# ddrakard/tensorflow-distributed-on-gke

Measured on AMD Instinct MI355X. Metric: tokens/sec (whole node), Transformer-base en-pt at 1/2/4/8 MI355X, higher is better.
Workload: dtype bf16; 1 GPU; model=transformer-base (6L, d_model=512, heads=8, d_ff=2048, vocab 7765/7010), global_batch=64, local_batch=64, seq_len=128, parallelism=dp1, hip_graph=single, grad_comm=fp32, defer_wgrad=True

## Files before the change

csrc/bindings/gemm.cpp:

```cpp
#include "common.h"

namespace {

void check_operand(const Tensor& t, bool kc, int64_t mn, int64_t K, int64_t ld, const char* n) {
  check_bf16(t, n);
  check_aligned(t, 16, n);
  if (kc) check_extent(t, mn, ld, round8(K), n);
  else check_extent(t, K, ld, round8(mn), n);
}
void check_group_c(const Tensor& C, bool f32, int64_t M, int64_t N, int64_t ldc) {
  TORCH_CHECK(C.is_cuda() && (C.scalar_type() == at::kFloat) == f32 &&
                  (f32 || C.scalar_type() == at::kBFloat16),
              "grouped gemm: C dtypes must match (f32 or bf16)");
  check_extent(C, M, ldc, N, "C");
}

void gemm(const Tensor& A, const Tensor& B, const Tensor& C, const optional<Tensor>& bias,
          const optional<Tensor>& aux, int64_t M, int64_t N, int64_t K, int64_t lda, int64_t ldb,
          int64_t ldc, int64_t ldaux, bool a_kc, bool b_kc, int64_t epi, double alpha,
          double beta, int64_t tile_cfg, int64_t splits, const optional<Tensor>& ws) {
  TORCH_CHECK(C.is_cuda(), "C must be a GPU tensor");
  const bool f32 = C.scalar_type() == at::kFloat;
  TORCH_CHECK(f32 || C.scalar_type() == at::kBFloat16, "C must be f32 or bf16");
  TORCH_CHECK(M > 0 && N > 0 && K > 0, "gemm: empty problem");
  TORCH_CHECK(lda % 8 == 0 && ldb % 8 == 0, "gemm: lda/ldb must be multiples of 8");
  TORCH_CHECK(lda >= round8(a_kc ? K : M), "gemm: lda < round8(", a_kc ? "K)" : "M)");
  TORCH_CHECK(ldb >= round8(b_kc ? K : N), "gemm: ldb < round8(", b_kc ? "K)" : "N)");
  check_operand(A, a_kc, M, K, lda, "A");
  check_operand(B, b_kc, N, K, ldb, "B");
  TORCH_CHECK(ldc >= N, "gemm: ldc < N");
  check_extent(C, M, ldc, N, "C");
  const float* bptr = nullptr;
  if (epi == 1 || epi == 2) {
    TORCH_CHECK(bias.has_value(), "gemm: bias epilogue needs bias");
    check_f32(*bias, "bias");
    TORCH_CHECK(bias->numel() >= N, "gemm: bias too short");
    bptr = bias->data_ptr<float>();
  }
  const void* xptr = nullptr;
  if (epi == 3) {
    TORCH_CHECK(aux.has_value(), "gemm: DRELU epilogue needs aux");
    check_bf16(*aux, "aux");
    check_extent(*aux, M, ldaux, N, "aux");
    xptr = aux->data_ptr();
  }
  float* wptr = nullptr;
  if (splits > 1) {
    TORCH_CHECK(ws.has_value(), "gemm: split-K needs a workspace");
    check_f32(*ws, "ws");
    TORCH_CHECK(ws->numel() >= splits * M * ldc, "gemm: workspace too small");
    wptr = ws->data_ptr<float>();
  }
  c10::DeviceGuard g(A.device());
  const int rc = tdg_gemm(A.data_ptr(), B.data_ptr(), C.data_ptr(), bptr, xptr, (int)M, (int)N,
                          (int)K, (int)lda, (int)ldb, (int)ldc, (int)ldaux, a_kc, b_kc, (int)epi,
                          f32, (float)alpha, (float)beta, (int)tile_cfg, (int)splits, wptr,
                          stream_of(A));
  check_err(rc, "tdg gemm");
}

void gemm_grouped(const std::vector<Tensor>& As, const std::vector<Tensor>& Bs,
                  const std::vector<Tensor>& Cs, int64_t M, int64_t N, int64_t K, int64_t lda,
                  int64_t ldb, int64_t ldc, bool a_kc, bool b_kc, double alpha, double beta,
                  int64_t tile_cfg) {
  const size_t G = As.size();
  TORCH_CHECK(G >= 1 && G <= 32 && Bs.size() == G && Cs.size() == G, "gemm_grouped: 1..32 problems");
  TORCH_CHECK(M > 0 && N > 0 && K > 0 && lda % 8 == 0 && ldb % 8 == 0 && ldc >= N, "gemm_grouped: shape");
  const bool f32 = Cs[0].scalar_type() == at::kFloat;
  std::vector<const void*> a(G), b(G);
  std::vector<void*> c(G);
  for (size_t i = 0; i < G; ++i) {
    check_operand(As[i], a_kc, M, K, lda, "A");
    check_operand(Bs[i], b_kc, N, K, ldb, "B");
    check_group_c(Cs[i], f32, M, N, ldc);
    a[i] = As[i].data_ptr();
    b[i] = Bs[i].data_ptr();
    c[i] = Cs[i].data_ptr();
  }
  c10::DeviceGuard g(As[0].device());
  const int rc = tdg_gemm_grouped(a.data(), b.data(), c.data(), (int)G, (int)M, (int)N, (int)K,
                                  (int)lda, (int)ldb, (int)ldc, a_kc, b_kc, f32, (float)alpha,
                                  (float)beta, (int)tile_cfg, stream_of(As[0]));
  check_err(rc, "tdg gemm_grouped");
}

void gemm_ragged(const std::vector<Tensor>& As, const std::vector<Tensor>& Bs,
                 const std::vector<Tensor>& Cs, const std::vector<int64_t>& shapes, int64_t K,
                 bool a_kc, bool b_kc, double alpha, double beta,
                 const std::vector<c10::optional<Tensor>>& bias_out) {
  const size_t P = As.size();
  TORCH_CHECK(P >= 1 && P <= 64 && Bs.size() == P && Cs.size() == P && shapes.size() == 7 * P,
              "gemm_ragged: 1..64 problems, 7 shape values each (M, N, lda, ldb, ldc, t_first, "
              "t_count)");
  TORCH_CHECK(K > 0 && K % 64 == 0, "gemm_ragged: K must be a multiple of 64");
  const bool f32 = Cs[0].scalar_type() == at::kFloat;
  std::vector<const void*> a(P), b(P);
  std::vector<void*> c(P);
  std::vector<int> sh(7 * P);
  for (size_t i = 0; i < P; ++i) {
    const int64_t M = shapes[7 * i], N = shapes[7 * i + 1], lda = shapes[7 * i + 2],
                  ldb = shapes[7 * i + 3], ldc = shapes[7 * i + 4];
    TORCH_CHECK(M > 0 && N > 0 && lda % 8 == 0 && ldb % 8 == 0 && ldc >= N, "gemm_ragged: shape");
    check_operand(As[i], a_kc, M, K, lda, "A");
    check_operand(Bs[i], b_kc, N, K, ldb, "B");
    check_group_c(Cs[i], f32, M, N, ldc);
    a[i] = As[i].data_ptr();
    b[i] = Bs[i].data_ptr();
    c[i] = Cs[i].data_ptr();
    for (int j = 0; j < 7; ++j) sh[7 * i + j] = (int)shapes[7 * i + j];
  }
  TORCH_CHECK(bias_out.empty() || bias_out.size() == P, "gemm_ragged: bias_out must be empty or P long");
  std::vector<float*> bo(P, nullptr);
  bool any_bias = false;
  for (size_t i = 0; i < bias_out.size(); ++i) {
    if (!bias_out[i].has_value()) continue;
    const Tensor& t = *bias_out[i];
    TORCH_CHECK(!a_kc, "gemm_ragged: fused bias sums need an MN-contiguous A");
    check_f32(t, "bias_out");
    TORCH_CHECK(t.is_contiguous() && t.numel() == shapes[7 * i], "gemm_ragged: bias_out[", i,
                "] must hold M floats");
    bo[i] = t.data_ptr<float>();
    any_bias = true;
  }
  c10::DeviceGuard g(As[0].device());
  const int rc = tdg_gemm_ragged(a.data(), b.data(), c.data(), (int)P, sh.data(), (int)K, a_kc,
                                 b_kc, f32, (float)alpha, (float)beta,
                                 any_bias ? bo.data() : nullptr, stream_of(As[0]));
  check_err(rc, "tdg gemm_ragged");
}

void colsum(const Tensor& X, const Tensor& out, const Tensor& part, int64_t M, int64_t N,
            int64_t ld, int64_t rows_per_block, double beta) {
  check_bf16(X, "X");
  check_f32(out, "out");
  check_f32(part, "part");
  check_extent(X, M, ld, N, "X");
  TORCH_CHECK(out.numel() >= N, "colsum: out too short");
  TORCH_CHECK(part.numel() >= ((M + rows_per_block - 1) / rows_per_block) * N,
              "colsum: partial buffer too small");
  c10::DeviceGuard g(X.device());
  tdg_colsum(X.data_ptr(), out.data_ptr<float>(), part.data_ptr<float>(), (int)M, (int)N, (int)ld,
             (int)rows_per_block, (float)beta, stream_of(X));
  check_err(0, "tdg colsum");
}

void colsum_grouped(const std::vector<Tensor>& Xs, const std::vector<Tensor>& outs,
                    const Tensor& part, int64_t M, int64_t N, int64_t ld, int64_t rows_per_block,
                    double beta) {
  const size_t G = Xs.size();
  TORCH_CHECK(G >= 1 && G <= 32 && outs.size() == G, "colsum_grouped: 1..32 problems");
  check_f32(part, "part");
  const int64_t nparts = (M + rows_per_block - 1) / rows_per_block;
  TORCH_CHECK(part.numel() >= (int64_t)G * nparts * N, "colsum_grouped: partials too small");
  std::vector<const void*> x(G);
  std::vector<float*> o(G);
  for (size_t i = 0; i < G; ++i) {
    check_bf16(Xs[i], "X");
    check_extent(Xs[i], M, ld, N, "X");
    check_f32(outs[i], "out");
    TORCH_CHECK(outs[i].numel() >= N, "colsum_grouped: out too short");
    x[i] = Xs[i].data_ptr();
    o[i] = outs[i].data_ptr<float>();
  }
  c10::DeviceGuard g(Xs[0].device());
  check_err(tdg_colsum_grouped(x.data(), o.data(), (int)G, part.data_ptr<float>(), (int)M, (int)N,
                               (int)ld, (int)rows_per_block, (float)beta, stream_of(Xs[0])),
            "tdg colsum_grouped");
}

}

void def_gemm(py::module_& m) {
  m.def("gemm", &gemm);
  m.def("gemm_grouped", &gemm_grouped);
  m.def("gemm_ragged", &gemm_ragged, py::arg("As"), py::arg("Bs"), py::arg("Cs"), py::arg("shapes"),
        py::arg("K"), py::arg("a_kc"), py::arg("b_kc"), py::arg("alpha"), py::arg("beta"),
        py::arg("bias_out") = std::vector<c10::optional<Tensor>>{});
  m.def("colsum", &colsum);
  m.def("colsum_grouped", &colsum_grouped);
}
```

csrc/include/tdg_api.h:

```cpp
#pragma once
#include <hip/hip_runtime.h>
#include <stdint.h>

#include "tdg_attn.h"

extern "C" {

int tdg_gemm(const void* A, const void* B, void* C, const float* bias, const void* aux, int M,
             int N, int K, int lda, int ldb, int ldc, int ldaux, int a_kc, int b_kc, int epi,
             int out_f32, float alpha, float beta, int tile_cfg, int splits, float* ws,
             hipStream_t st);
int tdg_gemm_grouped(const void* const* A, const void* const* B, void* const* C, int G, int M,
                     int N, int K, int lda, int ldb, int ldc, int a_kc, int b_kc, int out_f32,
                     float alpha, float beta, int tile_cfg, hipStream_t st);
int tdg_gemm_ragged(const void* const* A, const void* const* B, void* const* C, int P,
                    const int* shapes, int K, int a_kc, int b_kc, int out_f32, float alpha,
                    float beta, float* const* bias_out, hipStream_t st);
void tdg_colsum(const void* X, float* out, float* part, int M, int N, int ld, int rows_per_block,
                float beta, hipStream_t st);
int tdg_colsum_grouped(const void* const* X, float* const* out, int G, float* part, int M, int N,
                       int ld, int rows_per_block, float beta, hipStream_t st);

int tdg_attn_fwd(const tdg::AttnArgs* a, int hd, hipStream_t st);
int tdg_qkv_attn_fwd(const tdg::QkvAttnArgs* qa, hipStream_t st);
int tdg_attn_bwd(const tdg::AttnArgs* a, int hd, hipStream_t st);
int tdg_attn_bwd_fdo(const tdg::AttnArgs* a, hipStream_t st);
int tdg_attn_probs(const tdg::AttnArgs* a, int hd, float* probs, hipStream_t st);
int tdg_attn_fwd_fp8(const tdg::AttnArgs* a, int hd, hipStream_t st);
int tdg_attn_bwd_f8(const tdg::AttnArgs* a, int hd, hipStream_t st);

int tdg_ln_fwd(const void* x, const void* s, const float* gamma, const float* beta, void* y,
               void* hsave, float* mean, float* rstd, int M, int D, float p, uint64_t seed,
               const long long* ctr, uint64_t site, float eps, void* y8, const float* s8,
               unsigned* amax8, void* kbits, hipStream_t st);
int tdg_ln_bwd(const void* dy, const void* hsave, const float* mean, const float* rstd,
               const float* gamma, void* dh, void* ds, const void* dres, float* dgamma,
               float* dbeta, float* dbias, float* ws, int M, int D, float p, uint64_t seed,
               const long long* ctr, uint64_t site, int accumulate, int skip_reduce, int rpb,
               void* ds8, const float* s8, unsigned* amax8, const void* kbits, hipStream_t st);
int tdg_reduce_partials_multi(const float* const* parts, float* const* outs, const int* nparts,
                              int G, int N, float beta, hipStream_t st);

int tdg_embed_fwd(const void* tok, int tok64, const void* table, const float* pe, void* out, int M,
                  int L, int D, float scale, float p, uint64_t seed, const long long* ctr,
                  uint64_t site, void* kbits, hipStream_t st);
int tdg_embed_bwd(const void* tok, int tok64, const void* dout, float* dtable, int M, int D,
                  float scale, float p, uint64_t seed, const long long* ctr, uint64_t site,
                  hipStream_t st);
int tdg_embed_bwd_det(const void* tok, int tok64, const void* dout, float* dtable, long long* acc,
                      int M, int D, long long V, float scale, float p, uint64_t seed,
                      const long long* ctr, uint64_t site, float beta, hipStream_t st);
void tdg_embed_csr_ws(int M, int V, int D, long long* n32, long long* n64);
int tdg_embed_csr_ok(int M, int V);
int tdg_embed_csr_sort(int ntab, const void* const* tok, const int* tok64, const int* M,
                       const int* V, int* const* ws32, long long* stamps, hipStream_t st);
int tdg_embed_csr_apply(const void* dout, const void* kbits, float* dtable, int* ws32,
                        long long* ws64, int M, int D, int V, float scale, float p, uint64_t seed,
                        const long long* ctr, uint64_t site, float beta, hipStream_t st);

int tdg_count_tokens(const void* labels, int lab64, int M, float* out, hipStream_t st);
int tdg_prep_batch(const void* src, int S, const void* tgt, int T1, int B, int lab64, void* tgt_in,
                   void* labels, int* src_len, int* tgt_len, float* ntok, long long* ctr,
                   int* row_lab, unsigned* ticket, int* bad_rows, hipStream_t st);
int tdg_xent(void* logits, int M, int V, int ldl, const void* labels, int lab64, const float* ntok,
             float workers, float smoothing, float* row_loss, float* row_correct, int write_grad,
             hipStream_t st);
int tdg_xent_stats(const float* row_loss, const float* row_correct, int M, const float* ntok,
                   float workers, float* step_out, float* accum, hipStream_t st);

int tdg_adam(float* p, float* g, float* m, float* v, void* shadow, long long n, long long* step,
             float beta1, float beta2, float eps, float lr_const, float d_model, float warmup,
             float grad_scale, float weight_decay, int sched, int zero_grad, int inc_step,
             const float* gstate, hipStream_t st);
int tdg_adam_chunks(float* p, float* g, float* m, float* v, void* shadow, long long n,
                    const void* chunks, int nchunks, long long* step, float beta1, float beta2,
                    float eps, float lr_const, float d_model, float warmup, float grad_scale,
                    float weight_decay, int sched, int zero_grad, int inc_step,
                    const float* scale8, unsigned* amax8, const float* gstate, hipStream_t st);
int tdg_adam_step_inc(long long* step, const float* gstate, hipStream_t st);
long long tdg_grad_sumsq(const float* g, const void* chunks, long long nchunks, long long n,
                         float* partials, hipStream_t st);
int tdg_grad_norm_finalize(const float* partials, long long nparts, float* state,
                           unsigned* counters, float clip, int skip_on, float grad_scale,
                           hipStream_t st);
int tdg_to_bf16(const float* p, void* o, long long n, hipStream_t st);
int tdg_transpose_grouped(const void* const* src, void* const* dst, int G, int R, int C,
                          hipStream_t st);

int tdg_gemm_fp8(const void* A, const void* B, void* C, const float* bias, const float* sa,
                 const float* sb, void* C8, const float* sc8, unsigned* amax, int M, int N, int K,
                 int lda, int ldb, int ldc, int ldc8, int epi, int cfg, int afmt, int cfmt,
                 const void* aux, int ldaux, float beta, const void* aux8, float* colsum_out,
                 float colsum_beta, float* ws, hipStream_t st);
int tdg_wgrad_fp8(const void* const* A, const void* const* B, float* const* C,
                  const float* const* sa, const float* const* sb, int P, const int* shapes, int T,
                  float beta, hipStream_t st);
int tdg_fp8_set_persist(int on);
int tdg_fp8_quant(const void* x, void* y8, long long n, const float* scale, unsigned* amax,
                  int fmt, hipStream_t st);
int tdg_fp8_quant_multi(const void* const* x, void* const* y, const long long* n, const int* slot,
                        int nseg, const float* scale, unsigned* amax, hipStream_t st);
int tdg_fp8_quant_colsum(const void* x, int ld, void* y8, int M, int N, const float* scale,
                         unsigned* amax, float* part, int fmt, hipStream_t st);
int tdg_fp8_quant_t(const void* const* src, void* const* dst, const int* slot, int G, int R, int C,
                    const float* scale, unsigned* amax, hipStream_t st);
int tdg_fp8_scale_update(float* scale, unsigned* amax, int n, float margin_pow2, float fmax,
                         hipStream_t st);
int tdg_fp8_dequant(const void* x8, float* y, long long n, float inv_scale, hipStream_t st);

int tdg_signal_create(unsigned long long** host, unsigned long long** dhost,
                      unsigned long long** cnt);
int tdg_signal_emit(unsigned long long* cnt, unsigned long long* dhost, hipStream_t st);

}
```

csrc/include/tdg_gemm.h:

```cpp
#pragma once
#include "tdg_common.h"

#include <type_traits>

namespace tdg {

constexpr int BK = 64;

template <bool KC, int R>
__device__ __forceinline__ int lds_off(int row, int byte) {
  if constexpr (KC) {
    const int seg = (byte >> 5) ^ ((row >> 1) & 3);
    return row * (BK * 2) + (seg << 5) + (byte & 31);
  } else if constexpr (R >= 128) {
    const int seg = (byte >> 5) ^ ((row & 3) | (((row >> 3) & 1) << 2));
    return row * (R * 2) + (seg << 5) + (byte & 31);
  } else {
    static_assert(R == 64, "MN-contiguous tiles must be 64 or 128 wide");
    const int seg = (byte >> 5) ^ (((row >> 1) & 1) | (((row >> 3) & 1) << 1));
    return row * 128 + (seg << 5) + (byte & 31);
  }
}

template <bool KC, int R, int NW>
struct Glds {
  static constexpr int BYTES = R * BK * 2;
  static constexpr int P = BYTES / (NW * 1024);
  static_assert(BYTES % (NW * 1024) == 0, "tile must split into 1 KiB pieces per wave");
  static constexpr int RPP = KC ? 8 : 1024 / (R * 2);
  static constexpr int CPR = KC ? 8 : R / 8;
  int row[P];
  int col[P];
  __device__ __forceinline__ void init(int wid, int lane) {
#pragma unroll
    for (int i = 0; i < P; ++i) {
      const int j = wid * P + i;
      const int r = j * RPP + lane / CPR;
      const int pc = lane % CPR;
      int c;
      if constexpr (KC) {
        c = (((pc >> 1) ^ ((r >> 1) & 3)) << 1) | (pc & 1);
      } else if constexpr (R >= 128) {
        c = (((pc >> 1) ^ ((r & 3) | (((r >> 3) & 1) << 2))) << 1) | (pc & 1);
      } else {
        c = (((pc >> 1) ^ (((r >> 1) & 1) | (((r >> 3) & 1) << 1))) << 1) | (pc & 1);
      }
      row[i] = r;
      col[i] = c * 8;
    }
  }
  __device__ __forceinline__ void issue(const bf16_t* __restrict__ X, int ld, int len, int kend,
                                        int mn0, int k0, char* lds, int wid) const {
#pragma unroll
    for (int i = 0; i < P; ++i) {
      long long off;
      if constexpr (KC) {
        int mn = mn0 + row[i];
        mn = mn < len ? mn : len - 1;
        int k = k0 + col[i];
        k = k < kend ? k : 0;
        off = (long long)mn * ld + k;
      } else {
        int k = k0 + row[i];
        k = k < kend ? k : kend - 1;
        int mn = mn0 + col[i];
        mn = mn < len ? mn : 0;
        off = (long long)k * ld + mn;
      }
      __builtin_amdgcn_global_load_lds(
          (const void*)(X + off),
          (__attribute__((address_space(3))) void*)(lds + (wid * P + i) * 1024), 16, 0, 0);
    }
  }
  __device__ __forceinline__ static void zero_ktail(char* lds, int k0, int kend, int tid, int nt) {
    if constexpr (KC) {
      for (int id = tid; id < R * 8; id += nt) {
        const int r = id >> 3, c = id & 7;
        const int kk = k0 + c * 8;
        if (kk + 8 <= kend) continue;
        short8_t* p = reinterpret_cast<short8_t*>(lds + lds_off<KC, R>(r, c * 16));
        short8_t v = *p;
#pragma unroll
        for (int e = 0; e < 8; ++e)
          if (kk + e >= kend) v[e] = 0;
        *p = v;
      }
    } else {
      for (int id = tid; id < BK * (R / 8); id += nt) {
        const int r = id / (R / 8), c = id % (R / 8);
        if (k0 + r < kend) continue;
        *reinterpret_cast<short8_t*>(lds + lds_off<KC, R>(r, c * 16)) =
            short8_t{0, 0, 0, 0, 0, 0, 0, 0};
      }
    }
  }
};

#ifndef TDG_EPI_SC1
#define TDG_EPI_SC1 1
#endif
#ifndef TDG_GEMM_PRIO
#define TDG_GEMM_PRIO 1
#endif
__device__ __forceinline__ void prio_hi() {
  if (TDG_GEMM_PRIO) __builtin_amdgcn_s_setprio(1);
}
__device__ __forceinline__ void prio_lo() {
  if (TDG_GEMM_PRIO) __builtin_amdgcn_s_setprio(0);
}

template <int N>
__device__ __forceinline__ void wait_vmcnt() {
  asm volatile("s_waitcnt vmcnt(%0)" ::"n"(N) : "memory");
}
template <int N>
__device__ __forceinline__ void wait_vmcnt_known() {
  static_assert(N >= 0 && N <= 63, "vmcnt range");
  __builtin_amdgcn_s_waitcnt((N & 15) | (7 << 4) | (15 << 8) | ((N >> 4) << 14));
}

template <int PT, int NMAX>
__device__ __forceinline__ void wait_tiles(int n) {
  static_assert(NMAX <= 6 && PT * NMAX <= 63, "vmcnt range");
  if (NMAX >= 6 && n >= 6) { wait_vmcnt<(NMAX >= 6 ? 6 * PT : 0)>(); return; }
  if (NMAX >= 5 && n >= 5) { wait_vmcnt<(NMAX >= 5 ? 5 * PT : 0)>(); return; }
  if (NMAX >= 4 && n >= 4) { wait_vmcnt<(NMAX >= 4 ? 4 * PT : 0)>(); return; }
  if (NMAX >= 3 && n >= 3) { wait_vmcnt<(NMAX >= 3 ? 3 * PT : 0)>(); return; }
  if (NMAX >= 2 && n >= 2) { wait_vmcnt<(NMAX >= 2 ? 2 * PT : 0)>(); return; }
  if (NMAX >= 1 && n >= 1) { wait_vmcnt<PT>(); return; }
  wait_vmcnt<0>();
}

__device__ __forceinline__ void lds_barrier() {
  asm volatile("s_waitcnt lgkmcnt(0)" ::: "memory");
  __builtin_amdgcn_s_barrier();
  asm volatile("" ::: "memory");
}

template <bool KC, int R>
__device__ __forceinline__ short8_t frag(const char* lds, int base, int s, int lane) {
  if constexpr (KC) {
    const int row = base + (lane & 15);
    const int byte = (s * 4 + (lane >> 4)) * 16;
    return lds_read_b128_async(lds + lds_off<KC, R>(row, byte));
  } else {
    const int g = lane >> 4, w = lane & 15, q = w >> 2, p = w & 3;
    const int krow = s * 32 + 8 * g + q;
    const int byte = (base + 4 * p) * 2;
    const short4_t lo = lds_read_tr_async(lds + lds_off<KC, R>(krow, byte));
    const short4_t hi = lds_read_tr_async(lds + lds_off<KC, R>(krow + 4, byte));
    return cat4(lo, hi);
  }
}

template <bool KC>
constexpr int frag_ops() {
  return KC ? 1 : 2;
}

enum Epi : int {
  EPI_NONE = 0,
  EPI_BIAS = 1,
  EPI_BIAS_RELU = 2,
  EPI_DRELU = 3,
};

template <int EPI>
__device__ __forceinline__ f32x4 load_bias4(const float* __restrict__ bias, int n, int N) {
  f32x4 b = {0.f, 0.f, 0.f, 0.f};
  if constexpr (EPI == EPI_BIAS || EPI == EPI_BIAS_RELU) {
    if (n + 4 <= N && (reinterpret_cast<uintptr_t>(bias + n) & 15) == 0) {
      b = *reinterpret_cast<const f32x4*>(bias + n);
    } else {
#pragma unroll
      for (int r = 0; r < 4; ++r) b[r] = bias[min(n + r, N - 1)];
    }
  }
  return b;
}

template <int EPI, bool OUT_F32>
__device__ __forceinline__ bool epi_vec_ok(const void* C, int ldc, const bf16_t* aux, int ldaux) {
  constexpr int ES = OUT_F32 ? 4 : 2;
  bool ok = (ldc % 4) == 0 && (reinterpret_cast<uintptr_t>(C) % (4 * ES)) == 0;
  if constexpr (EPI == EPI_DRELU) ok = ok && (ldaux % 4) == 0 && (reinterpret_cast<uintptr_t>(aux) & 7) == 0;
  return ok;
}

template <int EPI, bool OUT_F32>
__device__ __forceinline__ void epi_store4(void* __restrict__ Cv, int ldc, int M, int N, int m, int n,
                                           const f32x4& a, float alpha, float beta, const f32x4& bn,
                                           const bf16_t* __restrict__ aux, int ldaux, bool vec) {
  if (m >= M || n >= N) return;
  float v[4];
#pragma unroll
  for (int r = 0; r < 4; ++r) {
    v[r] = alpha * a[r];
    if constexpr (EPI == EPI_BIAS) v[r] += bn[r];
    if constexpr (EPI == EPI_BIAS_RELU) v[r] = fmaxf(v[r] + bn[r], 0.f);
  }
  const size_t off = (size_t)m * ldc + n;
  if (vec && n + 4 <= N) {
    if constexpr (EPI == EPI_DRELU) {
      const short4_t x = *reinterpret_cast<const short4_t*>(aux + (size_t)m * ldaux + n);
#pragma unroll
      for (int r = 0; r < 4; ++r)
        if (!(bf2f((bf16_t)x[r]) > 0.f)) v[r] = 0.f;
    }
    if constexpr (OUT_F32) {
      f32x4* cp = reinterpret_cast<f32x4*>(reinterpret_cast<float*>(Cv) + off);
      f32x4 o = {v[0], v[1], v[2], v[3]};
      if (beta != 0.f) o += beta * *cp;
      *cp = o;
    } else {
      short4_t* cp = reinterpret_cast<short4_t*>(reinterpret_cast<bf16_t*>(Cv) + off);
      if (beta != 0.f) {
        const short4_t old = *cp;
#pragma unroll
        for (int r = 0; r < 4; ++r) v[r] += beta * bf2f((bf16_t)old[r]);
      }
      short4_t o;
#pragma unroll
      for (int r = 0; r < 4; ++r) o[r] = (short)f2bf(v[r]);
      *cp = o;
    }
  } else {
#pragma unroll
    for (int r = 0; r < 4; ++r) {
      if (n + r >= N) break;
      float x = v[r];
      if constexpr (EPI == EPI_DRELU) {
        if (!(bf2f(aux[(size_t)m * ldaux + n + r]) > 0.f)) x = 0.f;
      }
      if constexpr (OUT_F32) {
        float* cp = reinterpret_cast<float*>(Cv) + off + r;
        if (beta != 0.f) x += beta * *cp;
        *cp = x;
      } else {
        bf16_t* cp = reinterpret_cast<bf16_t*>(Cv) + off + r;
        if (beta != 0.f) x += beta * bf2f(*cp);
        *cp = f2bf(x);
      }
    }
  }
}

template <int EPI, bool OUT_F32, int TM, int TN, int RPASS>
struct EpiLds {
  static constexpr int ES = OUT_F32 ? 4 : 2;
  static constexpr int SP = TN * 16 * ES + 16;
  static constexpr int CPR = TN * 16 * ES / 16;
  static constexpr int EPC = 16 / ES;
  static constexpr int ITER = RPASS * CPR / 64;
  static constexpr int BYTES = RPASS * SP;
  static_assert(RPASS % 16 == 0 && (TM * 16) % RPASS == 0, "passes of whole 16-row sub-tiles");
  static_assert((RPASS * CPR) % 64 == 0, "whole chunk iterations");

  __device__ static __forceinline__ int row_of(int lane, int t) { return (lane + 64 * t) / CPR; }
  __device__ static __forceinline__ int col_of(int lane, int t) { return ((lane + 64 * t) % CPR) * EPC; }

  __device__ static __forceinline__ void run(char* wimg, const f32x4 (&acc)[TM][TN], int lane,
                                             void* __restrict__ Cv, int ldc, int M, int N, int mw0,
                                             int nw0, float alpha, float beta,
                                             const float* __restrict__ bias,
                                             const bf16_t* __restrict__ aux, int ldaux, bool vec) {
    int4 none[ITER];
    run_pre<false>(wimg, acc, lane, Cv, ldc, M, N, mw0, nw0, alpha, beta, bias, aux, ldaux, vec,
                   none, false, none, false);
  }
  template <bool PRE>
  __device__ static __forceinline__ void run_pre(char* wimg, const f32x4 (&acc)[TM][TN], int lane,
                                                 void* __restrict__ Cv, int ldc, int M, int N,
                                                 int mw0, int nw0, float alpha, float beta,
                                                 const float* __restrict__ bias,
                                                 const bf16_t* __restrict__ aux, int ldaux, bool vec,
                                                 const int4 (&pre_aux)[ITER], bool use_aux,
                                                 const int4 (&pre_c)[ITER], bool use_c) {
    const int g = lane >> 4, r16 = lane & 15;
    bool vok = vec && ((ldc * ES) % 16) == 0 && (reinterpret_cast<uintptr_t>(Cv) & 15) == 0;
    if constexpr (EPI == EPI_DRELU)
      vok = vok && (ldaux % EPC) == 0 && (reinterpret_cast<uintptr_t>(aux) % (2 * EPC)) == 0;
#if TDG_EPI_SC1
    const WtBuf wt(Cv, ((size_t)(M - 1) * ldc + N) * ES);
#endif
    f32x4 bn[TN];
#pragma unroll
    for (int j = 0; j < TN; ++j) bn[j] = load_bias4<EPI>(bias, nw0 + 16 * j + 4 * g, N);
    using VecT = typename std::conditional<OUT_F32, f32x4, short8_t>::type;
    constexpr bool AUX8 = EPI == EPI_DRELU && EPC == 8;
    const bool loc_aux = AUX8 && !(PRE && use_aux) && vok;
    const bool loc_c = !(PRE && use_c) && beta != 0.f && vok;
#pragma unroll
    for (int p = 0; p < TM * 16 / RPASS; ++p) {
      int4 la[ITER], lc[ITER];
      if (loc_aux || loc_c) {
#pragma unroll
        for (int t = 0; t < ITER; ++t) {
          const int id = lane + 64 * t;
          const int m = mw0 + p * RPASS + id / CPR, n = nw0 + (id % CPR) * EPC;
          const bool in = m < M && n + EPC <= N;
          if (loc_aux) {
            const bf16_t* a = in ? aux + (size_t)m * ldaux + n : aux;
            la[t] = *reinterpret_cast<const int4*>(a);
          }
          if (loc_c) {
            const char* c = in ? reinterpret_cast<const char*>(Cv) + ((size_t)m * ldc + n) * ES
                               : reinterpret_cast<const char*>(Cv);
            lc[t] = *reinterpret_cast<const int4*>(c);
          }
        }
      }
#pragma unroll
      for (int ii = 0; ii < RPASS / 16; ++ii) {
        const int i = p * (RPASS / 16) + ii;
#pragma unroll
        for (int j = 0; j < TN; ++j) {
          float v[4];
#pragma unroll
          for (int r = 0; r < 4; ++r) {
            v[r] = alpha * acc[i][j][r];
            if constexpr (EPI == EPI_BIAS) v[r] += bn[j][r];
            if constexpr (EPI == EPI_BIAS_RELU) v[r] = fmaxf(v[r] + bn[j][r], 0.f);
          }
          char* dst = wimg + (16 * ii + r16) * SP + (16 * j + 4 * g) * ES;
          if constexpr (OUT_F32) {
            *reinterpret_cast<f32x4*>(dst) = f32x4{v[0], v[1], v[2], v[3]};
          } else {
            short4_t w;
#pragma unroll
            for (int r = 0; r < 4; ++r) w[r] = (short)f2bf(v[r]);
            *reinterpret_cast<short4_t*>(dst) = w;
          }
        }
      }
      asm volatile("s_waitcnt lgkmcnt(0)" ::: "memory");
#pragma unroll
      for (int t = 0; t < ITER; ++t) {
        const int id = lane + 64 * t;
        const int row = id / CPR, ch = id % CPR;
        const int m = mw0 + p * RPASS + row;
        const int n = nw0 + ch * EPC;
        VecT vals = *reinterpret_cast<const VecT*>(wimg + row * SP + ch * 16);
        if (m >= M || n >= N) continue;
        char* cp = reinterpret_cast<char*>(Cv) + ((size_t)m * ldc + n) * ES;
        if (vok && n + EPC <= N) {
          if constexpr (EPI == EPI_DRELU) {
            if constexpr (EPC == 8) {
              const short8_t x = __builtin_bit_cast(short8_t, (PRE && use_aux) ? pre_aux[t] : la[t]);
#pragma unroll
              for (int e = 0; e < 8; ++e)
                if (!(bf2f((bf16_t)x[e]) > 0.f)) vals[e] = 0;
            } else {
              const short4_t x = *reinterpret_cast<const short4_t*>(aux + (size_t)m * ldaux + n);
#pragma unroll
              for (int e = 0; e < 4; ++e)
                if (!(bf2f((bf16_t)x[e]) > 0.f)) vals[e] = 0;
            }
          }
          if (beta != 0.f) {
            const VecT old = __builtin_bit_cast(VecT, (PRE && use_c) ? pre_c[t] : lc[t]);
            if constexpr (OUT_F32) {
              vals += beta * old;
            } else {
#pragma unroll
              for (int e = 0; e < 8; ++e)
                vals[e] = (short)f2bf(bf2f((bf16_t)vals[e]) + beta * bf2f((bf16_t)old[e]));
            }
          }
#if TDG_EPI_SC1
          wt.st16(cp, vals);
#else
          *reinterpret_cast<VecT*>(cp) = vals;
#endif
        } else {
#pragma unroll
          for (int e = 0; e < EPC; ++e) {
            if (n + e >= N) break;
            float v = OUT_F32 ? (float)vals[e] : bf2f((bf16_t)vals[e]);
            if constexpr (EPI == EPI_DRELU) {
              if (!(bf2f(aux[(size_t)m * ldaux + n + e]) > 0.f)) v = 0.f;
            }
            if constexpr (OUT_F32) {
              float* c = reinterpret_cast<float*>(cp) + e;
              if (beta != 0.f) v += beta * *c;
              *c = v;
            } else {
              bf16_t* c = reinterpret_cast<bf16_t*>(cp) + e;
              if (beta != 0.f) v += beta * bf2f(*c);
              *c = f2bf(v);
            }
          }
        }
      }
      asm volatile("s_waitcnt lgkmcnt(0)" ::: "memory");
    }
  }
};

template <int N>
__device__ __forceinline__ void tie_all(short8_t (&f)[N]) {
#pragma unroll
  for (int i = 0; i < N; ++i) tie(f[i]);
}

}
```

csrc/kernels/gemm.hip:

```cpp
#include "tdg_api.h"
#include "gemm_impl.h"

namespace tdg {

__global__ __launch_bounds__(256) void colsum_partial_kernel(const bf16_t* __restrict__ X,
                                                             float* __restrict__ part, int M, int N,
                                                             int ld, int rows_per_block) {
  __shared__ float red[32][65];
  const int cg = threadIdx.x & 7, rl = threadIdx.x >> 3;
  const int col0 = blockIdx.x * 64 + cg * 8;
  const int r0 = blockIdx.y * rows_per_block;
  const int r1 = min(M, r0 + rows_per_block);
  float acc[8];
#pragma unroll
  for (int i = 0; i < 8; ++i) acc[i] = 0.f;
  const bool vec = (col0 + 8 <= N) && (ld % 8 == 0);
  for (int r = r0 + rl; r < r1; r += 32) {
    const bf16_t* p = X + (size_t)r * ld + col0;
    if (vec) {
      const short8_t v = *reinterpret_cast<const short8_t*>(p);
#pragma unroll
      for (int i = 0; i < 8; ++i) acc[i] += bf2f((bf16_t)v[i]);
    } else {
#pragma unroll
      for (int i = 0; i < 8; ++i)
        if (col0 + i < N) acc[i] += bf2f(p[i]);
    }
  }
#pragma unroll
  for (int i = 0; i < 8; ++i) red[rl][cg * 8 + i] = acc[i];
  __syncthreads();
  if (threadIdx.x < 64) {
    float s = 0.f;
#pragma unroll 8
    for (int k = 0; k < 32; ++k) s += red[k][threadIdx.x];
    const int col = blockIdx.x * 64 + threadIdx.x;
    if (col < N) part[(size_t)blockIdx.y * N + col] = s;
  }
}

struct ColsumGroup {
  const bf16_t* X[32];
  float* out[32];
};

__global__ __launch_bounds__(256) void colsum_partial_grouped_kernel(ColsumGroup grp,
                                                                     float* __restrict__ part, int M,
                                                                     int N, int ld,
                                                                     int rows_per_block) {
  __shared__ float red[32][65];
  const bf16_t* X = grp.X[blockIdx.z];
  float* pz = part + (size_t)blockIdx.z * gridDim.y * N;
  const int cg = threadIdx.x & 7, rl = threadIdx.x >> 3;
  const int col0 = blockIdx.x * 64 + cg * 8;
  const int r0 = blockIdx.y * rows_per_block;
  const int r1 = min(M, r0 + rows_per_block);
  float acc[8];
#pragma unroll
  for (int i = 0; i < 8; ++i) acc[i] = 0.f;
  const bool vec = (col0 + 8 <= N) && (ld % 8 == 0);
  for (int r = r0 + rl; r < r1; r += 32) {
    const bf16_t* p = X + (size_t)r * ld + col0;
    if (vec) {
      const short8_t v = *reinterpret_cast<const short8_t*>(p);
#pragma unroll
      for (int i = 0; i < 8; ++i) acc[i] += bf2f((bf16_t)v[i]);
    } else {
#pragma unroll
      for (int i = 0; i < 8; ++i)
        if (col0 + i < N) acc[i] += bf2f(p[i]);
    }
  }
#pragma unroll
  for (int i = 0; i < 8; ++i) red[rl][cg * 8 + i] = acc[i];
  __syncthreads();
  if (threadIdx.x < 64) {
    float s = 0.f;
#pragma unroll 8
    for (int k = 0; k < 32; ++k) s += red[k][threadIdx.x];
    const int col = blockIdx.x * 64 + threadIdx.x;
    if (col < N) pz[(size_t)blockIdx.y * N + col] = s;
  }
}

__global__ __launch_bounds__(256) void reduce_partials_grouped_kernel(ColsumGroup grp,
                                                                      const float* __restrict__ part,
                                                                      int N, int P, float beta) {
  __shared__ float red[4][64];
  const float* pz = part + (size_t)blockIdx.y * P * N;
  float* out = grp.out[blockIdx.y];
  const int c = threadIdx.x & 63, g = threadIdx.x >> 6;
  const int col = blockIdx.x * 64 + c;
  float s = 0.f;
  if (col < N) {
#pragma unroll 8
    for (int p = g; p < P; p += 4) s += pz[(size_t)p * N + col];
  }
  red[g][c] = s;
  __syncthreads();
  if (g == 0 && col < N) {
    const float t = red[0][c] + red[1][c] + red[2][c] + red[3][c];
    out[col] = (beta != 0.f ? beta * out[col] : 0.f) + t;
  }
}

}

extern "C" int tdg_gemm(const void* A, const void* B, void* C, const float* bias, const void* aux,
                        int M, int N, int K, int lda, int ldb, int ldc, int ldaux, int a_kc,
                        int b_kc, int epi, int out_f32, float alpha, float beta, int tile_cfg,
                        int splits, float* ws, hipStream_t st) {
  const bf16_t* a = (const bf16_t*)A;
  const bf16_t* b = (const bf16_t*)B;
  const bf16_t* x = (const bf16_t*)aux;
  auto fn = a_kc ? (b_kc ? gemm_nt : gemm_nn) : (b_kc ? gemm_tt : gemm_tn);
  return fn(epi, out_f32 != 0, tile_cfg, a, b, C, bias, x, M, N, K, lda, ldb, ldc, ldaux, alpha,
            beta, splits, ws, st);
}

extern "C" int tdg_gemm_grouped(const void* const* A, const void* const* B, void* const* C, int G,
                                int M, int N, int K, int lda, int ldb, int ldc, int a_kc, int b_kc,
                                int out_f32, float alpha, float beta, int tile_cfg, hipStream_t st) {
  if (G < 1 || G > MAXG) return -2;
  GemmGroup g{};
  for (int i = 0; i < G; ++i) {
    g.A[i] = (const bf16_t*)A[i];
    g.B[i] = (const bf16_t*)B[i];
    g.C[i] = C[i];
  }
  auto fn = a_kc ? (b_kc ? gemm_grouped_nt : gemm_grouped_nn)
                 : (b_kc ? gemm_grouped_tt : gemm_grouped_tn);
  return fn(g, G, M, N, K, lda, ldb, ldc, out_f32 != 0, alpha, beta, tile_cfg, st);
}

extern "C" int tdg_gemm_ragged(const void* const* A, const void* const* B, void* const* C, int P,
                               const int* shapes, int K, int a_kc, int b_kc, int out_f32,
                               float alpha, float beta, float* const* bias_out,
                               hipStream_t st) {
  if (P < 1 || P > R256_MAXP) return -2;
  R256Args args{};
  int ncls = 0, tiles = 0;
  bool prev_partial = false;
  for (int i = 0; i < P; ++i) {
    const int* s = shapes + 7 * i;
    const int tpp = cdiv(s[0], 256) * cdiv(s[1], 256);
    const int first = s[5], count = s[6] < 0 ? tpp - s[5] : s[6];
    if (first < 0 || count <= 0 || first + count > tpp) return -8;
    const bool partial = count != tpp;
    const bool same = ncls > 0 && !partial && !prev_partial && args.cls[ncls - 1].M == s[0] &&
                      args.cls[ncls - 1].N == s[1] && args.cls[ncls - 1].lda == s[2] &&
                      args.cls[ncls - 1].ldb == s[3] && args.cls[ncls - 1].ldc == s[4];
    if (!same) {
      if (ncls == R256_MAXC) return -5;
      R256Class& c = args.cls[ncls++];
      c.M = s[0]; c.N = s[1]; c.lda = s[2]; c.ldb = s[3]; c.ldc = s[4];
      c.tiles_m = cdiv(s[0], 256); c.tiles_n = cdiv(s[1], 256);
      c.tile_start = tiles; c.prob_start = i; c.t_first = first;
      if ((!a_kc && s[2] % 8) || (!b_kc && s[3] % 8)) return -6;
    }
    prev_partial = partial;
    tiles += count;
    args.A[i] = (const bf16_t*)A[i];
    args.B[i] = (const bf16_t*)B[i];
    args.C[i] = C[i];
    args.bias_out[i] = bias_out ? bias_out[i] : nullptr;
    if (args.bias_out[i] && a_kc) return -7;
  }
  args.ncls = ncls;
  if (a_kc && b_kc) return gemm_ragged_nt(args, tiles, K, out_f32 != 0, alpha, beta, st);
  if (a_kc && !b_kc) return out_f32 ? -4 : gemm_ragged_nn(args, tiles, K, false, alpha, beta, st);
  if (!a_kc && !b_kc) return gemm_ragged_tn(args, tiles, K, out_f32 != 0, alpha, beta, st);
  return -4;
}

extern "C" void tdg_colsum(const void* X, float* out, float* part, int M, int N, int ld,
                           int rows_per_block, float beta, hipStream_t st) {
  const int nparts = cdiv(M, rows_per_block);
  dim3 grid(cdiv(N, 64), nparts);
  hipLaunchKernelGGL(colsum_partial_kernel, grid, dim3(256), 0, st, (const bf16_t*)X, part, M, N,
                     ld, rows_per_block);
  launch_reduce_partials(part, out, N, nparts, beta, st);
}

extern "C" int tdg_colsum_grouped(const void* const* X, float* const* out, int G, float* part,
                                  int M, int N, int ld, int rows_per_block, float beta,
                                  hipStream_t st) {
  if (G < 1 || G > 32) return -2;
  ColsumGroup g{};
  for (int i = 0; i < G; ++i) {
    g.X[i] = (const bf16_t*)X[i];
    g.out[i] = out[i];
  }
  const int nparts = cdiv(M, rows_per_block);
  hipLaunchKernelGGL(colsum_partial_grouped_kernel, dim3(cdiv(N, 64), nparts, G), dim3(256), 0, st,
                     g, part, M, N, ld, rows_per_block);
  hipLaunchKernelGGL(reduce_partials_grouped_kernel, dim3(cdiv(N, 64), G), dim3(256), 0, st, g,
                     part, N, nparts, beta);
  return 0;
}
```

csrc/kernels/gemm_impl.h:

```cpp
#pragma once
#include "tdg_common.h"
#include "tdg_gemm.h"
#include "tdg_reduce.h"
#include "gemm_pipe.h"

#include <cstdlib>
#include <type_traits>

namespace tdg {



constexpr int MAXG = 32;
struct GemmGroup {
  const bf16_t* A[MAXG];
  const bf16_t* B[MAXG];
  void* C[MAXG];
};

template <int BM, int BN, int WM, int WN, int STAGES, bool A_KC, bool B_KC, int EPI,
          bool OUT_F32>
__global__ __launch_bounds__(WM* WN * 64) void gemm_kernel(
    const bf16_t* __restrict__ A, const bf16_t* __restrict__ B, void* __restrict__ Cv,
    const float* __restrict__ bias, const bf16_t* __restrict__ aux, int M, int N, int K, int lda,
    int ldb, int ldc, int ldaux, float alpha, float beta, int k_per_split, long long split_stride,
    const GemmGroup grp) {
  if (gridDim.y > 1) {
    A = grp.A[blockIdx.y];
    B = grp.B[blockIdx.y];
    Cv = grp.C[blockIdx.y];
  }
  constexpr int NW = WM * WN;
  constexpr int NT = NW * 64;
  constexpr int TM = BM / WM / 16;
  constexpr int TN = BN / WN / 16;
  constexpr int A_BYTES = BM * BK * 2, B_BYTES = BN * BK * 2;
  constexpr int SB = A_BYTES + B_BYTES;
  using GA = Glds<A_KC, BM, NW>;
  using GB = Glds<B_KC, BN, NW>;
  constexpr int PT = GA::P + GB::P;
  extern __shared__ __attribute__((aligned(16))) char smem[];

  const int tid = threadIdx.x, lane = tid & 63;
  const int wid = __builtin_amdgcn_readfirstlane(tid >> 6);
  const int wm = wid / WN, wn = wid % WN;
  const int tiles_m = cdiv(M, BM), tiles_n = cdiv(N, BN);
  const int nwg = tiles_m * tiles_n;
  const int t = xcd_remap(blockIdx.x, nwg);
  int tm, tn;
  if (tiles_n <= tiles_m) {
    tn = t % tiles_n;
    tm = t / tiles_n;
  } else {
    tm = t % tiles_m;
    tn = t / tiles_m;
  }
  const int m0 = tm * BM, n0 = tn * BN;
  TDG_STAMP(0);

  const int kb = blockIdx.z * k_per_split;
  const int ke = min(K, kb + k_per_split);
  const int nk = cdiv(ke - kb, BK);
  const bool ktail = ((ke - kb) % BK) != 0;

  GA ga;
  GB gb;
  ga.init(wid, lane);
  gb.init(wid, lane);

  using OutT = typename std::conditional<OUT_F32, float, bf16_t>::type;
  constexpr int WTM = BM / WM, WTN = BN / WN;
  constexpr int RPASS = OUT_F32 ? (WTM < 32 ? WTM : 32) : WTM;
  using Epi = EpiLds<EPI, OUT_F32, TM, TN, RPASS>;
  using EpiF = EpiLds<EPI_NONE, true, TM, TN, (WTM < 32 ? WTM : 32)>;
  static_assert(NW * Epi::BYTES <= STAGES * (BM + BN) * BK * 2 &&
                    NW * EpiF::BYTES <= STAGES * (BM + BN) * BK * 2,
                "epilogue images must fit in the pipeline LDS");
  const bool split = gridDim.z > 1;
  const bool vec = epi_vec_ok<EPI, OUT_F32>(Cv, ldc, aux, ldaux);
  constexpr bool SINGLE = RPASS == WTM;
  const bool pre_aux = SINGLE && EPI == EPI_DRELU && !split && vec && (ldaux % 8) == 0 &&
                       (reinterpret_cast<uintptr_t>(aux) & 15) == 0;
  const bool pre_c = SINGLE && beta != 0.f && !split && vec && ((ldc * (int)sizeof(OutT)) % 16) == 0;
  int4 aux_r[Epi::ITER], c_r[Epi::ITER];
#pragma unroll
  for (int t = 0; t < Epi::ITER; ++t) {
    const int m = m0 + wm * WTM + Epi::row_of(lane, t);
    const int n = n0 + wn * WTN + Epi::col_of(lane, t);
    const bool in = m < M && n + Epi::EPC <= N;
    if (pre_aux && in) aux_r[t] = *reinterpret_cast<const int4*>(aux + (size_t)m * ldaux + n);
    if (pre_c && in)
      c_r[t] = *reinterpret_cast<const int4*>(reinterpret_cast<const OutT*>(Cv) + (size_t)m * ldc + n);
  }

  f32x4 acc[TM][TN];
#pragma unroll
  for (int i = 0; i < TM; ++i)
#pragma unroll
    for (int j = 0; j < TN; ++j) acc[i][j] = f32x4{0.f, 0.f, 0.f, 0.f};

  static_assert(BK == 64, "two 32-deep k-steps per tile");
  const int abase = wm * (BM / WM), bbase = wn * (BN / WN);
#pragma unroll
  for (int s = 0; s < STAGES; ++s) {
    if (s < nk) {
      ga.issue(A, lda, M, ke, m0, kb + s * BK, smem + s * SB, wid);
      gb.issue(B, ldb, N, ke, n0, kb + s * BK, smem + s * SB + A_BYTES, wid);
    }
  }
  short8_t fa0[TM], fb0[TN], fa1[TM], fb1[TN];
  if (nk > 0) {
    if (nk >= STAGES)
      wait_vmcnt<(STAGES - 1) * PT>();
    else
      wait_vmcnt<0>();
    lds_barrier();
    TDG_STAMP(1);
    if (ktail && nk == 1) {
      GA::zero_ktail(smem, kb, ke, tid, NT);
      GB::zero_ktail(smem + A_BYTES, kb, ke, tid, NT);
      lds_barrier();
    }
#pragma unroll
    for (int i = 0; i < TM; ++i) fa0[i] = frag<A_KC, BM>(smem, abase + 16 * i, 0, lane);
#pragma unroll
    for (int j = 0; j < TN; ++j) fb0[j] = frag<B_KC, BN>(smem + A_BYTES, bbase + 16 * j, 0, lane);
  }

  constexpr int STEP_OPS = TM * frag_ops<A_KC>() + TN * frag_ops<B_KC>();
  auto kstep = [&](int kt, auto modec) {
    constexpr int MODE = decltype(modec)::value;
    const char* st = smem + (kt % STAGES) * SB;
#pragma unroll
    for (int i = 0; i < TM; ++i) fa1[i] = frag<A_KC, BM>(st, abase + 16 * i, 1, lane);
#pragma unroll
    for (int j = 0; j < TN; ++j) fb1[j] = frag<B_KC, BN>(st + A_BYTES, bbase + 16 * j, 1, lane);
    lgkm_wait<STEP_OPS>();
    tie_all(fa0);
    tie_all(fb0);
    prio_hi();
#pragma unroll
    for (int i = 0; i < TM; ++i)
#pragma unroll
      for (int j = 0; j < TN; ++j) acc[i][j] = mfma16(fb0[j], fa0[i], acc[i][j]);
    prio_lo();
    if constexpr (MODE >= 1) {
      if constexpr (MODE >= 2) wait_vmcnt<(STAGES - 2) * PT>();
      else wait_vmcnt<0>();
      lds_barrier();
      const char* nx = smem + ((kt + 1) % STAGES) * SB;
      if constexpr (MODE <= 2) {
        if (ktail && kt + 1 == nk - 1) {
          GA::zero_ktail(const_cast<char*>(nx), kb + (kt + 1) * BK, ke, tid, NT);
          GB::zero_ktail(const_cast<char*>(nx) + A_BYTES, kb + (kt + 1) * BK, ke, tid, NT);
          lds_barrier();
        }
      }
      if constexpr (MODE == 3) {
        char* ns = smem + (kt % STAGES) * SB;
        ga.issue(A, lda, M, ke, m0, kb + (kt + STAGES) * BK, ns, wid);
        gb.issue(B, ldb, N, ke, n0, kb + (kt + STAGES) * BK, ns + A_BYTES, wid);
      }
#pragma unroll
      for (int i = 0; i < TM; ++i) fa0[i] = frag<A_KC, BM>(nx, abase + 16 * i, 0, lane);
#pragma unroll
      for (int j = 0; j < TN; ++j) fb0[j] = frag<B_KC, BN>(nx + A_BYTES, bbase + 16 * j, 0, lane);
    } else {
      lgkm_wait<0>();
    }
    tie_all(fa1);
    tie_all(fb1);
    prio_hi();
#pragma unroll
    for (int i = 0; i < TM; ++i)
#pragma unroll
      for (int j = 0; j < TN; ++j) acc[i][j] = mfma16(fb1[j], fa1[i], acc[i][j]);
    prio_lo();
  };
  {
    int kt = 0;
    for (; kt + STAGES < nk; ++kt) kstep(kt, std::integral_constant<int, 3>{});
    if (kt + STAGES - 1 < nk && kt + 1 < nk) kstep(kt++, std::integral_constant<int, 2>{});
    for (; kt + 1 < nk; ++kt) kstep(kt, std::integral_constant<int, 1>{});
    if (kt < nk) kstep(kt, std::integral_constant<int, 0>{});
  }

  TDG_STAMP(2);
  lds_barrier();
  const int mw0 = m0 + wm * WTM, nw0 = n0 + wn * WTN;
  if (split) {
    float* Cs = reinterpret_cast<float*>(Cv) + (size_t)blockIdx.z * split_stride;
    EpiF::run(smem + wid * EpiF::BYTES, acc, lane, Cs, ldc, M, N, mw0, nw0, 1.f, 0.f, nullptr,
              nullptr, 0, epi_vec_ok<EPI_NONE, true>(Cs, ldc, nullptr, 0));
  } else {
    Epi::template run_pre<true>(smem + wid * Epi::BYTES, acc, lane, Cv, ldc, M, N, mw0, nw0, alpha,
                                beta, bias, aux, ldaux, vec, aux_r, pre_aux, c_r, pre_c);
  }
#ifdef TDG_STAMPS
  TDG_STAMP(3);
  asm volatile("s_waitcnt vmcnt(0)" ::: "memory");
  TDG_STAMP(4);
#endif
}

constexpr int R256_MAXP = 64, R256_MAXC = 8;
struct R256Class {
  int M, N, lda, ldb, ldc, tiles_m, tiles_n, tile_start, prob_start, t_first;
};
struct R256Args {
  const bf16_t* A[R256_MAXP];
  const bf16_t* B[R256_MAXP];
  void* C[R256_MAXP];
  float* bias_out[R256_MAXP];
  R256Class cls[R256_MAXC];
  int ncls;
};

template <bool A_KC, bool B_KC, int EPI, bool OUT_F32>
__global__ __launch_bounds__(512) void gemm256_kernel(const R256Args args,
                                                      const float* __restrict__ bias,
                                                      const bf16_t* __restrict__ aux, int K,
                                                      int ldaux, float alpha, float beta) {
  constexpr int NW = 8;
  constexpr int HB = 128 * BK * 2;
  constexpr int SB = 4 * HB;
  using GA = Glds<A_KC, 128, NW>;
  using GB = Glds<B_KC, 128, NW>;
  static_assert(GA::P == 2 && GB::P == 2, "half-tile = 2 pieces per wave");
  extern __shared__ __attribute__((aligned(16))) char smem[];

  const int tid = threadIdx.x, lane = tid & 63;
  const int wid = __builtin_amdgcn_readfirstlane(tid >> 6);
  const int wm = wid >> 2, wn = wid & 3;

  const int t0 = xcd_remap(blockIdx.x, gridDim.x);
  R256Class cl = args.cls[0];
#pragma unroll
  for (int i = 1; i < R256_MAXC; ++i)
    if (i < args.ncls && t0 >= args.cls[i].tile_start) cl = args.cls[i];
  const int M = cl.M, N = cl.N, lda = cl.lda, ldb = cl.ldb, ldc = cl.ldc;
  const int tpp = cl.tiles_m * cl.tiles_n;
  const int lt = t0 - cl.tile_start + cl.t_first;
  const int p = cl.prob_start + lt / tpp;
  const int t = lt % tpp;
  const bf16_t* __restrict__ A = args.A[p];
  const bf16_t* __restrict__ B = args.B[p];
  void* __restrict__ Cv = args.C[p];
  int tm, tn;
  if (cl.tiles_n <= cl.tiles_m) {
    tn = t % cl.tiles_n;
    tm = t / cl.tiles_n;
  } else {
    tm = t % cl.tiles_m;
    tn = t / cl.tiles_m;
  }
  float* __restrict__ bias_out = A_KC ? nullptr : args.bias_out[p];
  const bool do_bsum = bias_out != nullptr && tn == 0;
  float bsum0 = 0.f, bsum1 = 0.f;
  const int m0 = tm * 256, n0 = tn * 256;
  const int nk = K / BK;
  TDG_STAMP(0);

  GA ga;
  GB gb;
  ga.init(wid, lane);
  gb.init(wid, lane);
  uint32_t a_off[2][2], b_off[2][2];
#pragma unroll
  for (int i = 0; i < 2; ++i) {
    const int xa = A_KC ? ga.row[i] : ga.col[i];
    const int xb = B_KC ? gb.row[i] : gb.col[i];
    const int ka = A_KC ? ga.col[i] : ga.row[i];
    const int kb = B_KC ? gb.col[i] : gb.row[i];
#pragma unroll
    for (int hh = 0; hh < 2; ++hh) {
      int ma = m0 + (xa >> 6) * 128 + hh * 64 + (xa & 63);
      int nb = n0 + (xb >> 5) * 64 + hh * 32 + (xb & 31);
      if (A_KC) {
        ma = ma < M ? ma : M - 1;
        a_off[hh][i] = 2u * (uint32_t)(ma * lda + ka);
      } else {
        ma = ma < M ? ma : 0;
        a_off[hh][i] = 2u * (uint32_t)(ka * lda + ma);
      }
      if (B_KC) {
        nb = nb < N ? nb : N - 1;
        b_off[hh][i] = 2u * (uint32_t)(nb * ldb + kb);
      } else {
        nb = nb < N ? nb : 0;
        b_off[hh][i] = 2u * (uint32_t)(kb * ldb + nb);
      }
    }
  }
  const int nrec_a = 2 * (A_KC ? (M - 1) * lda + K : (K - 1) * lda + M);
  const int nrec_b = 2 * (B_KC ? (N - 1) * ldb + K : (K - 1) * ldb + N);
  const uint32_t kstep_a = A_KC ? BK * 2u : (uint32_t)BK * (uint32_t)lda * 2u;
  const uint32_t kstep_b = B_KC ? BK * 2u : (uint32_t)BK * (uint32_t)ldb * 2u;
  auto issue = [&](const bf16_t* X, int nrec, const uint32_t* offs, uint32_t soff, char* dst) {
#pragma unroll
    for (int i = 0; i < 2; ++i)
      __builtin_amdgcn_raw_ptr_buffer_load_lds(
          __builtin_amdgcn_make_buffer_rsrc(const_cast<bf16_t*>(X), (short)0, nrec, 0x00020000),
          (__attribute__((address_space(3))) void*)(dst + (wid * 2 + i) * 1024), 16, offs[i],
          (int)soff, 0, 0);
  };
  auto issue_half = [&](int kt, int h) {
    char* st = smem + (kt & 1) * SB;
    if (h == 0) issue(A, nrec_a, a_off[0], kstep_a * (uint32_t)kt, st + 0 * HB);
    else if (h == 1) issue(B, nrec_b, b_off[0], kstep_b * (uint32_t)kt, st + 2 * HB);
    else if (h == 2) issue(B, nrec_b, b_off[1], kstep_b * (uint32_t)kt, st + 3 * HB);
    else issue(A, nrec_a, a_off[1], kstep_a * (uint32_t)kt, st + 1 * HB);
  };

  f32x4 acc[8][4];
#pragma unroll
  for (int i = 0; i < 8; ++i)
#pragma unroll
    for (int j = 0; j < 4; ++j) acc[i][j] = f32x4{0.f, 0.f, 0.f, 0.f};

  const int arow = wm * 64, brow = wn * 32;
  short8_t fa[8][2], fb[4][2];
  auto bias_sum = [&](int ph) {
    const bf16x2_t one = __builtin_bit_cast(bf16x2_t, 0x3f803f80);
    float bs = ph == 0 ? bsum0 : bsum1;
#pragma unroll
    for (int i = 0; i < 4; ++i) {
      if (i != wn) continue;
#pragma unroll
      for (int s2 = 0; s2 < 2; ++s2) {
        const short8_t f = ph == 0 ? fa[i][s2] : fa[4 + i][s2];
#pragma unroll
        for (int e = 0; e < 4; ++e)
          bs = __builtin_amdgcn_fdot2_f32_bf16(
              __builtin_bit_cast(bf16x2_t, (short2_t){f[2 * e], f[2 * e + 1]}), one, bs, false);
      }
    }
    if (ph == 0) bsum0 = bs;
    else bsum1 = bs;
  };
  {
#pragma unroll
    for (int h = 0; h < 4; ++h) issue_half(0, h);
    if (nk > 1) {
#pragma unroll
      for (int h = 0; h < 3; ++h) issue_half(1, h);
    }
    const int fg = lane >> 4, fcl = lane & 15, fq = fcl >> 2, fp = fcl & 3;
    const uint32_t lds0 = (uint32_t)(uintptr_t)smem;
    auto kc_base = [&](int row0, int s) -> uint32_t {
      return lds0 + (row0 + fcl) * (BK * 2) + (((2 * s + (fg >> 1)) ^ ((fcl >> 1) & 3)) << 5) + (fg & 1) * 16;
    };
    auto mn_base = [&](int sub) -> uint32_t {
      return lds0 + (8 * fg + fq) * 256 + 8 * fp + ((sub ^ (fq | ((fg & 1) << 2))) << 5);
    };
    uint32_t rba[4], rbb[2];
#pragma unroll
    for (int i = 0; i < 4; ++i) rba[i] = A_KC ? kc_base(arow, i & 1) : mn_base((arow >> 4) + i);
#pragma unroll
    for (int j = 0; j < 2; ++j) rbb[j] = B_KC ? kc_base(brow, j) : mn_base((brow >> 4) + j);
    auto frag_imm = [&](auto kcc, auto hc, auto ic, auto sc, const uint32_t* b) -> short8_t {
      constexpr bool KC = decltype(kcc)::value;
      constexpr int H = decltype(hc)::value, I = decltype(ic)::value, S = decltype(sc)::value;
      if constexpr (KC) {
        return lds_read_b128_at<H * HB + I * 16 * BK * 2>(b[S]);
      } else {
        return cat4(lds_read_tr16_at<H * HB + 8192 * S>(b[I]), lds_read_tr16_at<H * HB + 8192 * S + 1024>(b[I]));
      }
    };
    using AKCc = std::integral_constant<bool, A_KC>;
    using BKCc = std::integral_constant<bool, B_KC>;
    auto kstep_deep = [&](int kt, auto modec) {
      constexpr int MODE = decltype(modec)::value;
      const uint32_t stg = (uint32_t)(kt & 1) * SB;
      uint32_t ba[4], bb[2];
#pragma unroll
      for (int i = 0; i < 4; ++i) ba[i] = rba[i] + stg;
#pragma unroll
      for (int j = 0; j < 2; ++j) bb[j] = rbb[j] + stg;
#pragma unroll
      for (int ph = 0; ph < 4; ++ph) {
        if (ph < 3) {
          if (ph == 0) wait_vmcnt<MODE == 1 ? 4 : 10>();
          else if (ph == 1) wait_vmcnt<MODE == 1 ? 2 : 10>();
          else wait_vmcnt<MODE == 3 ? 12 : (MODE == 2 ? 8 : 0)>();
          lds_barrier();
          if (kt == 0 && ph == 0) TDG_STAMP(1);
        }
        using C0 = std::integral_constant<int, 0>;
        using C1 = std::integral_constant<int, 1>;
        using C2 = std::integral_constant<int, 2>;
        using C3 = std::integral_constant<int, 3>;
        if (ph == 0) {
          static_for<4>([&](auto I) {
            fa[I][0] = frag_imm(AKCc{}, C0{}, I, C0{}, ba);
            fa[I][1] = frag_imm(AKCc{}, C0{}, I, C1{}, ba);
          });
          static_for<2>([&](auto J) {
            fb[J][0] = frag_imm(BKCc{}, C2{}, J, C0{}, bb);
            fb[J][1] = frag_imm(BKCc{}, C2{}, J, C1{}, bb);
          });
        } else if (ph == 1) {
          static_for<2>([&](auto J) {
            fb[2 + J][0] = frag_imm(BKCc{}, C3{}, J, C0{}, bb);
            fb[2 + J][1] = frag_imm(BKCc{}, C3{}, J, C1{}, bb);
          });
        } else if (ph == 2) {
          static_for<4>([&](auto I) {
            fa[4 + I][0] = frag_imm(AKCc{}, C1{}, I, C0{}, ba);
            fa[4 + I][1] = frag_imm(AKCc{}, C1{}, I, C1{}, ba);
          });
        }
        if constexpr (MODE >= 2) {
          if (ph == 0) issue_half(kt + 1, 3);
        }
        if constexpr (MODE == 3) {
          if (ph == 1) {
            issue_half(kt + 2, 0);
            issue_half(kt + 2, 1);
          } else if (ph == 2) {
            issue_half(kt + 2, 2);
          }
        }
        if (ph < 3) {
          lgkm_wait<0>();
          if (ph == 0) {
#pragma unroll
            for (int i = 0; i < 4; ++i) tie_all(fa[i]);
#pragma unroll
            for (int j = 0; j < 2; ++j) tie_all(fb[j]);
          } else if (ph == 1) {
#pragma unroll
            for (int j = 2; j < 4; ++j) tie_all(fb[j]);
          } else {
#pragma unroll
            for (int i = 4; i < 8; ++i) tie_all(fa[i]);
          }
        }
        const int i0 = (ph < 2) ? 0 : 4;
        const int j0 = (ph == 0 || ph == 3) ? 0 : 2;
        __builtin_amdgcn_s_setprio(1);
#pragma unroll
        for (int s2 = 0; s2 < 2; ++s2)
#pragma unroll
          for (int i = 0; i < 4; ++i)
#pragma unroll
            for (int j = 0; j < 2; ++j)
              acc[i0 + i][j0 + j] = mfma16(fb[j0 + j][s2], fa[i0 + i][s2], acc[i0 + i][j0 + j]);
        __builtin_amdgcn_s_setprio(0);
        if (do_bsum && (ph == 0 || ph == 2)) bias_sum(ph);
      }
    };
    int kt = 0;
    for (; kt + 2 < nk; ++kt) kstep_deep(kt, std::integral_constant<int, 3>{});
    if (kt + 1 < nk) kstep_deep(kt++, std::integral_constant<int, 2>{});
    kstep_deep(kt, std::integral_constant<int, 1>{});
  }
  if (do_bsum) {
    bsum0 += __shfl_xor(bsum0, 16, 64);
    bsum0 += __shfl_xor(bsum0, 32, 64);
    bsum1 += __shfl_xor(bsum1, 16, 64);
    bsum1 += __shfl_xor(bsum1, 32, 64);
    if (lane < 16) {
      const int mA = m0 + wm * 128 + 16 * wn + lane, mB = mA + 64;
      if (mA < M) bias_out[mA] = alpha * bsum0 + (beta != 0.f ? beta * bias_out[mA] : 0.f);
      if (mB < M) bias_out[mB] = alpha * bsum1 + (beta != 0.f ? beta * bias_out[mB] : 0.f);
    }
  }

  TDG_STAMP(2);
  wait_vmcnt<0>();
  lds_barrier();
  {
    constexpr int RPASS = OUT_F32 ? 32 : 64;
    using Epi = EpiLds<EPI, OUT_F32, 8, 4, RPASS>;
    static_assert(8 * Epi::BYTES <= 2 * 4 * 128 * BK * 2, "epilogue images fit in the stages");
    Epi::run(smem + wid * Epi::BYTES, acc, lane, Cv, ldc, M, N, m0 + wm * 128, n0 + wn * 64, alpha,
             beta, bias, aux, ldaux, epi_vec_ok<EPI, OUT_F32>(Cv, ldc, aux, ldaux));
  }
#ifdef TDG_STAMPS
  TDG_STAMP(3);
  asm volatile("s_waitcnt vmcnt(0)" ::: "memory");
  TDG_STAMP(4);
#endif
}

template <int EPI, bool OUT_F32>
__global__ void splitk_reduce_kernel(const float* __restrict__ ws, void* __restrict__ Cv,
                                     const float* __restrict__ bias, const bf16_t* __restrict__ aux,
                                     int M, int N, int ldc, int ldaux, int splits,
                                     long long split_stride, float alpha, float beta) {
  const long long total = (long long)M * N;
  for (long long idx = (long long)blockIdx.x * blockDim.x + threadIdx.x; idx < total;
       idx += (long long)gridDim.x * blockDim.x) {
    const int m = (int)(idx / N), n = (int)(idx % N);
    const size_t o = (size_t)m * ldc + n;
    float v = 0.f;
    for (int z = 0; z < splits; ++z) v += ws[(size_t)z * split_stride + o];
    v *= alpha;
    if constexpr (EPI == EPI_BIAS) v += bias[n];
    if constexpr (EPI == EPI_BIAS_RELU) v = fmaxf(v + bias[n], 0.f);
    if constexpr (EPI == EPI_DRELU) {
      if (!(bf2f(aux[(size_t)m * ldaux + n]) > 0.f)) v = 0.f;
    }
    if constexpr (OUT_F32) {
      float* C = reinterpret_cast<float*>(Cv);
      if (beta != 0.f) v += beta * C[o];
      C[o] = v;
    } else {
      bf16_t* C = reinterpret_cast<bf16_t*>(Cv);
      if (beta != 0.f) v += beta * bf2f(C[o]);
      C[o] = f2bf(v);
    }
  }
}

}

using namespace tdg;

namespace {

template <int BM, int BN, int WM, int WN, int ST, bool AK, bool BKc, int EPI, bool F32>
void launch_cfg(const bf16_t* A, const bf16_t* B, void* C, const float* bias, const bf16_t* aux,
                int M, int N, int K, int lda, int ldb, int ldc, int ldaux, float alpha, float beta,
                int splits, float* ws, hipStream_t st, const GemmGroup* grp = nullptr, int G = 1) {
  static const GemmGroup kNoGroup{};
  const GemmGroup& gr = grp ? *grp : kNoGroup;
  const int tiles = cdiv(M, BM) * cdiv(N, BN);
  const int lds = ST * (BM + BN) * BK * 2;
  static bool attr_set = false;
  if (!attr_set) {
    (void)hipFuncSetAttribute((const void*)gemm_kernel<BM, BN, WM, WN, ST, AK, BKc, EPI, F32>,
                              hipFuncAttributeMaxDynamicSharedMemorySize, 160 * 1024);
    (void)hipFuncSetAttribute((const void*)gemm_kernel<BM, BN, WM, WN, ST, AK, BKc, EPI_NONE, true>,
                              hipFuncAttributeMaxDynamicSharedMemorySize, 160 * 1024);
    attr_set = true;
  }
  if (splits <= 1 || G > 1) {
    hipLaunchKernelGGL((gemm_kernel<BM, BN, WM, WN, ST, AK, BKc, EPI, F32>), dim3(tiles, G, 1),
                       dim3(WM * WN * 64), lds, st, A, B, C, bias, aux, M, N, K, lda, ldb, ldc,
                       ldaux, alpha, beta, K, 0LL, gr);
  } else {
    int kps = cdiv(cdiv(K, splits), BK) * BK;
    splits = cdiv(K, kps);
    const long long stride = (long long)M * ldc;
    hipLaunchKernelGGL((gemm_kernel<BM, BN, WM, WN, ST, AK, BKc, EPI_NONE, true>),
                       dim3(tiles, 1, splits), dim3(WM * WN * 64), lds, st, A, B, (void*)ws, bias,
                       aux, M, N, K, lda, ldb, ldc, ldaux, 1.f, 0.f, kps, stride, gr);
    const long long total = (long long)M * N;
    const int blocks = (int)std::min<long long>(4096, (total + 255) / 256);
    hipLaunchKernelGGL((splitk_reduce_kernel<EPI, F32>), dim3(blocks), dim3(256), 0, st, ws, C,
                       bias, aux, M, N, ldc, ldaux, splits, stride, alpha, beta);
  }
}

template <bool AK, bool BKc, int EPI, bool F32>
constexpr bool has_256() {
  if (AK && BKc) return !F32 || EPI == EPI_NONE;
  if (AK && !BKc) return !F32 && (EPI == EPI_NONE || EPI == EPI_DRELU);
  if (!AK && !BKc) return EPI == EPI_NONE;
  return false;
}

inline bool r256_offsets_ok(const R256Args& a, bool akc, bool bkc, int K) {
  for (int c = 0; c < a.ncls; ++c) {
    const R256Class& k = a.cls[c];
    const long long ea = akc ? (long long)(k.M - 1) * k.lda + K : (long long)(K - 1) * k.lda + k.M;
    const long long eb = bkc ? (long long)(k.N - 1) * k.ldb + K : (long long)(K - 1) * k.ldb + k.N;
    if (ea * 2 >= 0x7fffffffLL || eb * 2 >= 0x7fffffffLL) return false;
  }
  return true;
}

template <bool AK, bool BKc, int EPI, bool F32>
int launch_256(const R256Args& args, int tiles, const float* bias, const bf16_t* aux, int K,
               int ldaux, float alpha, float beta, hipStream_t st) {
  if constexpr (!has_256<AK, BKc, EPI, F32>()) {
    return -4;
  } else {
    if (K % BK != 0 || tiles <= 0) return -3;
    if (!r256_offsets_ok(args, AK, BKc, K)) return -9;
    constexpr int lds = 2 * 4 * 128 * BK * 2;
    static bool attr = false;
    if (!attr) {
      (void)hipFuncSetAttribute((const void*)gemm256_kernel<AK, BKc, EPI, F32>,
                                hipFuncAttributeMaxDynamicSharedMemorySize, 160 * 1024);
      attr = true;
    }
    hipLaunchKernelGGL((gemm256_kernel<AK, BKc, EPI, F32>), dim3(tiles), dim3(512), lds, st, args,
                       bias, aux, K, ldaux, alpha, beta);
    return 0;
  }
}

inline int r256_single(R256Args& a, const bf16_t* const* A, const bf16_t* const* B,
                       void* const* C, int G, int M, int N, int lda, int ldb, int ldc) {
  a.ncls = 1;
  for (int i = 0; i < G; ++i) {
    a.A[i] = A[i];
    a.B[i] = B[i];
    a.C[i] = C[i];
  }
  R256Class& c = a.cls[0];
  c.M = M; c.N = N; c.lda = lda; c.ldb = ldb; c.ldc = ldc;
  c.tiles_m = cdiv(M, 256); c.tiles_n = cdiv(N, 256);
  c.tile_start = 0; c.prob_start = 0; c.t_first = 0;
  return G * c.tiles_m * c.tiles_n;
}

template <int BM, int BN, int WM, int WN, int NS, bool AK, bool BKc, int EPI, bool F32>
bool launch_pipe(const bf16_t* A, const bf16_t* B, void* C, const float* bias, const bf16_t* aux,
                 int M, int N, int K, int lda, int ldb, int ldc, int ldaux, float alpha, float beta,
                 hipStream_t st) {
  if (K % PK != 0 || K <= 0) return false;
  const long long ab = AK ? (long long)(M - 1) * lda + K : (long long)(K - 1) * lda + M;
  const long long bb = BKc ? (long long)(N - 1) * ldb + K : (long long)(K - 1) * ldb + N;
  if (ab * 2 >= 0x7fffffffLL || bb * 2 >= 0x7fffffffLL) return false;
  if ((!AK && lda % 8) || (!BKc && ldb % 8)) return false;
  constexpr int lds = NS * (BM + BN) * PK * 2;
  static bool attr = false;
  if (!attr) {
    (void)hipFuncSetAttribute((const void*)gemm_pipe_kernel<BM, BN, WM, WN, NS, AK, BKc, EPI, F32>,
                              hipFuncAttributeMaxDynamicSharedMemorySize, 160 * 1024);
    attr = true;
  }
  const int tiles = cdiv(M, BM) * cdiv(N, BN);
  hipLaunchKernelGGL((gemm_pipe_kernel<BM, BN, WM, WN, NS, AK, BKc, EPI, F32>), dim3(tiles),
                     dim3(WM * WN * 64), lds,
                     st, A, B, C, bias, aux, M, N, K, lda, ldb, ldc, ldaux, alpha, beta,
                     (int)(ab * 2), (int)(bb * 2));
  return true;
}

template <bool AK, bool BKc, int EPI, bool F32>
void launch_tiles(int tile_cfg, const bf16_t* A, const bf16_t* B, void* C, const float* bias,
                  const bf16_t* aux, int M, int N, int K, int lda, int ldb, int ldc, int ldaux,
                  float alpha, float beta, int splits, float* ws, hipStream_t st,
                  const GemmGroup* grp = nullptr, int G = 1) {
  if (tile_cfg >= 20 && tile_cfg <= 26) {
    if (!grp && splits <= 1) {
      bool ok = false;
#define TDG_PIPE(ID, BM_, BN_, WM_, WN_, NS_)                                                      \
  case ID:                                                                                    \
    ok = launch_pipe<BM_, BN_, WM_, WN_, NS_, AK, BKc, EPI, F32>(A, B, C, bias, aux, M, N, K, lda, \
                                                                 ldb, ldc, ldaux, alpha, beta, st); \
    break;
      switch (tile_cfg) {
        TDG_PIPE(20, 256, 256, 2, 4, 4)
        TDG_PIPE(21, 256, 128, 2, 4, 6)
        TDG_PIPE(22, 128, 256, 2, 4, 6)
        TDG_PIPE(23, 256, 256, 2, 2, 4)
        TDG_PIPE(24, 256, 256, 2, 2, 5)
        TDG_PIPE(25, 256, 128, 2, 2, 6)
        TDG_PIPE(26, 128, 256, 2, 2, 6)
        default: break;
      }
#undef TDG_PIPE
      if (ok) return;
    }
    tile_cfg = 13;
  }
  if (tile_cfg == 12) {
    if (splits <= 1 && (AK || lda % 8 == 0) && (BKc || ldb % 8 == 0)) {
      R256Args args{};
      const bf16_t* a1 = A;
      const bf16_t* b1 = B;
      void* c1 = C;
      const int tiles = grp ? r256_single(args, grp->A, grp->B, grp->C, G, M, N, lda, ldb, ldc)
                            : r256_single(args, &a1, &b1, &c1, 1, M, N, lda, ldb, ldc);
      if (launch_256<AK, BKc, EPI, F32>(args, tiles, bias, aux, K, ldaux, alpha, beta, st) == 0)
        return;
    }
    tile_cfg = 13;
  }
#define TDG_CFG(ID, BM_, BN_, WM_, WN_, ST_)                                                  \
  case ID:                                                                                    \
    launch_cfg<BM_, BN_, WM_, WN_, ST_, AK, BKc, EPI, F32>(A, B, C, bias, aux, M, N, K, lda, ldb, \
                                                          ldc, ldaux, alpha, beta, splits, ws,   \
                                                          st, grp, G);                           \
    break;
  switch (tile_cfg) {
    TDG_CFG(0, 128, 128, 2, 2, 2)
    TDG_CFG(1, 128, 64, 2, 2, 3)
    TDG_CFG(2, 64, 128, 2, 2, 3)
    TDG_CFG(3, 64, 64, 2, 2, 4)
    TDG_CFG(4, 128, 128, 2, 4, 3)
    TDG_CFG(5, 256, 128, 4, 2, 2)
    TDG_CFG(6, 128, 256, 2, 4, 2)
    TDG_CFG(7, 64, 128, 2, 2, 2)
    TDG_CFG(9, 256, 128, 4, 2, 3)
    TDG_CFG(10, 128, 256, 2, 4, 3)
    TDG_CFG(11, 128, 128, 2, 2, 4)
    TDG_CFG(13, 128, 128, 2, 4, 4)
    TDG_CFG(14, 128, 128, 2, 4, 5)
    default:
      TDG_CFG(8, 64, 64, 2, 2, 2)
  }
#undef TDG_CFG
}

template <bool AK, bool BKc>
int dispatch_epi(int epi, bool f32, int tile_cfg, const bf16_t* A, const bf16_t* B, void* C,
                 const float* bias, const bf16_t* aux, int M, int N, int K, int lda, int ldb,
                 int ldc, int ldaux, float alpha, float beta, int splits, float* ws,
                 hipStream_t st) {
#define TDG_E(E, F)                                                                              \
  if (epi == E && f32 == F) {                                                                    \
    launch_tiles<AK, BKc, E, F>(tile_cfg, A, B, C, bias, aux, M, N, K, lda, ldb, ldc, ldaux,     \
                                alpha, beta, splits, ws, st);                                    \
    return 0;                                                                                    \
  }
  TDG_E(EPI_NONE, false)
  TDG_E(EPI_NONE, true)
  TDG_E(EPI_BIAS, false)
  TDG_E(EPI_BIAS, true)
  TDG_E(EPI_BIAS_RELU, false)
  TDG_E(EPI_DRELU, false)
#undef TDG_E
  return -1;
}

}

namespace tdg {
using GemmFn = int(int epi, bool f32, int tile_cfg, const bf16_t* A, const bf16_t* B, void* C,
                   const float* bias, const bf16_t* aux, int M, int N, int K, int lda, int ldb,
                   int ldc, int ldaux, float alpha, float beta, int splits, float* ws,
                   hipStream_t st);
using GemmGroupedFn = int(const GemmGroup& g, int G, int M, int N, int K, int lda, int ldb,
                          int ldc, bool f32, float alpha, float beta, int tile_cfg,
                          hipStream_t st);
using GemmRaggedFn = int(const R256Args& args, int tiles, int K, bool f32, float alpha,
                         float beta, hipStream_t st);
GemmFn gemm_nt, gemm_nn, gemm_tn, gemm_tt;
GemmGroupedFn gemm_grouped_nt, gemm_grouped_nn, gemm_grouped_tn, gemm_grouped_tt;
GemmRaggedFn gemm_ragged_nt, gemm_ragged_nn, gemm_ragged_tn, gemm_ragged_tt;
}

#define TDG_GEMM_LAYOUT(NAME, AK, BKc)                                                          \
  namespace tdg {                                                                               \
  int gemm_##NAME(int epi, bool f32, int tile_cfg, const bf16_t* A, const bf16_t* B, void* C,    \
                  const float* bias, const bf16_t* aux, int M, int N, int K, int lda, int ldb,     \
                  int ldc, int ldaux, float alpha, float beta, int splits, float* ws,              \
                  hipStream_t st) {                                                              \
    return dispatch_epi<AK, BKc>(epi, f32, tile_cfg, A, B, C, bias, aux, M, N, K, lda, ldb, ldc,  \
                                 ldaux, alpha, beta, splits, ws, st);                             \
  }                                                                                             \
  int gemm_grouped_##NAME(const GemmGroup& g, int G, int M, int N, int K, int lda, int ldb,       \
                          int ldc, bool f32, float alpha, float beta, int tile_cfg,              \
                          hipStream_t st) {                                                      \
    if (f32)                                                                                    \
      launch_tiles<AK, BKc, EPI_NONE, true>(tile_cfg, g.A[0], g.B[0], g.C[0], nullptr, nullptr,  \
                                            M, N, K, lda, ldb, ldc, 0, alpha, beta, 1, nullptr,  \
                                            st, &g, G);                                           \
    else                                                                                        \
      launch_tiles<AK, BKc, EPI_NONE, false>(tile_cfg, g.A[0], g.B[0], g.C[0], nullptr, nullptr, \
                                             M, N, K, lda, ldb, ldc, 0, alpha, beta, 1, nullptr, \
                                             st, &g, G);                                          \
    return 0;                                                                                   \
  }                                                                                             \
  int gemm_ragged_##NAME(const R256Args& args, int tiles, int K, bool f32, float alpha,         \
                         float beta, hipStream_t st) {                                          \
    if (f32)                                                                                    \
      return launch_256<AK, BKc, EPI_NONE, true>(args, tiles, nullptr, nullptr, K, 0, alpha, beta, \
                                                st);                                             \
    return launch_256<AK, BKc, EPI_NONE, false>(args, tiles, nullptr, nullptr, K, 0, alpha, beta,  \
                                                st);                                             \
  }                                                                                             \
  static_assert(std::is_same<decltype(gemm_##NAME), GemmFn>::value &&                           \
                    std::is_same<decltype(gemm_grouped_##NAME), GemmGroupedFn>::value &&        \
                    std::is_same<decltype(gemm_ragged_##NAME), GemmRaggedFn>::value,            \
                "layout entry points must match their declarations");                          \
  }
```

csrc/kernels/gemm_pipe.h:

```cpp
#pragma once
#include "tdg_common.h"
#include "tdg_gemm.h"

namespace tdg {

constexpr int PK = 32;

template <bool KC, int R>
__device__ __forceinline__ int plds_off(int row, int byte) {
  if constexpr (KC) {
    const int ch = (byte >> 4) ^ (((row >> 3) & 1) << 1);
    return row * 64 + (ch << 4) + (byte & 15);
  } else {
    return lds_off<false, R>(row, byte);
  }
}

template <bool KC, int R, int NW>
struct PStage {
  static constexpr int BYTES = R * PK * 2;
  static constexpr int P = BYTES / (NW * 1024);
  static_assert(BYTES % (NW * 1024) == 0, "tile must split into 1 KiB pieces per wave");
  uint32_t voff[P];
  const bf16_t* base;
  int nrec;
  uint32_t kstep;
  __device__ __forceinline__ void init(const bf16_t* X, int ld, int len, int mn0, int nrec_bytes,
                                       int wid, int lane) {
    base = X;
    nrec = nrec_bytes;
#pragma unroll
    for (int i = 0; i < P; ++i) {
      const int piece = wid * P + i;
      if constexpr (KC) {
        const int r = piece * 16 + (lane >> 2);
        const int c = (lane & 3) ^ (((r >> 3) & 1) << 1);
        int mn = mn0 + r;
        mn = mn < len ? mn : len - 1;
        voff[i] = (uint32_t)(((long long)mn * ld + c * 8) * 2);
      } else {
        constexpr int RPP = 1024 / (R * 2);
        constexpr int CPR = R / 8;
        const int r = piece * RPP + lane / CPR;
        const int pc = lane % CPR;
        const int c = (((pc >> 1) ^ ((r & 3) | (((r >> 3) & 1) << 2))) << 1) | (pc & 1);
        int mn = mn0 + c * 8;
        mn = mn < len ? mn : 0;
        voff[i] = (uint32_t)(((long long)r * ld + mn) * 2);
      }
    }
    kstep = KC ? PK * 2 : (uint32_t)PK * (uint32_t)ld * 2u;
  }
  __device__ __forceinline__ void issue(int i, int kt, char* lds, int wid) const {
    __builtin_amdgcn_raw_ptr_buffer_load_lds(
        __builtin_amdgcn_make_buffer_rsrc(const_cast<bf16_t*>(base), (short)0, nrec, 0x00020000), (__attribute__((address_space(3))) void*)(lds + (wid * P + i) * 1024), 16, voff[i],
        (int)(kstep * (uint32_t)kt), 0, 0);
  }
};

template <bool KC, int R>
struct PFrag {
  static constexpr int NI = KC ? 1 : 2;
  short8_t v;
  short4_t lo, hi;
  __device__ __forceinline__ void read(const char* lds, int base, int lane) {
    if constexpr (KC) {
      const int row = base + (lane & 15);
      v = lds_read_b128_async(lds + plds_off<true, R>(row, (lane >> 4) * 16));
    } else {
      const int g = lane >> 4, w = lane & 15, q = w >> 2, p = w & 3;
      const int krow = 8 * g + q;
      const int byte = (base + 4 * p) * 2;
      lo = lds_read_tr_async(lds + plds_off<false, R>(krow, byte));
      hi = lds_read_tr_async(lds + plds_off<false, R>(krow + 4, byte));
    }
  }
  __device__ __forceinline__ void tie_() {
    if constexpr (KC) {
      tie(v);
    } else {
      tie(lo);
      tie(hi);
    }
  }
  __device__ __forceinline__ short8_t get() const {
    if constexpr (KC) return v;
    else return cat4(lo, hi);
  }
};

template <int BM, int BN, int WM, int WN, int NS, bool A_KC, bool B_KC>
struct Pipe {
  static constexpr int NW = WM * WN;
  static constexpr int TM = BM / (16 * WM), TN = BN / (16 * WN);
  static constexpr int A_BYTES = BM * PK * 2, SB = A_BYTES + BN * PK * 2;
  using SA = PStage<A_KC, BM, NW>;
  using SBt = PStage<B_KC, BN, NW>;
  static constexpr int PT = SA::P + SBt::P;

  static __device__ __forceinline__ void stage(const SA& sa, const SBt& sb, char* smem, int kt,
                                               int wid) {
    char* st = smem + (kt % NS) * SB;
#pragma unroll
    for (int i = 0; i < SA::P; ++i) sa.issue(i, kt, st, wid);
#pragma unroll
    for (int i = 0; i < SBt::P; ++i) sb.issue(i, kt, st + A_BYTES, wid);
  }
  static __device__ __forceinline__ void stage_piece(const SA& sa, const SBt& sb, char* smem, int q,
                                                     int kt, int wid) {
    char* st = smem + (kt % NS) * SB;
    if (q < SA::P) sa.issue(q, kt, st, wid);
    else sb.issue(q - SA::P, kt, st + A_BYTES, wid);
  }

  using FA = PFrag<A_KC, BM>;
  using FBt = PFrag<B_KC, BN>;
  static constexpr int LGKM = (TM - 1) * FA::NI + TN * FBt::NI;
  template <typename F>
  static __device__ __forceinline__ void throttle() {
    lgkm_wait<15 - F::NI>();
  }

  static __device__ __forceinline__ void ktile(int kt, int nk, FBt (&FB)[TN],
                                               FBt (&FN)[TN], FA (&fa)[TM],
                                               f32x4 (&acc)[TM][TN], const SA& sa, const SBt& sb,
                                               char* smem, int lane, int wid, int abase,
                                               int bbase) {
    float none[TM];
    ktile_bs<false>(kt, nk, FB, FN, fa, acc, sa, sb, smem, lane, wid, abase, bbase, none, false);
  }
  static __device__ __forceinline__ void ktile_s(int kt, int nk, FBt (&FB)[TN],
                                                 FBt (&FN)[TN], FA (&fa)[TM],
                                                 f32x4 (&acc)[TM][TN], const SA& sa, const SBt& sb,
                                                 char* smem, int lane, int wid, int abase,
                                                 int bbase) {
    float none[TM];
    ktile_bs<false, true>(kt, nk, FB, FN, fa, acc, sa, sb, smem, lane, wid, abase, bbase, none,
                          false);
  }
  template <bool BS, bool STEADY = false>
  static __device__ __forceinline__ void ktile_bs(int kt, int nk, FBt (&FB)[TN],
                                                  FBt (&FN)[TN], FA (&fa)[TM],
                                                  f32x4 (&acc)[TM][TN], const SA& sa,
                                                  const SBt& sb, char* smem, int lane, int wid,
                                                  int abase, int bbase, float (&bs)[TM],
                                                  bool do_bs) {
    if (STEADY || kt + 1 < nk) {
      if constexpr (STEADY) wait_vmcnt<(NS - 3) * PT>();
      else wait_tiles<PT, NS - 2>(kt == 0 ? min(NS - 2, nk - 2) : min(NS - 3, nk - 2 - kt));
      __builtin_amdgcn_s_barrier();
    }
    const char* nx = smem + ((kt + 1) % NS) * SB;
    const int rt = kt - 1 + NS;
    const bool refill = STEADY || (rt < nk && kt >= 1);
#pragma unroll
    for (int j = 0; j < TN; ++j) {
      throttle<FBt>();
      FN[j].read(nx + A_BYTES, bbase + 16 * j, lane);
    }
#pragma unroll
    for (int i = 0; i < TM; ++i) {
      lgkm_wait<LGKM>();
      fa[i].tie_();
      if (i == 0) {
#pragma unroll
        for (int j = 0; j < TN; ++j) FB[j].tie_();
      }
      const short8_t a = fa[i].get();
      __builtin_amdgcn_s_setprio(1);
#pragma unroll
      for (int j = 0; j < TN; ++j) acc[i][j] = mfma16(FB[j].get(), a, acc[i][j]);
      __builtin_amdgcn_s_setprio(0);
      if constexpr (BS) {
        if (do_bs) {
          const bf16x2_t one = __builtin_bit_cast(bf16x2_t, 0x3f803f80);
          float b = bs[i];
#pragma unroll
          for (int e = 0; e < 4; ++e)
            b = __builtin_amdgcn_fdot2_f32_bf16(
                __builtin_bit_cast(bf16x2_t, (short2_t){a[2 * e], a[2 * e + 1]}), one, b, false);
          bs[i] = b;
        }
      }
      throttle<FA>();
      fa[i].read(nx, abase + 16 * i, lane);
#pragma unroll
      for (int q = 0; q < PT; ++q)
        if (q * TM / PT == i && refill) stage_piece(sa, sb, smem, q, rt, wid);
      __builtin_amdgcn_sched_barrier(0);
    }
  }
};

template <int BM, int BN, int WM, int WN, int NS, bool A_KC, bool B_KC, int EPI, bool OUT_F32>
__global__ __launch_bounds__(WM * WN * 64) void gemm_pipe_kernel(
    const bf16_t* __restrict__ A, const bf16_t* __restrict__ B, void* __restrict__ Cv,
    const float* __restrict__ bias, const bf16_t* __restrict__ aux, int M, int N, int K, int lda,
    int ldb, int ldc, int ldaux, float alpha, float beta, int a_bytes, int b_bytes) {
  using P = Pipe<BM, BN, WM, WN, NS, A_KC, B_KC>;
  constexpr int NW = P::NW, TM = P::TM, TN = P::TN, A_BYTES = P::A_BYTES, SB = P::SB, PT = P::PT;
  constexpr int WTM = BM / WM, WTN = BN / WN;
  static_assert(NS >= 3, "ring: refilled, being read, landed");
  extern __shared__ __attribute__((aligned(16))) char smem[];

  const int tid = threadIdx.x, lane = tid & 63;
  const int wid = __builtin_amdgcn_readfirstlane(tid >> 6);
  const int wm = wid / WN, wn = wid % WN;
  const int tiles_m = cdiv(M, BM), tiles_n = cdiv(N, BN);
  const int t = xcd_remap(blockIdx.x, tiles_m * tiles_n);
  int tm, tn;
  if (tiles_n <= tiles_m) {
    tn = t % tiles_n;
    tm = t / tiles_n;
  } else {
    tm = t % tiles_m;
    tn = t / tiles_m;
  }
  const int m0 = tm * BM, n0 = tn * BN;
  const int nk = K / PK;

  typename P::SA sa;
  typename P::SBt sb;
  sa.init(A, lda, M, m0, a_bytes, wid, lane);
  sb.init(B, ldb, N, n0, b_bytes, wid, lane);
  f32x4 acc[TM][TN];
#pragma unroll
  for (int i = 0; i < TM; ++i)
#pragma unroll
    for (int j = 0; j < TN; ++j) acc[i][j] = f32x4{0.f, 0.f, 0.f, 0.f};

  const int abase = wm * WTM, bbase = wn * WTN;
#pragma unroll
  for (int s = 0; s < NS - 1; ++s)
    if (s < nk) P::stage(sa, sb, smem, s, wid);
  wait_tiles<PT, NS - 2>(min(NS - 1, nk) - 1);
  __builtin_amdgcn_s_barrier();
  typename P::FA fa[TM];
  typename P::FBt fb[TN], fbn[TN];
#pragma unroll
  for (int j = 0; j < TN; ++j) {
    lgkm_wait<15 - P::FBt::NI>();
    fb[j].read(smem + A_BYTES, bbase + 16 * j, lane);
  }
#pragma unroll
  for (int i = 0; i < TM; ++i) {
    lgkm_wait<15 - P::FA::NI>();
    fa[i].read(smem, abase + 16 * i, lane);
  }

  if (NS - 1 < nk) P::stage(sa, sb, smem, NS - 1, wid);
  int kt = 0;
  if (nk > 0) P::ktile(kt++, nk, fb, fbn, fa, acc, sa, sb, smem, lane, wid, abase, bbase);
  for (; kt + 1 <= nk - NS; kt += 2) {
    P::ktile_s(kt, nk, fbn, fb, fa, acc, sa, sb, smem, lane, wid, abase, bbase);
    P::ktile_s(kt + 1, nk, fb, fbn, fa, acc, sa, sb, smem, lane, wid, abase, bbase);
  }
  for (; kt + 1 < nk; kt += 2) {
    P::ktile(kt, nk, fbn, fb, fa, acc, sa, sb, smem, lane, wid, abase, bbase);
    P::ktile(kt + 1, nk, fb, fbn, fa, acc, sa, sb, smem, lane, wid, abase, bbase);
  }
  if (kt < nk) P::ktile(kt, nk, fbn, fb, fa, acc, sa, sb, smem, lane, wid, abase, bbase);

  lgkm_wait<0>();
  wait_vmcnt<0>();
  lds_barrier();
  {
    using OutT = typename std::conditional<OUT_F32, float, bf16_t>::type;
    (void)sizeof(OutT);
    constexpr int RPASS = OUT_F32 ? (WTM < 32 ? WTM : 32) : (WTM > 64 ? 64 : WTM);
    using Epi = EpiLds<EPI, OUT_F32, TM, TN, RPASS>;
    static_assert(NW * Epi::BYTES <= NS * SB, "epilogue images fit in the stages");
    Epi::run(smem + wid * Epi::BYTES, acc, lane, Cv, ldc, M, N, m0 + wm * WTM, n0 + wn * WTN, alpha,
             beta, bias, aux, ldaux, epi_vec_ok<EPI, OUT_F32>(Cv, ldc, aux, ldaux));
  }
}

}
```

tensorflow_distributed_on_gke_amd/models/layers.py:

```python
from __future__ import annotations

import math
import os
from dataclasses import dataclass, field
from typing import Optional

import torch

from tensorflow_distributed_on_gke_amd.models.params import Param, ParamStore
from tensorflow_distributed_on_gke_amd.ops import kernels as K
from tensorflow_distributed_on_gke_amd.ops import fp8, philox

LN_EPS = 1e-6
RAGGED_WGRAD = True


@dataclass
class RunCtx:

    training: bool = False
    dropout: float = 0.1
    seed: int = 0
    ctr: Optional[torch.Tensor] = None
    accumulate: bool = False
    store: Optional[ParamStore] = None
    attn_maps: Optional[dict] = None
    fp8: Optional[object] = None
    wgrad: Optional["WgradQueue"] = None
    emb_csr: Optional[dict] = None

    @property
    def p(self) -> float:
        return self.dropout if self.training else 0.0

    def cpu_offset(self, site: int) -> int:
        if self.ctr is None:
            return site
        return philox.rng_offset(int(self.ctr.item()), site)


@dataclass
class KVGrad:

    buf: Optional[torch.Tensor] = None
    dec_len: int = 0
    heads: int = 0
    f8b: bool = False
    buf8: Optional[torch.Tensor] = None
    part: Optional[torch.Tensor] = None
    wkv: Optional["Param"] = None


def _dgrad_res(dy2: torch.Tensor, w: Param, N: int, dres: Optional[torch.Tensor]) -> torch.Tensor:
    if dres is None:
        return K.linear_dgrad(dy2, w.compute, N)
    return _dgrad_into(dy2, w, N, dres)


def _keep_scale(rt: RunCtx, site: int, shape, device) -> Optional[torch.Tensor]:
    p = rt.p
    if p <= 0:
        return None
    n = math.prod(shape)
    keep = philox.keep_mask(rt.seed, rt.cpu_offset(site), n, p).view(shape)
    return keep.to(torch.float32).to(device) / (1.0 - p)


def _beta(rt: RunCtx) -> float:
    return 1.0 if rt.accumulate else 0.0


def _ready(rt: RunCtx, *params: Param) -> None:
    if rt.store is not None:
        for p in params:
            rt.store.grad_ready(p)


def _write_grad(p: Param, g: torch.Tensor, rt: RunCtx) -> None:
    if rt.accumulate:
        p.grad.add_(g.to(p.grad.dtype))
    else:
        p.grad.copy_(g.to(p.grad.dtype))


class WgradQueue:

    def __init__(self, flush_at_boundary: bool = False, wave_tiles: int = 0):
        self.items = []
        self.flush_at_boundary = flush_at_boundary
        self.wave_tiles = wave_tiles
        self.layers_per_step = 0
        self._layer_ends = 0
        self._cursor = 0
        self.reductions = []
        self.reduced_params = []
        self.fp8_items = []
        self.small_per_shape = False

    def boundary(self) -> None:
        if self.flush_at_boundary and not self._chunking() and (self.items or self.reductions or self.fp8_items):
            self.flush()

    @staticmethod
    def _tiles(it) -> int:
        dy2, x2, N = it[0], it[1], it[2]
        return -(-N // 256) * -(-x2.shape[1] // 256)

    @staticmethod
    def _ragged_ok(it) -> bool:
        dy2, x2 = it[0], it[1]
        return x2.shape[0] % 64 == 0 and dy2.stride(0) % 8 == 0 and x2.stride(0) % 8 == 0

    def _chunking(self) -> bool:
        return bool(self.wave_tiles) and RAGGED_WGRAD

    def layer_end(self) -> None:
        self._layer_ends += 1
        last = self.layers_per_step > 0 and self._layer_ends >= self.layers_per_step
        if self._chunking() and self.fp8_items:
            self._flush_fp8()
        if not self._chunking() or not self.items:
            return
        if last or not all(self._ragged_ok(it) for it in self.items):
            self.flush()
            return
        queued = sum(self._tiles(it) for it in self.items) - self._cursor
        n = queued // self.wave_tiles * self.wave_tiles
        if n:
            self._launch_prefix(n)
            self._finish_flush()

    def add(self, dy2, x2, N, w: Param, b: Optional[Param], beta: float, rt: "RunCtx"):
        self.items.append((dy2, x2, N, w, b, beta, rt))

    def add_fp8(self, dy8, sa, x8, sb, w: Param, beta: float, rt: "RunCtx"):
        self.fp8_items.append((dy8, sa, x8, sb, w, beta, rt))

    def _flush_fp8(self) -> None:
        if not self.fp8_items:
            return
        by_beta = {}
        for it in self.fp8_items:
            by_beta.setdefault(it[5], []).append(it)
        for beta, its in by_beta.items():
            its.sort(key=lambda it: (it[4].shape, it[0].stride(0), it[2].stride(0)))
            fp8.wgrad_fp8([it[0] for it in its], [it[1] for it in its], [it[2] for it in its],
                          [it[3] for it in its], [it[4].grad for it in its], beta)
        for it in self.fp8_items:
            _ready(it[6], it[4])
        self.fp8_items = []

    def step_done(self) -> None:
        self._layer_ends = 0

    def flush(self) -> None:
        self._flush_fp8()
        if self.items:
            if RAGGED_WGRAD and all(self._ragged_ok(it) for it in self.items) and (
                    not self.small_per_shape or self._cursor
                    or sum(self._tiles(it) for it in self.items) >= K.NUM_CU // 2):
                self._launch_prefix(sum(self._tiles(it) for it in self.items) - self._cursor)
            else:
                self._flush_grouped()
                self._flush_bias()
                self._done = self.items
                self.items = []
        else:
            self._done = []
        self._finish_flush()

    def _finish_flush(self) -> None:
        if self.reductions:
            K.reduce_partials_multi(self.reductions)
        done = getattr(self, "_done", [])
        for dy2, x2, N, w, b, beta, rt in done:
            _ready(rt, w, *([b] if b is not None else []))
        for rt, p in self.reduced_params:
            _ready(rt, p)
        rts = [it[6] for it in done] + [rp[0] for rp in self.reduced_params]
        if rts and rts[0].store is not None:
            rts[0].store.grad_sync()
        self._done = []
        self.reductions = []
        self.reduced_params = []

    def _launch_prefix(self, n: int) -> None:
        sel = []
        done = []
        left = n
        while left > 0 and self.items:
            it = self.items[0]
            avail = self._tiles(it) - self._cursor
            take = min(avail, left)
            sel.append((it, self._cursor, take))
            left -= take
            if take == avail:
                done.append(self.items.pop(0))
                self._cursor = 0
            else:
                self._cursor += take
        self._done = done
        runs = {}
        for it, first, cnt in sel:
            dy2, x2, N, w, b, beta, rt = it
            full = first == 0 and cnt == self._tiles(it)
            key = (N, x2.shape[1], dy2.stride(0), x2.stride(0)) if full else ("cut", id(it), first)
            runs.setdefault((x2.shape[0], beta), {}).setdefault(key, []).append((it, first, cnt))
        for (_, beta), by_shape in runs.items():
            groups = list(by_shape.values())
            for s0 in range(0, len(groups), K.RAGGED_MAX_SHAPES):
                chunk = [e for grp in groups[s0:s0 + K.RAGGED_MAX_SHAPES] for e in grp]
                for c0 in range(0, len(chunk), K.RAGGED_MAX_PROBLEMS):
                    part = chunk[c0:c0 + K.RAGGED_MAX_PROBLEMS]
                    K.wgrad_ragged([e[0][0] for e in part], [e[0][1] for e in part],
                                   [e[0][3].grad for e in part], beta,
                                   [e[0][4].grad if e[0][4] is not None else None for e in part],
                                   ranges=[(e[1], e[2]) for e in part])

    def _flush_grouped(self) -> None:
        groups = {}
        for it in self.items:
            dy2, x2, N, w, b, beta, rt = it
            key = (tuple(dy2.shape), dy2.stride(0), tuple(x2.shape), x2.stride(0), N, beta)
            groups.setdefault(key, []).append(it)
        for key, items in groups.items():
            for c0 in range(0, len(items), 32):
                chunk = items[c0:c0 + 32]
                beta = chunk[0][5]
                if len(chunk) == 1:
                    dy2, x2, N, w, *_ = chunk[0]
                    K.linear_wgrad(dy2, x2, N, w.grad, beta)
                else:
                    K.wgrad_grouped([i[0] for i in chunk], [i[1] for i in chunk],
                                    [i[3].grad for i in chunk], beta)

    def _flush_bias(self) -> None:
        bgroups = {}
        for dy2, x2, N, w, b, beta, rt in self.items:
            if b is not None:
                bgroups.setdefault((tuple(dy2.shape), dy2.stride(0), N, beta), []).append((dy2, b))
        for (shape, ld, N, beta), items in bgroups.items():
            for c0 in range(0, len(items), 32):
                chunk = items[c0:c0 + 32]
                if len(chunk) == 1:
                    K.colsum(chunk[0][0], N, chunk[0][1].grad, beta)
                else:
                    K.colsum_grouped([i[0] for i in chunk], [i[1].grad for i in chunk], beta)


def _wgrad(rt: RunCtx, dy2, x2, N: int, w: Param, b: Optional[Param] = None) -> None:
    bt = _beta(rt)
    if rt.wgrad is not None:
        rt.wgrad.add(dy2, x2, N, w, b, bt, rt)
        return
    K.linear_wgrad(dy2, x2, N, w.grad, bt)
    if b is not None:
        K.colsum(dy2, N, b.grad, bt)
    _ready(rt, w, *([b] if b is not None else []))


def _attn_lean(rt: RunCtx, M: int, w_in: Param, w_out: Optional[Param], d: int) -> bool:
    st = rt.fp8
    return (st is not None and rt.training and rt.wgrad is not None and fp8.ATTN_PROJ_FP8
            and id(w_in) in st.proj_bwd and (w_out is None or id(w_out) in st.attn_out)
            and fp8.wgrad_fp8_ok(M, d, d))


def _fp8_grad_bias(g: torch.Tensor, g_slot: int, b: Param, rt: RunCtx, key: str):
    st = rt.fp8
    g8, part, nparts = fp8.quantize_colsum(g, st.gmeta, g_slot, key)
    q = rt.wgrad
    q.reductions.append((part, b.grad, nparts, g.shape[1], _beta(rt)))
    q.reduced_params.append((rt, b))
    return g8


def _fold_bias_later(rt: RunCtx, part: torch.Tensor, nparts: int, N: int, b: Param) -> None:
    q = rt.wgrad
    q.reductions.append((part, b.grad, nparts, N, _beta(rt)))
    q.reduced_params.append((rt, b))


def _fp8_dgrad_into(g8, g_slot: int, w: Param, out: torch.Tensor, rt: RunCtx, beta: float) -> None:
    st = rt.fp8
    wt8, swt = st.weights.get(w, transposed=not fp8.DGRAD_PLAIN_W)
    fp8.gemm_bf8_dgrad(g8, st.gmeta, g_slot, wt8, st.meta, swt, out, beta=beta,
                       w_plain=fp8.DGRAD_PLAIN_W)


def _fp8_dgrad8(g8, g_slot: int, w: Param, out_slot: int, rt: RunCtx) -> torch.Tensor:
    st = rt.fp8
    wt8, swt = st.weights.get(w, transposed=not fp8.DGRAD_PLAIN_W)
    return fp8.gemm_bf8_dgrad(g8, st.gmeta, g_slot, wt8, st.meta, swt, None, out8_slot=out_slot,
                              w_plain=fp8.DGRAD_PLAIN_W)


def _f8_bwd_planned(rt: RunCtx, lean: bool, Lq: int, Lk: int, hd: int) -> bool:
    return (lean and fp8.ATTN_BWD_F8 and rt.attn_maps is None and K.attn_bwd_f8_ok(Lq, Lk, hd))


def _attn_f8_bwd(ctx, Lq: int, Lk: int, hd: int) -> bool:
    return getattr(ctx, "f8b", False) and getattr(ctx, "q8", None) is not None


def _proj_ln_fwd(a2, w: Param, b: Param, x, gamma: Param, beta: Param, site: int, rt: RunCtx):
    s = K.linear_fwd(a2, w.compute, b.master)
    return _ln_fwd(x, s.view(x.shape), gamma, beta, site, rt)


LN_KEEP_BITS = os.environ.get("TDG_LN_KEEP_BITS", "1") != "0"


def _kbits(rt: RunCtx, x: torch.Tensor) -> Optional[torch.Tensor]:
    D = x.shape[-1]
    if LN_KEEP_BITS and x.is_cuda and rt.training and rt.p > 0 and D % 512 == 0:
        return torch.empty(x.numel() // D, D // 8, dtype=torch.uint8, device=x.device)
    return None


def _ln_fwd(x, s, gamma: Param, beta: Param, site: int, rt: RunCtx):
    if x.is_cuda:
        y8 = s8 = a8 = None
        slot = rt.fp8.ln_slots.get(id(gamma)) if rt.fp8 is not None else None
        if slot is not None:
            y8 = torch.empty(x.shape, dtype=fp8.FP8, device=x.device)
            s8, a8 = rt.fp8.meta.s(slot), rt.fp8.meta.a(slot)
            rt.fp8.stash[slot] = y8
        kbits = _kbits(rt, x)
        y, h, mean, rstd = K.ln_fwd(x.contiguous(), s.contiguous(), gamma.master, beta.master,
                                    rt.p, rt.seed, rt.ctr, site, y8=y8, s8=s8, amax8=a8, kbits=kbits)
        return y, (h, mean, rstd, None, kbits)
    ks = _keep_scale(rt, site, s.shape, s.device)
    h = x + (s * ks if ks is not None else s)
    mean = h.mean(-1, keepdim=True)
    rstd = torch.rsqrt(((h - mean) ** 2).mean(-1, keepdim=True) + LN_EPS)
    return (h - mean) * rstd * gamma.master + beta.master, (h, mean, rstd, ks, None)


def _ln_bwd(dy, saved, gamma: Param, beta: Param, sub_bias: Param, site: int, rt: RunCtx,
            ds8_slot: Optional[int] = None):
    h, mean, rstd, ks = saved[:4]
    if dy.is_cuda:
        q = rt.wgrad
        ds8 = s8 = a8 = None
        if ds8_slot is not None:
            gm = rt.fp8.gmeta
            ds8 = torch.empty(dy.shape, dtype=gm.dtype, device=dy.device)
            s8, a8 = gm.s(ds8_slot), gm.a(ds8_slot)
        dh, ds = K.ln_bwd(dy.contiguous(), h, mean, rstd, gamma.master, gamma.grad, beta.grad,
                          sub_bias.grad, rt.p, rt.seed, rt.ctr, site, want_ds=ds8 is None,
                          accumulate=rt.accumulate, defer=q.reductions if q is not None else None,
                          ds8=ds8, s8=s8, amax8=a8, kbits=saved[4])
        if ds8 is not None:
            ds = ds8
        if q is not None:
            q.reduced_params += [(rt, gamma), (rt, beta), (rt, sub_bias)]
            return dh, ds
    else:
        xhat = (h - mean) * rstd
        D = h.shape[-1]
        g = dy * gamma.master
        dh = rstd * (g - g.mean(-1, keepdim=True) - xhat * (g * xhat).mean(-1, keepdim=True))
        ds = dh * ks if ks is not None else dh
        _write_grad(gamma, (dy * xhat).reshape(-1, D).sum(0), rt)
        _write_grad(beta, dy.reshape(-1, D).sum(0), rt)
        _write_grad(sub_bias, ds.reshape(-1, D).sum(0), rt)
    _ready(rt, gamma, beta, sub_bias)
    return dh, ds


def _dgrad_into(dy2: torch.Tensor, w: Param, N: int, dx: torch.Tensor) -> torch.Tensor:
    if dy2.is_cuda:
        return K.linear_dgrad(dy2, w.compute, N, out=dx.view(dy2.shape[0], -1), beta=1.0)
    dx.view(dy2.shape[0], -1).add_(dy2 @ w.master)
    return dx


class EmbedFn(torch.autograd.Function):
    @staticmethod
    def forward(ctx, anchor, tok, table: Param, pe: torch.Tensor, site: int, rt: RunCtx):
        d = table.shape[1]
        scale = math.sqrt(d)
        ctx.table, ctx.site, ctx.rt, ctx.scale = table, site, rt, scale
        ctx.save_for_backward(tok)
        if tok.is_cuda:
            ctx.kbits = None
            ctx.csr = rt.emb_csr.get(site) if rt.emb_csr else None
            if ctx.csr is not None and rt.p > 0 and d % 512 == 0:
                ctx.kbits = torch.empty(tok.numel(), d // 8, dtype=torch.uint8, device=tok.device)
            return K.embed_fwd(tok, table.compute, pe, scale, rt.p, rt.seed, rt.ctr, site,
                               kbits=ctx.kbits)
        B, L = tok.shape
        x = table.master[tok] * scale + pe[:L].unsqueeze(0)
        ks = _keep_scale(rt, site, x.shape, x.device)
        ctx.ks = ks
        return x * ks if ks is not None else x

    @staticmethod
    def backward(ctx, dout):
        (tok,) = ctx.saved_tensors
        table, rt = ctx.table, ctx.rt
        if dout.is_cuda:
            dc = dout.contiguous()
            K.embed_bwd(tok, dc, table.grad, ctx.scale, rt.p, rt.seed, rt.ctr, ctx.site,
                        accumulate=rt.accumulate, kbits=ctx.kbits, csr=ctx.csr)
            _ready(rt, table)
            return None, None, None, None, None, None
        else:
            g = dout * ctx.ks if ctx.ks is not None else dout
            g = (g * ctx.scale).reshape(-1, table.shape[1])
            table.grad.index_add_(0, tok.reshape(-1), g.to(table.grad.dtype))
        _ready(rt, table)
        return None, None, None, None, None, None


def _ref_attn_fwd(q, k, v, kv_len, causal, scale):
    s = torch.einsum("bqhd,bkhd->bhqk", q, k) * scale
    B, H, Lq, Lk = s.shape
    mask = torch.zeros(B, 1, Lq, Lk, dtype=s.dtype, device=s.device)
    keys = torch.arange(Lk, device=s.device)
    if kv_len is not None:
        mask = mask + (keys.view(1, 1, 1, Lk) >= kv_len.view(B, 1, 1, 1).to(keys.device)).to(s.dtype)
    if causal:
        qs = torch.arange(Lq, device=s.device)
        mask = torch.maximum(mask, (keys.view(1, Lk) > qs.view(Lq, 1)).to(s.dtype).view(1, 1, Lq, Lk))
    p = torch.softmax(s + mask * -1e9, dim=-1)
    out = torch.einsum("bhqk,bkhd->bqhd", p, v)
    return out, p


def _ref_attn_bwd(q, k, v, p, dout, scale):
    dv = torch.einsum("bhqk,bqhd->bkhd", p, dout)
    dp = torch.einsum("bqhd,bkhd->bhqk", dout, v)
    ds = p * (dp - (dp * p).sum(-1, keepdim=True))
    dq = torch.einsum("bhqk,bkhd->bqhd", ds, k) * scale
    dk = torch.einsum("bhqk,bqhd->bkhd", ds, q) * scale
    return dq, dk, dv


def attention_probs(q, k, kv_len, causal: bool, scale: float) -> torch.Tensor:
    if q.is_cuda:
        return K.attn_probs(q, k, kv_len, scale, causal)
    return _ref_attn_fwd(q, k, k, kv_len, causal, scale)[1]


class SelfAttnBlockFn(torch.autograd.Function):
    @staticmethod
    def forward(ctx, x, wqkv: Param, bqkv: Param, wo: Param, bo: Param, gamma: Param,
                beta: Param, heads: int, kv_len, causal: bool, site: int, rt: RunCtx):
        B, L, d = x.shape
        hd = d // heads
        scale = 1.0 / math.sqrt(hd)
        ctx.p = (wqkv, bqkv, wo, bo, gamma, beta)
        ctx.meta = (heads, causal, scale, site, rt)
        x2 = x.reshape(B * L, d)
        ctx.lean = lean = x.is_cuda and _attn_lean(rt, B * L, wqkv, wo, d)
        kx = [] if lean else None
        if x.is_cuda:
            f8 = rt.fp8 is not None and K.attn_fwd_fp8_ok(L, L, hd)
            ctx.f8b = f8 and _f8_bwd_planned(rt, lean, L, L, hd)
            r = (rt.fp8.linear(x2, wqkv, bqkv, want8=f8, keep_x8=kx, want_y=not ctx.f8b)
                 if rt.fp8 is not None else None)
            qkv, qkv8 = (r[0], r[1]) if f8 and r is not None else (r, None)
            fused = None
            if qkv is None and not ctx.f8b and rt.fp8 is None and rt.attn_maps is None:
                fused = K.qkv_attn_fwd(x2, wqkv.compute, bqkv.master, B, heads, kv_len, scale, causal)
                if fused is not None:
                    qkv = fused[0]
            if qkv is None and not ctx.f8b:
                qkv = K.linear_fwd(x2, wqkv.compute, bqkv.master)
            q5 = qkv.view(B, L, 3, heads, hd) if qkv is not None else None
            o8e = None
            ctx.q8 = None
            if fused is not None:
                o, aux = fused[1], fused[2]
            elif qkv8 is not None:
                q85 = qkv8.view(B, L, 3, heads, hd)
                s8 = rt.fp8.meta.s(r[2])
                ctx.q8 = (qkv8, r[2])
                o8e = rt.fp8.o8_for(wo, (B, L, heads, hd), x.device) if lean else None
                o, aux = K.attn_fwd_fp8(q85[:, :, 0], q85[:, :, 1], q85[:, :, 2], s8, s8, s8, kv_len,
                                        scale, causal, *(o8e or ()))
            else:
                o, aux = K.attn_fwd(q5[:, :, 0], q5[:, :, 1], q5[:, :, 2], kv_len, scale, causal)
            s = None
        else:
            qkv = x2 @ wqkv.master.t() + bqkv.master
            q5 = qkv.view(B, L, 3, heads, hd)
            o, aux = _ref_attn_fwd(q5[:, :, 0], q5[:, :, 1], q5[:, :, 2], kv_len, causal, scale)
            s = o.reshape(B * L, d) @ wo.master.t() + bo.master
        if rt.attn_maps is not None:
            rt.attn_maps[site] = attention_probs(q5[:, :, 0], q5[:, :, 1], kv_len, causal, scale)
        ctx.f8a = None
        if lean:
            s, o8 = rt.fp8.out_proj(o.view(B * L, d), wo, bo, o8e[0] if o8e else None)
            ctx.f8a = (kx[0], kx[1], o8)
            y, ctx.ln = _ln_fwd(x, s.view(B, L, d), gamma, beta, site, rt)
        elif s is None:
            y, ctx.ln = _proj_ln_fwd(o.view(B * L, d), wo, bo, x, gamma, beta, site, rt)
        else:
            y, ctx.ln = _ln_fwd(x, s.view(B, L, d), gamma, beta, site, rt)
        ctx.save_for_backward(x2, qkv, o, aux, kv_len)
        return y

    @staticmethod
    def backward(ctx, dy):
        wqkv, bqkv, wo, bo, gamma, beta = ctx.p
        heads, causal, scale, site, rt = ctx.meta
        x2, qkv, o, aux, kv_len = ctx.saved_tensors
        B, L, d = dy.shape
        M = B * L
        hd = d // heads
        bt = _beta(rt)
        if ctx.lean:
            return SelfAttnBlockFn._backward_fp8(ctx, dy)
        dh, ds = _ln_bwd(dy, ctx.ln, gamma, beta, bo, site, rt)
        ds2 = ds.reshape(M, d)
        q5 = qkv.view(B, L, 3, heads, hd)
        if dy.is_cuda:
            _wgrad(rt, ds2, o.view(M, d), d, wo)
            dqkv = torch.empty(M, 3 * d, dtype=torch.bfloat16, device=dy.device)
            g5 = dqkv.view(B, L, 3, heads, hd)
            if not K.attn_bwd_fdo(q5[:, :, 0], q5[:, :, 1], q5[:, :, 2], o, ds2, wo.compute, aux,
                                  g5[:, :, 0], g5[:, :, 1], g5[:, :, 2], kv_len, scale, causal):
                do = K.linear_dgrad(ds2, wo.compute, d)
                K.attn_bwd(q5[:, :, 0], q5[:, :, 1], q5[:, :, 2], o, do.view(B, L, heads, hd), aux,
                           g5[:, :, 0], g5[:, :, 1], g5[:, :, 2], kv_len, scale, causal)
            _wgrad(rt, dqkv, x2, 3 * d, wqkv, bqkv)
            dx = _dgrad_res(dqkv, wqkv, 3 * d, dh)
            if rt.wgrad is not None:
                rt.wgrad.layer_end()
            return (dx.view(B, L, d),) + (None,) * 11
        else:
            _write_grad(wo, ds2.t() @ o.reshape(M, d), rt)
            _ready(rt, wo)
            do = (ds2 @ wo.master).view(B, L, heads, hd)
            dq, dk, dv = _ref_attn_bwd(q5[:, :, 0], q5[:, :, 1], q5[:, :, 2], aux, do, scale)
            dqkv = torch.stack([dq, dk, dv], dim=2).reshape(M, 3 * d)
            _write_grad(wqkv, dqkv.t() @ x2, rt)
            _write_grad(bqkv, dqkv.sum(0), rt)
        _ready(rt, wqkv, bqkv)
        dx = _dgrad_into(dqkv, wqkv, 3 * d, dh)
        return (dx.view(B, L, d),) + (None,) * 11

    @staticmethod
    def _backward_fp8(ctx, dy):
        wqkv, bqkv, wo, bo, gamma, beta = ctx.p
        heads, causal, scale, site, rt = ctx.meta
        x2, qkv, o, aux, kv_len = ctx.saved_tensors
        B, L, d = dy.shape
        M, hd, bt = B * L, d // heads, _beta(rt)
        st = rt.fp8
        x8, xs, o8 = ctx.f8a
        os_, go = st.attn_out[id(wo)]
        dh, ds8 = _ln_bwd(dy, ctx.ln, gamma, beta, bo, site, rt, ds8_slot=go)
        ds8 = ds8.view(M, d)
        gq = st.proj_bwd[id(wqkv)]
        if _attn_f8_bwd(ctx, L, L, hd):
            gdo, gds = st.attn_bwd8[id(wo)]
            do8 = _fp8_dgrad8(ds8, go, wo, gdo, rt)
            qkv8, qs = ctx.q8
            q85 = qkv8.view(B, L, 3, heads, hd)
            s8 = st.meta.s(qs)
            dqkv8 = torch.empty(M, 3 * d, dtype=st.gmeta.dtype, device=dy.device)
            g85 = dqkv8.view(B, L, 3, heads, hd)
            part = K.workspace(f"f8cs_qkv{site}", B * 3 * d, dy.device)
            nparts = K.attn_bwd_f8(q85[:, :, 0], q85[:, :, 1], q85[:, :, 2], s8, s8, s8, o,
                                   do8.view(B, L, heads, hd), st.gmeta.s(gdo), aux, kv_len, scale,
                                   causal, st.gmeta.s(gds), st.gmeta.a(gds), dq8=g85[:, :, 0],
                                   dk8=g85[:, :, 1], dv8=g85[:, :, 2], sg8=st.gmeta.s(gq),
                                   amaxg8=st.gmeta.a(gq), cs_part=part, cs_ld=3 * d, cs_q=0,
                                   cs_k=d, cs_v=2 * d)
            _fold_bias_later(rt, part[: nparts * 3 * d], nparts, 3 * d, bqkv)
            return SelfAttnBlockFn._finish_fp8(ctx, rt, st, dh, ds8, go, dqkv8, gq, x8, xs, o8, os_,
                                               M, d, B, L, bt)
        do = torch.empty(M, d, dtype=torch.bfloat16, device=dy.device)
        _fp8_dgrad_into(ds8, go, wo, do, rt, 0.0)
        q5 = qkv.view(B, L, 3, heads, hd)
        dqkv = torch.empty(M, 3 * d, dtype=torch.bfloat16, device=dy.device)
        g5 = dqkv.view(B, L, 3, heads, hd)
        if fp8.ATTN_BWD_G8 and K.attn_bwd_g8_ok(L, L, hd):
            dqkv8 = torch.empty(M, 3 * d, dtype=st.gmeta.dtype, device=dy.device)
            g85 = dqkv8.view(B, L, 3, heads, hd)
            part = K.workspace(f"qcs_qkv{site}", B * -(-L // 128) * 3 * d, dy.device)
            nparts = K.attn_bwd_g8(q5[:, :, 0], q5[:, :, 1], q5[:, :, 2], o, do.view(B, L, heads, hd),
                                   aux, g5[:, :, 0], g5[:, :, 1], g5[:, :, 2], kv_len, scale, causal,
                                   g85[:, :, 0], g85[:, :, 1], g85[:, :, 2], st.gmeta.s(gq),
                                   st.gmeta.a(gq), part, 3 * d, 0, d, 2 * d)
            _fold_bias_later(rt, part[: nparts * 3 * d], nparts, 3 * d, bqkv)
        else:
            K.attn_bwd(q5[:, :, 0], q5[:, :, 1], q5[:, :, 2], o, do.view(B, L, heads, hd), aux,
                       g5[:, :, 0], g5[:, :, 1], g5[:, :, 2], kv_len, scale, causal)
            dqkv8 = _fp8_grad_bias(dqkv, gq, bqkv, rt, f"qkv{site}")
        return SelfAttnBlockFn._finish_fp8(ctx, rt, st, dh, ds8, go, dqkv8, gq, x8, xs, o8, os_, M,
                                           d, B, L, bt)

    @staticmethod
    def _finish_fp8(ctx, rt, st, dh, ds8, go, dqkv8, gq, x8, xs, o8, os_, M, d, B, L, bt):
        wqkv, bqkv, wo = ctx.p[0], ctx.p[1], ctx.p[2]
        _fp8_dgrad_into(dqkv8, gq, wqkv, dh.view(M, d), rt, 1.0)
        q = rt.wgrad
        q.add_fp8(ds8, st.gmeta.s(go), o8, st.meta.s(os_), wo, bt, rt)
        q.add_fp8(dqkv8, st.gmeta.s(gq), x8, st.meta.s(xs), wqkv, bt, rt)
        q.layer_end()
        return (dh.view(B, L, d),) + (None,) * 11


def _take_dkv(dkv_in, kvh: KVGrad, rows: int) -> torch.Tensor:
    dkv = (dkv_in if dkv_in is not None else kvh.buf).reshape(rows, -1)
    kvh.buf = None
    return dkv


class CrossKVFn(torch.autograd.Function):

    @staticmethod
    def forward(ctx, enc, wkv: Param, bkv: Param, kvh: KVGrad, rt: RunCtx):
        B, S, d = enc.shape
        e2 = enc.reshape(B * S, d)
        ctx.p = (wkv, bkv)
        ctx.kvh, ctx.rt, ctx.shape = kvh, rt, (B, S, d)
        ctx.save_for_backward(e2)
        ctx.lean = lean = enc.is_cuda and _attn_lean(rt, B * S, wkv, None, d)
        kx = [] if lean else None
        ctx.f8a = None
        T = kvh.dec_len
        hd = d // kvh.heads if kvh.heads else 0
        kvh.f8b = bool(lean and enc.is_cuda and T and K.attn_fwd_fp8_ok(T, S, hd)
                       and fp8.wgrad_fp8_ok(B * T, d, d) and _f8_bwd_planned(rt, True, T, S, hd))
        if enc.is_cuda:
            kv = None
            if rt.fp8 is not None:
                r = rt.fp8.linear(e2.contiguous(), wkv, bkv, want8=True, keep_x8=kx, want_y=not kvh.f8b)
                if lean and r is not None:
                    ctx.f8a = tuple(kx)
                if r is not None:
                    kv = r[0]
                    rt.fp8.kv8 = (r[1].view(B, S, -1), r[2])
                    if kvh.f8b:
                        kv = torch.zeros(1, dtype=torch.bfloat16, device=enc.device).expand(
                            B * S, r[1].shape[1])
            if kv is None:
                kv = K.linear_fwd(e2.contiguous(), wkv.compute, bkv.master)
        else:
            kv = e2 @ wkv.master.t() + bkv.master
        return kv.view(B, S, -1)

    @staticmethod
    def backward(ctx, dkv_in):
        wkv, bkv = ctx.p
        rt = ctx.rt
        B, S, d = ctx.shape
        (e2,) = ctx.saved_tensors
        kvh = ctx.kvh
        N = wkv.shape[0]
        bt = _beta(rt)
        if e2.is_cuda and ctx.f8a is not None:
            st = rt.fp8
            x8, xs = ctx.f8a
            gk = st.proj_bwd[id(wkv)]
            if kvh.f8b:
                dkv8 = kvh.buf8.reshape(B * S, -1)
                _fold_bias_later(rt, kvh.part, B, N, bkv)
                kvh.buf8 = kvh.part = None
            else:
                dkv8 = _fp8_grad_bias(_take_dkv(dkv_in, kvh, B * S).contiguous(), gk, bkv, rt, "kv")
            rt.wgrad.add_fp8(dkv8, st.gmeta.s(gk), x8, st.meta.s(xs), wkv, bt, rt)
            rt.wgrad.boundary()
            denc = torch.empty(B * S, d, dtype=torch.bfloat16, device=e2.device)
            _fp8_dgrad_into(dkv8, gk, wkv, denc, rt, 0.0)
            if rt.store is not None:
                rt.store.release_point()
            return denc.view(B, S, d), None, None, None, None
        dkv = _take_dkv(dkv_in, kvh, B * S)
        if e2.is_cuda:
            _wgrad(rt, dkv, e2, N, wkv, bkv)
            if rt.wgrad is not None:
                rt.wgrad.boundary()
            denc = _dgrad_res(dkv, wkv, N, None)
        else:
            _write_grad(wkv, dkv.t() @ e2, rt)
            _write_grad(bkv, dkv.sum(0), rt)
            _ready(rt, wkv, bkv)
            denc = dkv @ wkv.master
        if rt.store is not None:
            rt.store.release_point()
        return denc.view(B, S, d), None, None, None, None


class CrossAttnBlockFn(torch.autograd.Function):

    @staticmethod
    def forward(ctx, x, kv_all, layer: int, kvh: KVGrad, wq: Param, bq: Param, wo: Param,
                bo: Param, gamma: Param, beta: Param, heads: int, kv_len, site: int, rt: RunCtx):
        B, T, d = x.shape
        S = kv_all.shape[1]
        hd = d // heads
        scale = 1.0 / math.sqrt(hd)
        ctx.p = (wq, bq, wo, bo, gamma, beta)
        ctx.meta = (heads, scale, site, rt, layer, kvh)
        x2 = x.reshape(B * T, d)
        kv5 = None
        if not kvh.f8b:
            if not kv_all.is_contiguous():
                raise ValueError("kv_all must be contiguous")
            kv5 = kv_all[:, :, layer * 2 * d:(layer + 1) * 2 * d].view(B, S, 2, heads, hd)
        ctx.lean = lean = x.is_cuda and _attn_lean(rt, B * T, wq, wo, d)
        kx = [] if lean else None
        if x.is_cuda:
            o8e = None
            f8 = (rt.fp8 is not None and rt.fp8.kv8 is not None and K.attn_fwd_fp8_ok(T, S, hd))
            ctx.f8b = f8 and _f8_bwd_planned(rt, lean, T, S, hd)
            if kvh.f8b and not ctx.f8b:
                raise RuntimeError("cross-attention: the batched K|V were produced for the fp8 "
                                   "backward (no bf16 copy) but this layer does not run it")
            r = (rt.fp8.linear(x2, wq, bq, want8=f8, keep_x8=kx, want_y=not ctx.f8b)
                 if rt.fp8 is not None else None)
            q, q8 = (r[0], r[1]) if f8 and r is not None else (r, None)
            fused = None
            if q is None and not ctx.f8b and rt.fp8 is None and rt.attn_maps is None and kv5 is not None:
                fused = K.qkv_attn_fwd(x2, wq.compute, bq.master, B, heads, kv_len, scale, False,
                                       k=kv5[:, :, 0], v=kv5[:, :, 1])
                if fused is not None:
                    q = fused[0]
            if q is None and not ctx.f8b:
                q = K.linear_fwd(x2, wq.compute, bq.master)
            ctx.q8 = None
            if fused is not None:
                o, aux = fused[1], fused[2]
            elif q8 is not None:
                kv8, kvs = rt.fp8.kv8
                if kv8.shape != kv_all.shape:
                    raise RuntimeError(f"fp8 cross K|V {tuple(kv8.shape)} is not this forward's "
                                       f"{tuple(kv_all.shape)}")
                kv85 = kv8[:, :, layer * 2 * d:(layer + 1) * 2 * d].view(B, S, 2, heads, hd)
                skv = rt.fp8.meta.s(kvs)
                ctx.q8 = (q8, r[2], kv85, kvs)
                o8e = rt.fp8.o8_for(wo, (B, T, heads, hd), x.device) if lean else None
                o, aux = K.attn_fwd_fp8(q8.view(B, T, heads, hd), kv85[:, :, 0], kv85[:, :, 1],
                                        rt.fp8.meta.s(r[2]), skv, skv, kv_len, scale, False,
                                        *(o8e or ()))
            else:
                o, aux = K.attn_fwd(q.view(B, T, heads, hd), kv5[:, :, 0], kv5[:, :, 1], kv_len,
                                    scale, False)
            s = None
        else:
            q = x2 @ wq.master.t() + bq.master
            o, aux = _ref_attn_fwd(q.view(B, T, heads, hd), kv5[:, :, 0], kv5[:, :, 1], kv_len,
                                   False, scale)
            s = o.reshape(B * T, d) @ wo.master.t() + bo.master
        if rt.attn_maps is not None:
            rt.attn_maps[site] = attention_probs(q.view(B, T, heads, hd), kv5[:, :, 0], kv_len, False, scale)
        ctx.f8a = None
        if lean:
            s, o8 = rt.fp8.out_proj(o.view(B * T, d), wo, bo, o8e[0] if o8e else None)
            ctx.f8a = (kx[0], kx[1], o8)
            y, ctx.ln = _ln_fwd(x, s.view(B, T, d), gamma, beta, site, rt)
        elif s is None:
            y, ctx.ln = _proj_ln_fwd(o.view(B * T, d), wo, bo, x, gamma, beta, site, rt)
        else:
            y, ctx.ln = _ln_fwd(x, s.view(B, T, d), gamma, beta, site, rt)
        ctx.save_for_backward(x2, kv_all, q, o, aux, kv_len)
        return y

    @staticmethod
    def backward(ctx, dy):
        wq, bq, wo, bo, gamma, beta = ctx.p
        heads, scale, site, rt, layer, kvh = ctx.meta
        x2, kv_all, q, o, aux, kv_len = ctx.saved_tensors
        B, T, d = dy.shape
        S = kv_all.shape[1]
        hd = d // heads
        bt = _beta(rt)
        M = B * T
        if kvh.f8b:
            dkv_all = kv5 = g5 = None
        else:
            if kvh.buf is None:
                kvh.buf = torch.empty(B * S, kv_all.shape[2], dtype=kv_all.dtype, device=dy.device)
            dkv_all = kvh.buf.view(B, S, -1)
            kv5 = kv_all[:, :, layer * 2 * d:(layer + 1) * 2 * d].view(B, S, 2, heads, hd)
            g5 = dkv_all[:, :, layer * 2 * d:(layer + 1) * 2 * d].view(B, S, 2, heads, hd)
        if ctx.lean:
            st = rt.fp8
            x8, xs, o8 = ctx.f8a
            os_, go = st.attn_out[id(wo)]
            dh, ds8 = _ln_bwd(dy, ctx.ln, gamma, beta, bo, site, rt, ds8_slot=go)
            ds8 = ds8.view(M, d)
            gq = st.proj_bwd[id(wq)]
            if _attn_f8_bwd(ctx, T, S, hd):
                gdo, gds = st.attn_bwd8[id(wo)]
                do8 = _fp8_dgrad8(ds8, go, wo, gdo, rt)
                q8, qs, kv85, kvs = ctx.q8
                skv = st.meta.s(kvs)
                dq8 = torch.empty(M, d, dtype=st.gmeta.dtype, device=dy.device)
                part = K.workspace(f"f8cs_q{site}", B * d, dy.device)
                if kvh.f8b:
                    NKV = kv_all.shape[2]
                    if kvh.buf8 is None:
                        kvh.buf8 = torch.empty(B, S, NKV, dtype=st.gmeta.dtype, device=dy.device)
                        kvh.part = torch.empty(B, NKV, dtype=torch.float32, device=dy.device)
                    g85 = kvh.buf8[:, :, layer * 2 * d:(layer + 1) * 2 * d].view(B, S, 2, heads, hd)
                    gk = st.proj_bwd[id(kvh.wkv)]
                    kvo = dict(dk8=g85[:, :, 0], dv8=g85[:, :, 1], sgkv8=st.gmeta.s(gk),
                               amaxgkv8=st.gmeta.a(gk), cs_part2=kvh.part, cs_ld2=NKV,
                               cs_k=layer * 2 * d, cs_v=layer * 2 * d + d)
                else:
                    kvo = dict(dk=g5[:, :, 0], dv=g5[:, :, 1])
                nparts = K.attn_bwd_f8(q8.view(B, T, heads, hd), kv85[:, :, 0], kv85[:, :, 1],
                                       st.meta.s(qs), skv, skv, o, do8.view(B, T, heads, hd),
                                       st.gmeta.s(gdo), aux, kv_len, scale, False, st.gmeta.s(gds),
                                       st.gmeta.a(gds), dq8=dq8.view(B, T, heads, hd),
                                       sg8=st.gmeta.s(gq), amaxg8=st.gmeta.a(gq), cs_part=part,
                                       cs_ld=d, cs_q=0, **kvo)
                _fold_bias_later(rt, part[: nparts * d], nparts, d, bq)
                _fp8_dgrad_into(dq8, gq, wq, dh.view(M, d), rt, 1.0)
                rt.wgrad.add_fp8(ds8, st.gmeta.s(go), o8, st.meta.s(os_), wo, bt, rt)
                rt.wgrad.add_fp8(dq8, st.gmeta.s(gq), x8, st.meta.s(xs), wq, bt, rt)
                dkv_ret = None
                if layer == 0:
                    dkv_ret = dkv_all if dkv_all is not None else torch.zeros(
                        1, dtype=kv_all.dtype, device=dy.device).expand(kv_all.shape)
                return (dh.view(B, T, d), dkv_ret) + (None,) * 12
            do = torch.empty(M, d, dtype=torch.bfloat16, device=dy.device)
            _fp8_dgrad_into(ds8, go, wo, do, rt, 0.0)
            dq = torch.empty(M, d, dtype=torch.bfloat16, device=dy.device)
            if fp8.ATTN_BWD_G8 and K.attn_bwd_g8_ok(T, S, hd):
                dq8 = torch.empty(M, d, dtype=st.gmeta.dtype, device=dy.device)
                part = K.workspace(f"qcs_q{site}", B * -(-T // 128) * d, dy.device)
                nparts = K.attn_bwd_g8(q.view(B, T, heads, hd), kv5[:, :, 0], kv5[:, :, 1], o,
                                       do.view(B, T, heads, hd), aux, dq.view(B, T, heads, hd),
                                       g5[:, :, 0], g5[:, :, 1], kv_len, scale, False,
                                       dq8.view(B, T, heads, hd), None, None, st.gmeta.s(gq),
                                       st.gmeta.a(gq), part, d, 0, 0, 0, skip_bf16=False)
                _fold_bias_later(rt, part[: nparts * d], nparts, d, bq)
            else:
                K.attn_bwd(q.view(B, T, heads, hd), kv5[:, :, 0], kv5[:, :, 1], o,
                           do.view(B, T, heads, hd), aux, dq.view(B, T, heads, hd), g5[:, :, 0],
                           g5[:, :, 1], kv_len, scale, False)
                dq8 = _fp8_grad_bias(dq, gq, bq, rt, f"q{site}")
            _fp8_dgrad_into(dq8, gq, wq, dh.view(M, d), rt, 1.0)
            rt.wgrad.add_fp8(ds8, st.gmeta.s(go), o8, st.meta.s(os_), wo, bt, rt)
            rt.wgrad.add_fp8(dq8, st.gmeta.s(gq), x8, st.meta.s(xs), wq, bt, rt)
            dkv_ret = dkv_all if layer == 0 else None
            return (dh.view(B, T, d), dkv_ret) + (None,) * 12
        dh, ds = _ln_bwd(dy, ctx.ln, gamma, beta, bo, site, rt)
        ds2 = ds.reshape(M, d)
        if dy.is_cuda:
            _wgrad(rt, ds2, o.view(M, d), d, wo)
            dq = torch.empty(M, d, dtype=torch.bfloat16, device=dy.device)
            if not K.attn_bwd_fdo(q.view(B, T, heads, hd), kv5[:, :, 0], kv5[:, :, 1], o, ds2,
                                  wo.compute, aux, dq.view(B, T, heads, hd), g5[:, :, 0],
                                  g5[:, :, 1], kv_len, scale, False):
                do = K.linear_dgrad(ds2, wo.compute, d)
                K.attn_bwd(q.view(B, T, heads, hd), kv5[:, :, 0], kv5[:, :, 1], o,
                           do.view(B, T, heads, hd), aux, dq.view(B, T, heads, hd), g5[:, :, 0],
                           g5[:, :, 1], kv_len, scale, False)
            _wgrad(rt, dq, x2, d, wq, bq)
        else:
            _write_grad(wo, ds2.t() @ o.reshape(M, d), rt)
            _ready(rt, wo)
            do = (ds2 @ wo.master).view(B, T, heads, hd)
            dqh, dk, dv = _ref_attn_bwd(q.view(B, T, heads, hd), kv5[:, :, 0], kv5[:, :, 1], aux,
                                        do, scale)
            g5[:, :, 0] = dk
            g5[:, :, 1] = dv
            dq = dqh.reshape(M, d)
            _write_grad(wq, dq.t() @ x2, rt)
            _write_grad(bq, dq.sum(0), rt)
            _ready(rt, wq, bq)
        dx = _dgrad_res(dq, wq, d, dh)
        dkv_ret = dkv_all if layer == 0 else None
        return (dx.view(B, T, d), dkv_ret) + (None,) * 12


class FFNBlockFn(torch.autograd.Function):

    @staticmethod
    def forward(ctx, x, w1: Param, b1: Param, w2: Param, b2: Param, gamma: Param, beta: Param,
                site: int, rt: RunCtx):
        B, L, d = x.shape
        x2 = x.reshape(B * L, d)
        ctx.p = (w1, b1, w2, b2, gamma, beta)
        ctx.meta = (site, rt)
        ctx.f8 = None
        ctx.lean = False
        if x.is_cuda and rt.fp8 is not None:
            st = rt.fp8
            xs, hs = st.ffn_slots[id(w1)]
            w1_8, s1 = st.weights.get(w1)
            w2_8, s2 = st.weights.get(w2)
            x8 = st.stash.pop(xs, None)
            if x8 is None:
                x8 = fp8.quantize(x2, st.meta, xs)
            x8 = x8.view(x2.shape)
            lean = (rt.training and rt.wgrad is not None and fp8.WGRAD_FP8
                    and st.ffn_bwd_slots.get(id(w1)) is not None
                    and fp8.wgrad_fp8_ok(B * L, d, w1.shape[0]))
            h, h8 = fp8.gemm_fp8(x8, w1_8, b1.master, st.meta, xs, s1, relu=True, out8_slot=hs,
                                 want_y=not lean)
            f, _ = fp8.gemm_fp8(h8, w2_8, b2.master, st.meta, hs, s2)
            ctx.f8 = (x8, h8) if rt.training else None
            ctx.lean = lean
        elif x.is_cuda:
            h = K.linear_fwd(x2, w1.compute, b1.master, relu=True)
            f = None
        else:
            h = torch.relu(x2 @ w1.master.t() + b1.master)
            f = h @ w2.master.t() + b2.master
        if f is None:
            y, ctx.ln = _proj_ln_fwd(h, w2, b2, x, gamma, beta, site, rt)
        else:
            y, ctx.ln = _ln_fwd(x, f.view(B, L, d), gamma, beta, site, rt)
        ctx.save_for_backward(x2, h if h is not None else x2)
        return y

    @staticmethod
    def backward(ctx, dy):
        w1, b1, w2, b2, gamma, beta = ctx.p
        site, rt = ctx.meta
        x2, h = ctx.saved_tensors
        B, L, d = dy.shape
        ff = w1.shape[0]
        bt = _beta(rt)
        f8w = ctx.lean
        bw = rt.fp8.ffn_bwd_slots.get(id(w1)) if (dy.is_cuda and rt.fp8 is not None) else None
        dh, ds = _ln_bwd(dy, ctx.ln, gamma, beta, b2, site, rt, ds8_slot=bw[0] if f8w else None)
        ds2 = ds.reshape(B * L, d)
        if dy.is_cuda:
            if not f8w:
                _wgrad(rt, ds2, h, d, w2)
            if bw is not None:
                st = rt.fp8
                gs, gh = bw
                M = B * L
                ds8 = ds2 if f8w else fp8.quantize(ds2, st.gmeta, gs)
                wp = fp8.DGRAD_PLAIN_W
                w2t8, s2t = st.weights.get(w2, transposed=not wp)
                w1t8, s1t = st.weights.get(w1, transposed=not wp)
                if f8w:
                    x8, h8 = ctx.f8
                    xs, hs = st.ffn_slots[id(w1)]
                    q = rt.wgrad
                    dpre8 = fp8.gemm_bf8_dgrad(ds8, st.gmeta, gs, w2t8, st.meta, s2t, None,
                                               relu_aux8=h8.view(M, ff), out8_slot=gh,
                                               colsum_out=b1.grad, colsum_beta=bt, w_plain=wp,
                                               defer=q.reductions)
                    q.reduced_params.append((rt, b1))
                    q.add_fp8(ds8.view(M, d), st.gmeta.s(gs), h8.view(M, ff), st.meta.s(hs), w2, bt, rt)
                    q.add_fp8(dpre8.view(M, ff), st.gmeta.s(gh), x8.view(M, d), st.meta.s(xs), w1, bt, rt)
                else:
                    dpre = torch.empty(M, ff, dtype=ds2.dtype, device=ds2.device)
                    dpre8 = fp8.gemm_bf8_dgrad(ds8, st.gmeta, gs, w2t8, st.meta, s2t, dpre, relu_aux=h,
                                               out8_slot=gh, w_plain=wp)
                    _wgrad(rt, dpre, x2, ff, w1, b1)
                fp8.gemm_bf8_dgrad(dpre8, st.gmeta, gh, w1t8, st.meta, s1t, dh.view(M, d), beta=1.0,
                                   w_plain=wp)
                return (dh.view(B, L, d),) + (None,) * 8
            if w2.compute_t is not None and not w2.compute_t_stale:
                dpre = K.linear_dgrad_t(ds2, w2.compute_t, relu_aux=h)
            else:
                dpre = K.linear_dgrad(ds2, w2.compute, d, relu_aux=h)
            _wgrad(rt, dpre, x2, ff, w1, b1)
            dx = _dgrad_res(dpre, w1, ff, dh)
            return (dx.view(B, L, d),) + (None,) * 8
        else:
            _write_grad(w2, ds2.t() @ h, rt)
            _ready(rt, w2)
            dpre = (ds2 @ w2.master) * (h > 0).to(ds2.dtype)
            _write_grad(w1, dpre.t() @ x2, rt)
            _write_grad(b1, dpre.sum(0), rt)
        _ready(rt, w1, b1)
        dx = _dgrad_into(dpre, w1, ff, dh)
        return (dx.view(B, L, d),) + (None,) * 8
```

tensorflow_distributed_on_gke_amd/ops/kernels.py:

```python
from __future__ import annotations

import math
import os
from typing import Dict, List, Optional, Tuple

import torch

from tensorflow_distributed_on_gke_amd.ops._ext import C

EPI_NONE, EPI_BIAS, EPI_BIAS_RELU, EPI_DRELU = 0, 1, 2, 3
NUM_CU = 256

_WS: Dict[Tuple[int, int, str], torch.Tensor] = {}
_WS_RETIRED: List[torch.Tensor] = []


def workspace(name: str, numel: int, device, dtype=torch.float32, zero: bool = False) -> torch.Tensor:
    dev = torch.device(device)
    sid = torch.cuda.current_stream(dev).stream_id if dev.type == "cuda" else 0
    key = (dev.index or 0, sid, name)
    t = _WS.get(key)
    if t is None or t.numel() < numel or t.dtype != dtype:
        if t is not None:
            _WS_RETIRED.append(t)
        t = (torch.zeros if zero else torch.empty)(max(numel, 1), dtype=dtype, device=dev)
        _WS[key] = t
    return t


def reset_workspace() -> None:
    _WS.clear()
    _WS_RETIRED.clear()


_TILES = {0: (128, 128), 1: (128, 64), 2: (64, 128), 3: (64, 64), 4: (128, 128), 5: (256, 128),
          6: (128, 256), 7: (64, 128), 8: (64, 64), 9: (256, 128), 10: (128, 256), 11: (128, 128),
          12: (256, 256), 13: (128, 128), 14: (128, 128),
          20: (256, 256), 21: (256, 128), 22: (128, 256)}
_CFG_OVERRIDE: Dict[Tuple[int, int, int, bool, bool], Tuple[int, int]] = {}


def set_gemm_config(M: int, N: int, K: int, a_kc: bool, b_kc: bool, cfg: int, splits: int) -> None:
    _CFG_OVERRIDE[(M, N, K, a_kc, b_kc)] = (cfg, splits)


def choose_gemm(M: int, N: int, K: int, a_kc: bool = True, b_kc: bool = True) -> Tuple[int, int]:
    o = _CFG_OVERRIDE.get((M, N, K, a_kc, b_kc))
    if o is not None:
        return o
    if not a_kc and not b_kc:
        t128 = math.ceil(M / 128) * math.ceil(N / 128)
        splits = 1
        while t128 * splits < NUM_CU and K // (splits * 2) >= 512:
            splits *= 2
        return 0, splits
    if K % 64 == 0 and math.ceil(M / 256) * math.ceil(N / 256) >= 192:
        return 12, 1
    if a_kc and not b_kc and N >= 1024 and math.ceil(M / 128) * math.ceil(N / 256) >= NUM_CU:
        return 6, 1
    return (13, 1) if not b_kc else (4, 1)


_TUNED: Dict[tuple, Tuple[int, int]] = {}
AUTOTUNE = os.environ.get("TDG_GEMM_AUTOTUNE", "0") == "1"
_CANDIDATES = [(0, 1), (4, 1), (5, 1), (6, 1), (9, 1), (10, 1), (12, 1), (13, 1), (14, 1),
               (20, 1), (21, 1), (22, 1)]


def _autotune(key, run) -> Tuple[int, int]:
    M, N, K, a_kc, b_kc = key[:5]
    cands = list(_CANDIDATES)
    if not a_kc and not b_kc:
        cands = [(c, s) for c in (0, 7, 8) for s in (1, 2, 4, 8) if K // s >= 256] + [(12, 1)]
    times: Dict[Tuple[int, int], float] = {}
    for rnd in range(2):
        for cfg in cands:
            if rnd and cfg not in times:
                continue
            try:
                run(cfg)
                ev = [torch.cuda.Event(enable_timing=True) for _ in range(2)]
                ev[0].record()
                for _ in range(5):
                    run(cfg)
                ev[1].record()
                ev[1].synchronize()
                t = ev[0].elapsed_time(ev[1])
            except RuntimeError:
                continue
            times[cfg] = min(t, times.get(cfg, float("inf")))
    return min(times, key=times.get)


def _key_str(k: tuple) -> str:
    M, N, K, a_kc, b_kc, epi, dt, ld8, beta = k
    return f"{M},{N},{K},{int(a_kc)},{int(b_kc)},{epi},{str(dt).replace('torch.', '')},{int(ld8)},{int(beta)}"


def save_tuned(path: str) -> None:
    import json

    with open(path, "w") as f:
        json.dump({_key_str(k): list(v[0]) for k, v in sorted(_TUNED.items(), key=lambda kv: str(kv[0]))},
                  f, indent=0)


def load_tuned(path: str) -> int:
    import json

    if not os.path.exists(path):
        return 0
    with open(path) as f:
        data = json.load(f)
    for ks, v in data.items():
        M, N, K, a, b, epi, dt, ld8, beta = ks.split(",")
        key = (int(M), int(N), int(K), bool(int(a)), bool(int(b)), int(epi), getattr(torch, dt),
               bool(int(ld8)), bool(int(beta)))
        cfg = (int(v[0]), int(v[1]))
        _TUNED[key] = (cfg, cfg)
    return len(data)


TUNED_FILE = os.environ.get("TDG_GEMM_TUNED_FILE") or os.path.join(
    os.path.dirname(os.path.abspath(__file__)), "gemm_tuned_gfx950.json")
load_tuned(TUNED_FILE)


def _tok_bucket(v: int) -> int:
    return -(-v // 1024) * 1024


def gemm(A, B, Cout, M, N, K, lda, ldb, ldc, a_kc, b_kc, epi=EPI_NONE, bias=None, aux=None,
         ldaux=0, alpha=1.0, beta=0.0, cfg: Optional[Tuple[int, int]] = None) -> torch.Tensor:

    def run(c, out=Cout):
        tile, splits = c
        ws = workspace("splitk", splits * M * ldc, A.device) if splits > 1 else None
        C().gemm(A, B, out, bias, aux, M, N, K, lda, ldb, ldc, ldaux, a_kc, b_kc, epi, alpha,
                 beta, tile, splits, ws)

    if cfg is None:
        Mk, Kk = (M, _tok_bucket(K)) if (not a_kc and not b_kc) else (_tok_bucket(M), K)
        key = (Mk, N, Kk, a_kc, b_kc, epi, Cout.dtype, ldc % 8 == 0, beta != 0.0)
        ent = _TUNED.get(key)
        if ent is None:
            o = _CFG_OVERRIDE.get((M, N, K, a_kc, b_kc))
            if o is not None:
                ent = (o, o)
        if ent is None and AUTOTUNE and A.is_cuda and not torch.cuda.is_current_stream_capturing():
            if beta != 0.0:
                scratch = workspace("tune_c", Cout.numel(), A.device, Cout.dtype)[: Cout.numel()]
                scratch = scratch.view_as(Cout)
                best = _autotune(key, lambda c: run(c, scratch))
            else:
                best = _autotune(key, run)
            ent = (best, best)
            _TUNED[key] = ent
        if ent is None:
            cfg = choose_gemm(M, N, K, a_kc, b_kc)
        else:
            cfg = ent[0]
    run(cfg)
    return Cout


def tuned_table() -> Dict[str, str]:
    return {f"{k[0]}x{k[1]}x{k[2]} a_kc={k[3]} b_kc={k[4]} epi={k[5]}": f"cfg{v[0]} split{v[1]}"
            for k, v in _TUNED.items()}


def linear_fwd(x2: torch.Tensor, w: torch.Tensor, bias: Optional[torch.Tensor], relu: bool = False,
               out: Optional[torch.Tensor] = None, ldc: Optional[int] = None) -> torch.Tensor:
    M, K = x2.shape
    N = w.shape[0]
    ldc = ldc or N
    if out is None:
        out = torch.empty(M, ldc, dtype=torch.bfloat16, device=x2.device)
    epi = EPI_BIAS_RELU if relu else (EPI_BIAS if bias is not None else EPI_NONE)
    return gemm(x2, w, out, M, N, K, x2.stride(0), w.stride(0), ldc, True, True, epi, bias=bias)


def linear_dgrad(dy2: torch.Tensor, w: torch.Tensor, N: int, relu_aux: Optional[torch.Tensor] = None,
                 out: Optional[torch.Tensor] = None, beta: float = 0.0) -> torch.Tensor:
    M = dy2.shape[0]
    K = w.shape[1]
    if out is None:
        out = torch.empty(M, K, dtype=torch.bfloat16, device=dy2.device)
    epi = EPI_DRELU if relu_aux is not None else EPI_NONE
    return gemm(dy2, w, out, M, K, N, dy2.stride(0), w.stride(0), out.stride(0), True, False, epi,
                aux=relu_aux, ldaux=(relu_aux.stride(0) if relu_aux is not None else 0), beta=beta)


def transpose_grouped(srcs, dsts) -> None:
    for c0 in range(0, len(srcs), 64):
        C().transpose_grouped(list(srcs[c0:c0 + 64]), list(dsts[c0:c0 + 64]))


def linear_dgrad_t(dy2: torch.Tensor, w_t: torch.Tensor, relu_aux: Optional[torch.Tensor] = None,
                   out: Optional[torch.Tensor] = None) -> torch.Tensor:
    M, K = dy2.shape
    N = w_t.shape[0]
    if out is None:
        out = torch.empty(M, N, dtype=torch.bfloat16, device=dy2.device)
    epi = EPI_DRELU if relu_aux is not None else EPI_NONE
    return gemm(dy2, w_t, out, M, N, K, dy2.stride(0), w_t.stride(0), out.stride(0), True, True, epi,
                aux=relu_aux, ldaux=(relu_aux.stride(0) if relu_aux is not None else 0))


def linear_wgrad(dy2: torch.Tensor, x2: torch.Tensor, N: int, dw: torch.Tensor,
                 beta: float = 0.0) -> torch.Tensor:
    M, K = x2.shape
    return gemm(dy2, x2, dw, N, K, M, dy2.stride(0), x2.stride(0), dw.stride(0), False, False,
                EPI_NONE, beta=beta)


_GROUP_TUNED: Dict[tuple, int] = {}
_GROUP_CANDS = (0, 4, 5, 6, 7, 8, 2, 12)


def wgrad_grouped(dys, xs, dws, beta: float = 0.0) -> None:
    M, K = xs[0].shape
    N = dws[0].shape[0]
    lda, ldb, ldc = dys[0].stride(0), xs[0].stride(0), dws[0].stride(0)

    def run(c):
        C().gemm_grouped(dys, xs, dws, N, K, M, lda, ldb, ldc, False, False, 1.0, beta, c)

    key = (M, N, K, len(dys), lda, ldb, beta != 0.0)
    cfg = _GROUP_TUNED.get(key)
    if cfg is None:
        if AUTOTUNE and not torch.cuda.is_current_stream_capturing():
            scratch = [workspace(f"gw{i}", d.numel(), d.device)[: d.numel()].view_as(d)
                       for i, d in enumerate(dws)]

            def trial(c):
                C().gemm_grouped(dys, xs, scratch, N, K, M, lda, ldb, ldc, False, False, 1.0, 0.0, c)

            times: Dict[int, float] = {}
            for _ in range(2):
                for c in _GROUP_CANDS:
                    try:
                        trial(c)
                        e0, e1 = torch.cuda.Event(enable_timing=True), torch.cuda.Event(enable_timing=True)
                        e0.record()
                        for _ in range(3):
                            trial(c)
                        e1.record()
                        e1.synchronize()
                        times[c] = min(times.get(c, float("inf")), e0.elapsed_time(e1))
                    except RuntimeError:
                        continue
            if not times:
                run(0)
            cfg = min(times, key=times.get)
        else:
            cfg = 0
        _GROUP_TUNED[key] = cfg
    run(cfg)


RAGGED_MAX_PROBLEMS, RAGGED_MAX_SHAPES = 64, 8


def wgrad_ragged(dys, xs, dws, beta: float = 0.0, biases=None, ranges=None) -> None:
    M = xs[0].shape[0]
    shapes = []
    for i, (dy, x, dw) in enumerate(zip(dys, xs, dws)):
        if x.shape[0] != M or dy.shape[0] != M:
            raise ValueError("wgrad_ragged: all problems must share the token count")
        r = ranges[i] if ranges is not None else None
        shapes += [dw.shape[0], x.shape[1], dy.stride(0), x.stride(0), dw.stride(0)]
        shapes += [0, -1] if r is None else [int(r[0]), int(r[1])]
    C().gemm_ragged(list(dys), list(xs), list(dws), shapes, M, False, False, 1.0, beta,
                    list(biases) if biases is not None else [])


def colsum_grouped(xs, outs, beta: float = 0.0) -> None:
    M, N = xs[0].shape[0], outs[0].numel()
    rpb = 256
    part = workspace("colsum_g", len(xs) * math.ceil(M / rpb) * N, xs[0].device)
    C().colsum_grouped(xs, outs, part, M, N, xs[0].stride(0), rpb, beta)


def colsum(x2: torch.Tensor, N: int, out: torch.Tensor, beta: float = 0.0) -> torch.Tensor:
    M = x2.shape[0]
    rpb = 128
    part = workspace("colsum", math.ceil(M / rpb) * N, x2.device)
    C().colsum(x2, out, part, M, N, x2.stride(0), rpb, beta)
    return out


def attn_fwd(q, k, v, kv_len, scale: float, causal: bool):
    B, Lq, H, hd = q.shape
    out = torch.empty(B, Lq, H, hd, dtype=torch.bfloat16, device=q.device)
    lse = torch.empty(B, H, Lq, dtype=torch.float32, device=q.device)
    C().attn_fwd(q, k, v, out, lse, kv_len, scale, causal)
    return out, lse


QKV_ATTN = os.environ.get("TDG_QKV_ATTN", "1") != "0"


def qkv_attn_fwd(x2, w, bias, B: int, heads: int, kv_len, scale: float, causal: bool,
                 k=None, v=None):
    M, d = x2.shape
    L, hd = M // B, d // heads
    if not QKV_ATTN or L > 128 or hd != 64 or (k is not None and k.shape[1] > 128):
        return None
    np_ = 1 if k is not None else 3
    qkv = torch.empty(M, np_ * d, dtype=torch.bfloat16, device=x2.device)
    out = torch.empty(B, L, heads, hd, dtype=torch.bfloat16, device=x2.device)
    lse = torch.empty(B, heads, L, dtype=torch.float32, device=x2.device)
    if not C().qkv_attn_fwd(x2, w, bias, qkv, out, lse, kv_len, scale, causal, B, heads, k, v):
        return None
    return qkv, out, lse


def attn_fwd_fp8_ok(Lq: int, Lk: int, hd: int) -> bool:
    return hd == 64 and Lq > 128


def attn_fwd_fp8(q8, k8, v8, sq, sk, sv, kv_len, scale: float, causal: bool, o8=None, so8=None,
                 amax8=None):
    B, Lq, H, hd = q8.shape
    out = torch.empty(B, Lq, H, hd, dtype=torch.bfloat16, device=q8.device)
    lse = torch.empty(B, H, Lq, dtype=torch.float32, device=q8.device)
    C().attn_fwd_fp8(q8, k8, v8, out, lse, kv_len, sq, sk, sv, scale, causal, o8, so8, amax8)
    return out, lse


def attn_bwd(q, k, v, o, dout, lse, dq, dk, dv, kv_len, scale: float, causal: bool):
    delta = workspace("attn_delta", lse.numel(), q.device)[: lse.numel()]
    C().attn_bwd(q, k, v, o, dout, lse, delta, dq, dk, dv, kv_len, scale, causal)


ATTN_BWD_FDO = os.environ.get("TDG_ATTN_BWD_FDO", "1") != "0"


def attn_bwd_fdo(q, k, v, o, dy2, wo, lse, dq, dk, dv, kv_len, scale: float, causal: bool) -> bool:
    if not ATTN_BWD_FDO:
        return False
    delta = workspace("attn_delta", lse.numel(), q.device)[: lse.numel()]
    return C().attn_bwd_fdo(q, k, v, o, dy2, wo, lse, delta, dq, dk, dv, kv_len, scale, causal)


def attn_bwd_g8_ok(Lq: int, Lk: int, hd: int) -> bool:
    return hd == 64 and (Lq > 128 or Lk > 128)


def attn_bwd_g8(q, k, v, o, dout, lse, dq, dk, dv, kv_len, scale: float, causal: bool, dq8,
                dk8, dv8, sg8, amax8, cs_part, cs_ld: int, cs_q: int, cs_k: int, cs_v: int,
                skip_bf16: Optional[bool] = None) -> int:
    if skip_bf16 is None:
        skip_bf16 = dk8 is not None
    B, Lq = q.shape[0], q.shape[1]
    np_ = -(-Lq // 128)
    delta = workspace("attn_delta", lse.numel(), q.device)[: lse.numel()]
    C().attn_bwd_g8(q, k, v, o, dout, lse, delta, dq, dk, dv, kv_len, scale, causal, dq8, dk8, dv8,
                    sg8, amax8, cs_part, np_, cs_ld, cs_q, cs_k, cs_v, skip_bf16)
    return B * np_


def attn_bwd_f8_ok(Lq: int, Lk: int, hd: int) -> bool:
    return hd == 64 and 128 < Lq <= 512 and Lk <= 512


def attn_bwd_f8(q8, k8, v8, sq, sk, sv, o, do8, sdo, lse, kv_len, scale: float, causal: bool,
                sds, amaxds, dq=None, dk=None, dv=None, dq8=None, dk8=None, dv8=None, sg8=None,
                amaxg8=None, cs_part=None, cs_ld: int = 0, cs_q: int = 0, cs_k: int = 0,
                cs_v: int = 0, sgkv8=None, amaxgkv8=None, cs_part2=None, cs_ld2: int = 0) -> int:
    C().attn_bwd_f8(q8, k8, v8, sq, sk, sv, o, do8, sdo, lse, kv_len, scale, causal, sds, amaxds,
                    dq, dk, dv, dq8, dk8, dv8, sg8, amaxg8, cs_part, cs_ld, cs_q, cs_k, cs_v, sgkv8,
                    amaxgkv8, cs_part2, cs_ld2)
    return q8.shape[0]


def attn_probs(q, k, kv_len, scale: float, causal: bool) -> torch.Tensor:
    B, Lq, H, hd = q.shape
    Lk = k.shape[1]
    probs = torch.empty(B, H, Lq, Lk, dtype=torch.float32, device=q.device)
    C().attn_probs(q, k, probs, kv_len, scale, causal)
    return probs


def ln_fwd(x, s, gamma, beta, p, seed, ctr, site, eps=1e-6, save=True, y8=None, s8=None,
           amax8=None, kbits=None):
    D = x.shape[-1]
    M = x.numel() // D
    y = torch.empty_like(x)
    h = torch.empty_like(x) if save else None
    mean = torch.empty(M, dtype=torch.float32, device=x.device) if save else None
    rstd = torch.empty(M, dtype=torch.float32, device=x.device) if save else None
    C().ln_fwd(x, s, gamma, beta, y, h, mean, rstd, p, seed, ctr, site, eps, y8, s8, amax8, kbits)
    return y, h, mean, rstd


LN_BWD_RPB = int(os.environ.get("TDG_LN_BWD_RPB", "0") or 0)


def ln_bwd_rpb(D: int) -> int:
    return LN_BWD_RPB or (32 if D <= 512 else 16)


def ln_bwd_nparts(M: int, D: int) -> int:
    return math.ceil(M / ln_bwd_rpb(D))


def ln_bwd(dy, h, mean, rstd, gamma, dgamma, dbeta, dbias, p, seed, ctr, site, want_ds=True,
           dres=None, accumulate=False, defer=None, ds8=None, s8=None, amax8=None, kbits=None):
    D = dy.shape[-1]
    M = dy.numel() // D
    dh = torch.empty_like(dy)
    need_ds = (want_ds and (p > 0 or dres is not None)) or (dbias is not None and ds8 is None)
    ds = torch.empty_like(dy) if need_ds else None
    if defer is None:
        ws = workspace("ln_bwd", 3 * ln_bwd_nparts(M, D) * D, dy.device)
    else:
        ws = workspace(f"ln_bwd_part_{site}", 3 * ln_bwd_nparts(M, D) * D, dy.device)
    C().ln_bwd(dy, h, mean, rstd, gamma, dh, ds, dres, dgamma, dbeta, dbias, ws, p, seed, ctr, site,
               accumulate, defer is not None, ln_bwd_rpb(D), ds8, s8, amax8, kbits)
    if defer is not None:
        nb = ln_bwd_nparts(M, D)
        outs = [dgamma, dbeta] + ([dbias] if dbias is not None else [])
        for i, o in enumerate(outs):
            defer.append((ws[i * nb * D:(i + 1) * nb * D], o, nb, D, 1.0 if accumulate else 0.0))
    if ds is None:
        ds = dh
    return dh, ds


def reduce_partials_multi(items) -> None:
    groups = {}
    for part, out, nparts, N, beta in items:
        groups.setdefault((N, beta), []).append((part, out, nparts))
    for (N, beta), its in groups.items():
        for c0 in range(0, len(its), 96):
            ch = its[c0:c0 + 96]
            C().reduce_partials_multi([i[0] for i in ch], [i[1] for i in ch], [i[2] for i in ch],
                                      N, beta)


def embed_fwd(tok, table, pe, scale, p, seed, ctr, site, kbits=None):
    B, L = tok.shape
    D = table.shape[1]
    out = torch.empty(B, L, D, dtype=torch.bfloat16, device=tok.device)
    C().embed_fwd(tok, table, pe, out, scale, p, seed, ctr, site, kbits)
    return out


DETERMINISTIC_EMBED = os.environ.get("TDG_DETERMINISTIC", "1") != "0"


EMBED_CSR = os.environ.get("TDG_EMBED_CSR", "1") != "0"


class EmbCsr:

    def __init__(self, tok: torch.Tensor, V: int, name: str):
        self.tok, self.V, self.M = tok, int(V), tok.numel()
        n32, _ = C().embed_csr_ws(self.M, self.V, 128)
        self.w32 = workspace("embed_csr32_" + name, n32, tok.device, torch.int32)


def embed_csr_ok(M: int, V: int) -> bool:
    return DETERMINISTIC_EMBED and EMBED_CSR and C().embed_csr_ok(M, V)


def embed_csr_sort(tables, stamps=None) -> list:
    cs = [EmbCsr(t.contiguous(), V, name) for t, V, name in tables]
    C().embed_csr_sort([c.tok for c in cs], [c.V for c in cs], [c.w32 for c in cs], stamps)
    return cs


def embed_csr_apply(cs: EmbCsr, dout, dtable, scale, p, seed, ctr, site, accumulate=False,
                    kbits=None) -> None:
    _, n64 = C().embed_csr_ws(cs.M, cs.V, dtable.shape[1])
    w64 = workspace("embed_csr64", n64, dtable.device, torch.int64)
    C().embed_csr_apply(dout, dtable, cs.w32, w64, cs.M, scale, p, seed, ctr, site, accumulate, kbits)


def embed_bwd(tok, dout, dtable, scale, p, seed, ctr, site, accumulate=False, kbits=None,
              csr: Optional[EmbCsr] = None):
    if csr is not None or embed_csr_ok(tok.numel(), dtable.shape[0]):
        if csr is None:
            csr = embed_csr_sort([(tok, dtable.shape[0], "bwd")])[0]
        embed_csr_apply(csr, dout.contiguous(), dtable, scale, p, seed, ctr, site, accumulate, kbits)
        return
    if DETERMINISTIC_EMBED:
        acc = workspace("embed_fx", dtable.numel(), dtable.device, torch.int64, zero=True)
        C().embed_bwd_det(tok, dout, dtable, acc, scale, p, seed, ctr, site, accumulate)
    else:
        C().embed_bwd(tok, dout, dtable, scale, p, seed, ctr, site)


def count_tokens(labels, out):
    C().count_tokens(labels, out)


_PREP_SCRATCH: Dict[tuple, torch.Tensor] = {}


def prep_batch(src, tgt, ctr=None):
    src = src.contiguous()
    tgt = tgt.contiguous()
    B, T1 = tgt.shape
    tgt_in = torch.empty(B, T1 - 1, dtype=tgt.dtype, device=tgt.device)
    labels = torch.empty(B, T1 - 1, dtype=tgt.dtype, device=tgt.device)
    lens = torch.empty(2, B, dtype=torch.int32, device=tgt.device)
    ntok = torch.empty(1, dtype=torch.float32, device=tgt.device)
    key = (tgt.device, B)
    scratch = _PREP_SCRATCH.get(key)
    if scratch is None:
        scratch = _PREP_SCRATCH[key] = torch.zeros(B + 2, dtype=torch.int32, device=tgt.device)
    C().prep_batch(src, tgt, tgt_in, labels, lens[0], lens[1], ntok, ctr, scratch)
    return tgt_in, labels, lens[0], lens[1], ntok


def interior_pad_rows(reset: bool = False) -> int:
    n = 0
    for scratch in _PREP_SCRATCH.values():
        n += int(scratch[-1].item())
        if reset:
            scratch[-1].zero_()
    return n


def check_trailing_padding() -> None:
    n = interior_pad_rows(reset=True)
    if n:
        raise ValueError(f"{n} batch rows had a PAD (id 0) token before a non-PAD token; sequences "
                         "must be right-padded (attention masks keys by length)")


def xent(logits, V, labels, ntok, workers, smoothing, row_loss, row_correct, write_grad=True):
    C().xent(logits, V, labels, ntok, workers, smoothing, row_loss, row_correct, write_grad)


def xent_stats(row_loss, row_correct, ntok, workers, step_out=None, accum=None):
    C().xent_stats(row_loss, row_correct, ntok, workers, step_out, accum)


def adam_chunks(p, g, m, v, shadow, chunks, step, beta1, beta2, eps, lr_const, d_model, warmup,
                grad_scale, weight_decay, sched, zero_grad, inc_step, scale8, amax8, norm_state=None):
    C().adam_chunks(p, g, m, v, shadow, chunks, step, beta1, beta2, eps, lr_const, d_model, warmup,
                    grad_scale, weight_decay, sched, zero_grad, inc_step, scale8, amax8, norm_state)


def adam(p, g, m, v, shadow, step, beta1, beta2, eps, lr_const, d_model, warmup, grad_scale=1.0,
         weight_decay=0.0, sched=1, zero_grad=True, inc_step=True, norm_state=None):
    C().adam(p, g, m, v, shadow, step, beta1, beta2, eps, lr_const, d_model, warmup, grad_scale,
             weight_decay, sched, zero_grad, inc_step, norm_state)


def adam_step_inc(step, norm_state=None):
    C().adam_step_inc(step, norm_state)


NORM_SUMSQ, NORM_NORM, NORM_FACTOR, NORM_SKIP = 0, 1, 2, 3
NORM_CLIPPED, NORM_SKIPPED, NORM_MAX = 0, 1, 2


def grad_sumsq(g, partials, base=0, chunks=None) -> int:
    return C().grad_sumsq(g, chunks, partials, base)


def grad_norm_finalize(partials, nparts, state, counters, clip=0.0, skip_nonfinite=False,
                       grad_scale=1.0):
    C().grad_norm_finalize(partials, nparts, state, counters, clip, skip_nonfinite, grad_scale)


class StreamSignal:

    def __init__(self, device: torch.device):
        self.device = device.index if device.index is not None else torch.cuda.current_device()
        with torch.cuda.device(self.device):
            self._host, self._dhost, self._cnt = C().signal_create()
        self.expected = 0

    def emit(self) -> None:
        C().signal_emit(self._dhost, self._cnt, self.device)

    def wait(self, n: int, timeout_s: float) -> bool:
        return C().signal_wait(self._host, n, timeout_s)

    def value(self) -> int:
        return C().signal_read(self._host)
```

Baseline: 3.592 million tokens/s.

## Store FFN ReLU mask as packed bits and use it in dgrad epilogue

The FFN forward GEMM with the bias+ReLU epilogue now also writes a packed 1-bit-per-element ReLU mask, built in the LDS epilogue image. The backward dgrad GEMM reads this bitmap instead of the full bf16 activation `h` to apply the ReLU derivative, loading it into registers before the main loop. The goal is to cut the aux read traffic in the dgrad epilogue by a factor of 16, at the cost of an extra small write in the forward pass and extra epilogue bit manipulation. The new path is restricted to certain tile shapes and excludes split-K and some tile configs, so an autotuned config that falls outside these limits could return an error.

```diff
diff --git a/csrc/bindings/gemm.cpp b/csrc/bindings/gemm.cpp
--- a/csrc/bindings/gemm.cpp
+++ b/csrc/bindings/gemm.cpp
@@ -18,7 +18,8 @@
 void gemm(const Tensor& A, const Tensor& B, const Tensor& C, const optional<Tensor>& bias,
           const optional<Tensor>& aux, int64_t M, int64_t N, int64_t K, int64_t lda, int64_t ldb,
           int64_t ldc, int64_t ldaux, bool a_kc, bool b_kc, int64_t epi, double alpha,
-          double beta, int64_t tile_cfg, int64_t splits, const optional<Tensor>& ws) {
+          double beta, int64_t tile_cfg, int64_t splits, const optional<Tensor>& ws,
+          const optional<Tensor>& relu_bits, int64_t ldbits) {
   TORCH_CHECK(C.is_cuda(), "C must be a GPU tensor");
   const bool f32 = C.scalar_type() == at::kFloat;
   TORCH_CHECK(f32 || C.scalar_type() == at::kBFloat16, "C must be f32 or bf16");
@@ -38,7 +39,17 @@
     bptr = bias->data_ptr<float>();
   }
   const void* xptr = nullptr;
-  if (epi == 3) {
+  void* bits = nullptr;
+  if (relu_bits.has_value()) {
+    TORCH_CHECK(epi == 2 || epi == 3, "gemm: relu_bits needs the bias+ReLU or ReLU-backward epilogue");
+    TORCH_CHECK(relu_bits->is_cuda() && relu_bits->scalar_type() == at::kByte,
+                "relu_bits must be a uint8 GPU tensor");
+    TORCH_CHECK(N % 8 == 0, "gemm: relu_bits needs N % 8 == 0");
+    TORCH_CHECK(ldbits >= N / 8, "gemm: ldbits < N / 8");
+    check_extent(*relu_bits, M, ldbits, N / 8, "relu_bits");
+    bits = relu_bits->data_ptr();
+  }
+  if (epi == 3 && bits == nullptr) {
     TORCH_CHECK(aux.has_value(), "gemm: DRELU epilogue needs aux");
     check_bf16(*aux, "aux");
     check_extent(*aux, M, ldaux, N, "aux");
@@ -55,7 +66,7 @@
   const int rc = tdg_gemm(A.data_ptr(), B.data_ptr(), C.data_ptr(), bptr, xptr, (int)M, (int)N,
                           (int)K, (int)lda, (int)ldb, (int)ldc, (int)ldaux, a_kc, b_kc, (int)epi,
                           f32, (float)alpha, (float)beta, (int)tile_cfg, (int)splits, wptr,
-                          stream_of(A));
+                          stream_of(A), bits, (int)ldbits);
   check_err(rc, "tdg gemm");
 }
 
@@ -171,7 +182,11 @@
 }
 
 void def_gemm(py::module_& m) {
-  m.def("gemm", &gemm);
+  m.def("gemm", &gemm, py::arg("A"), py::arg("B"), py::arg("C"), py::arg("bias"), py::arg("aux"),
+        py::arg("M"), py::arg("N"), py::arg("K"), py::arg("lda"), py::arg("ldb"), py::arg("ldc"),
+        py::arg("ldaux"), py::arg("a_kc"), py::arg("b_kc"), py::arg("epi"), py::arg("alpha"),
+        py::arg("beta"), py::arg("tile_cfg"), py::arg("splits"), py::arg("ws"),
+        py::arg("relu_bits") = optional<Tensor>(), py::arg("ldbits") = 0);
   m.def("gemm_grouped", &gemm_grouped);
   m.def("gemm_ragged", &gemm_ragged, py::arg("As"), py::arg("Bs"), py::arg("Cs"), py::arg("shapes"),
         py::arg("K"), py::arg("a_kc"), py::arg("b_kc"), py::arg("alpha"), py::arg("beta"),
diff --git a/csrc/include/tdg_api.h b/csrc/include/tdg_api.h
--- a/csrc/include/tdg_api.h
+++ b/csrc/include/tdg_api.h
@@ -9,7 +9,7 @@
 int tdg_gemm(const void* A, const void* B, void* C, const float* bias, const void* aux, int M,
              int N, int K, int lda, int ldb, int ldc, int ldaux, int a_kc, int b_kc, int epi,
              int out_f32, float alpha, float beta, int tile_cfg, int splits, float* ws,
-             hipStream_t st);
+             hipStream_t st, void* relu_bits, int ldbits);
 int tdg_gemm_grouped(const void* const* A, const void* const* B, void* const* C, int G, int M,
                      int N, int K, int lda, int ldb, int ldc, int a_kc, int b_kc, int out_f32,
                      float alpha, float beta, int tile_cfg, hipStream_t st);
diff --git a/csrc/include/tdg_gemm.h b/csrc/include/tdg_gemm.h
--- a/csrc/include/tdg_gemm.h
+++ b/csrc/include/tdg_gemm.h
@@ -163,12 +163,17 @@
   EPI_BIAS = 1,
   EPI_BIAS_RELU = 2,
   EPI_DRELU = 3,
+  EPI_BIAS_RELU_BITS = 4,
+  EPI_DRELU_BITS = 5,
 };
+constexpr bool epi_has_bias(int e) { return e == EPI_BIAS || e == EPI_BIAS_RELU || e == EPI_BIAS_RELU_BITS; }
+constexpr bool epi_has_relu(int e) { return e == EPI_BIAS_RELU || e == EPI_BIAS_RELU_BITS; }
+constexpr bool epi_has_bits(int e) { return e == EPI_BIAS_RELU_BITS || e == EPI_DRELU_BITS; }
 
 template <int EPI>
 __device__ __forceinline__ f32x4 load_bias4(const float* __restrict__ bias, int n, int N) {
   f32x4 b = {0.f, 0.f, 0.f, 0.f};
-  if constexpr (EPI == EPI_BIAS || EPI == EPI_BIAS_RELU) {
+  if constexpr (epi_has_bias(EPI)) {
     if (n + 4 <= N && (reinterpret_cast<uintptr_t>(bias + n) & 15) == 0) {
       b = *reinterpret_cast<const f32x4*>(bias + n);
     } else {
@@ -255,6 +260,39 @@
   static constexpr int BYTES = RPASS * SP;
   static_assert(RPASS % 16 == 0 && (TM * 16) % RPASS == 0, "passes of whole 16-row sub-tiles");
   static_assert((RPASS * CPR) % 64 == 0, "whole chunk iterations");
+  static constexpr bool BITS = epi_has_bits(EPI);
+  static constexpr int PAD = TN * 16 * ES;
+  static constexpr int MBW = CPR / 4 > 0 ? CPR / 4 : 1;
+  static constexpr int MBR = MBW * ((TM * 16 + 63) / 64);
+  static_assert(!BITS || (!OUT_F32 && (CPR == 4 || CPR == 8) && (RPASS == 64 || RPASS == TM * 16)),
+                "bitmap epilogues: bf16 out, 32/64-wide wave tiles, rows of a pass held by lanes 0..RPASS-1");
+
+  __device__ static __forceinline__ void mask_load(uint32_t (&mb)[MBR], const unsigned char* bits,
+                                                   int ldb, int M, int N, int mw0, int nw0, int lane) {
+    const bool wide = nw0 + TN * 16 <= N && (ldb % (4 * MBW)) == 0 &&
+                      (reinterpret_cast<uintptr_t>(bits) % (4 * MBW)) == 0;
+#pragma unroll
+    for (int k = 0; k < MBR / MBW; ++k) {
+      int m = mw0 + lane + 64 * k;
+      m = m < M ? m : M - 1;
+      const unsigned char* p = bits + (size_t)m * ldb + (nw0 >> 3);
+      if (wide) {
+        if constexpr (MBW == 2) {
+          const uint2 v = *reinterpret_cast<const uint2*>(p);
+          mb[2 * k] = v.x;
+          mb[2 * k + 1] = v.y;
+        } else {
+          mb[k] = *reinterpret_cast<const uint32_t*>(p);
+        }
+      } else {
+#pragma unroll
+        for (int w = 0; w < MBW; ++w) mb[MBW * k + w] = 0u;
+#pragma unroll
+        for (int c = 0; c < CPR; ++c)
+          if (nw0 + 8 * c < N) mb[MBW * k + c / 4] |= (uint32_t)p[c] << (8 * (c % 4));
+      }
+    }
+  }
 
   __device__ static __forceinline__ int row_of(int lane, int t) { return (lane + 64 * t) / CPR; }
   __device__ static __forceinline__ int col_of(int lane, int t) { return ((lane + 64 * t) % CPR) * EPC; }
@@ -265,8 +303,19 @@
                                              const float* __restrict__ bias,
                                              const bf16_t* __restrict__ aux, int ldaux, bool vec) {
     int4 none[ITER];
+    uint32_t nomask[MBR];
     run_pre<false>(wimg, acc, lane, Cv, ldc, M, N, mw0, nw0, alpha, beta, bias, aux, ldaux, vec,
-                   none, false, none, false);
+                   none, false, none, false, nomask);
+  }
+  __device__ static __forceinline__ void run_mask(char* wimg, const f32x4 (&acc)[TM][TN], int lane,
+                                                  void* __restrict__ Cv, int ldc, int M, int N,
+                                                  int mw0, int nw0, float alpha, float beta,
+                                                  const float* __restrict__ bias,
+                                                  const bf16_t* __restrict__ aux, int ldaux, bool vec,
+                                                  const uint32_t (&mb)[MBR]) {
+    int4 none[ITER];
+    run_pre<false>(wimg, acc, lane, Cv, ldc, M, N, mw0, nw0, alpha, beta, bias, aux, ldaux, vec,
+                   none, false, none, false, mb);
   }
   template <bool PRE>
   __device__ static __forceinline__ void run_pre(char* wimg, const f32x4 (&acc)[TM][TN], int lane,
@@ -275,7 +324,8 @@
                                                  const float* __restrict__ bias,
                                                  const bf16_t* __restrict__ aux, int ldaux, bool vec,
                                                  const int4 (&pre_aux)[ITER], bool use_aux,
-                                                 const int4 (&pre_c)[ITER], bool use_c) {
+                                                 const int4 (&pre_c)[ITER], bool use_c,
+                                                 const uint32_t (&mb)[MBR]) {
     const int g = lane >> 4, r16 = lane & 15;
     bool vok = vec && ((ldc * ES) % 16) == 0 && (reinterpret_cast<uintptr_t>(Cv) & 15) == 0;
     if constexpr (EPI == EPI_DRELU)
@@ -310,6 +360,14 @@
           }
         }
       }
+      if constexpr (EPI == EPI_DRELU_BITS) {
+        if (RPASS == 64 || lane < RPASS) {
+          const int k = p * RPASS / 64;
+          char* dst = wimg + lane * SP + PAD;
+          if constexpr (MBW == 2) *reinterpret_cast<uint2*>(dst) = uint2{mb[2 * k], mb[2 * k + 1]};
+          else *reinterpret_cast<uint32_t*>(dst) = mb[k];
+        }
+      }
 #pragma unroll
       for (int ii = 0; ii < RPASS / 16; ++ii) {
         const int i = p * (RPASS / 16) + ii;
@@ -320,7 +378,7 @@
           for (int r = 0; r < 4; ++r) {
             v[r] = alpha * acc[i][j][r];
             if constexpr (EPI == EPI_BIAS) v[r] += bn[j][r];
-            if constexpr (EPI == EPI_BIAS_RELU) v[r] = fmaxf(v[r] + bn[j][r], 0.f);
+            if constexpr (epi_has_relu(EPI)) v[r] = fmaxf(v[r] + bn[j][r], 0.f);
           }
           char* dst = wimg + (16 * ii + r16) * SP + (16 * j + 4 * g) * ES;
           if constexpr (OUT_F32) {
@@ -343,7 +401,19 @@
         VecT vals = *reinterpret_cast<const VecT*>(wimg + row * SP + ch * 16);
         if (m >= M || n >= N) continue;
         char* cp = reinterpret_cast<char*>(Cv) + ((size_t)m * ldc + n) * ES;
-        if (vok && n + EPC <= N) {
+        if (BITS || (vok && n + EPC <= N)) {
+          if constexpr (EPI == EPI_DRELU_BITS) {
+            const uint32_t b = *reinterpret_cast<const unsigned char*>(wimg + row * SP + PAD + ch);
+#pragma unroll
+            for (int e = 0; e < 8; ++e)
+              if (!((b >> e) & 1u)) vals[e] = 0;
+          }
+          if constexpr (EPI == EPI_BIAS_RELU_BITS) {
+            uint32_t b = 0;
+#pragma unroll
+            for (int e = 0; e < 8; ++e) b |= (bf2f((bf16_t)vals[e]) > 0.f ? 1u : 0u) << e;
+            *reinterpret_cast<unsigned char*>(wimg + row * SP + PAD + ch) = (unsigned char)b;
+          }
           if constexpr (EPI == EPI_DRELU) {
             if constexpr (EPC == 8) {
               const short8_t x = __builtin_bit_cast(short8_t, (PRE && use_aux) ? pre_aux[t] : la[t]);
@@ -372,7 +442,7 @@
 #else
           *reinterpret_cast<VecT*>(cp) = vals;
 #endif
-        } else {
+        } else if constexpr (!BITS) {
 #pragma unroll
           for (int e = 0; e < EPC; ++e) {
             if (n + e >= N) break;
@@ -392,6 +462,25 @@
           }
         }
       }
+      if constexpr (EPI == EPI_BIAS_RELU_BITS) {
+        asm volatile("s_waitcnt lgkmcnt(0)" ::: "memory");
+        unsigned char* bits = reinterpret_cast<unsigned char*>(const_cast<bf16_t*>(aux));
+        const int m = mw0 + p * RPASS + lane;
+        if ((RPASS == 64 || lane < RPASS) && m < M && nw0 < N) {
+          const char* src = wimg + lane * SP + PAD;
+          unsigned char* dst = bits + (size_t)m * ldaux + (nw0 >> 3);
+          const bool wide = nw0 + TN * 16 <= N && (ldaux % (4 * MBW)) == 0 &&
+                            (reinterpret_cast<uintptr_t>(bits) % (4 * MBW)) == 0;
+          if (wide) {
+            if constexpr (MBW == 2) *reinterpret_cast<uint2*>(dst) = *reinterpret_cast<const uint2*>(src);
+            else *reinterpret_cast<uint32_t*>(dst) = *reinterpret_cast<const uint32_t*>(src);
+          } else {
+#pragma unroll
+            for (int c = 0; c < CPR; ++c)
+              if (nw0 + 8 * c < N) dst[c] = (unsigned char)src[c];
+          }
+        }
+      }
       asm volatile("s_waitcnt lgkmcnt(0)" ::: "memory");
     }
   }
diff --git a/csrc/kernels/gemm.hip b/csrc/kernels/gemm.hip
--- a/csrc/kernels/gemm.hip
+++ b/csrc/kernels/gemm.hip
@@ -109,10 +109,21 @@
 extern "C" int tdg_gemm(const void* A, const void* B, void* C, const float* bias, const void* aux,
                         int M, int N, int K, int lda, int ldb, int ldc, int ldaux, int a_kc,
                         int b_kc, int epi, int out_f32, float alpha, float beta, int tile_cfg,
-                        int splits, float* ws, hipStream_t st) {
+                        int splits, float* ws, hipStream_t st, void* relu_bits, int ldbits) {
   const bf16_t* a = (const bf16_t*)A;
   const bf16_t* b = (const bf16_t*)B;
   const bf16_t* x = (const bf16_t*)aux;
+  if (relu_bits) {
+    if (epi != EPI_BIAS_RELU && epi != EPI_DRELU) return -11;
+    if (out_f32 || N % 8 != 0 || ldc % 8 != 0 || (reinterpret_cast<uintptr_t>(C) & 15) != 0 ||
+        ldbits < N / 8)
+      return -11;
+    epi = epi == EPI_BIAS_RELU ? EPI_BIAS_RELU_BITS : EPI_DRELU_BITS;
+    x = (const bf16_t*)relu_bits;
+    ldaux = ldbits;
+  } else if (epi > EPI_DRELU) {
+    return -1;
+  }
   auto fn = a_kc ? (b_kc ? gemm_nt : gemm_nn) : (b_kc ? gemm_tt : gemm_tn);
   return fn(epi, out_f32 != 0, tile_cfg, a, b, C, bias, x, M, N, K, lda, ldb, ldc, ldaux, alpha,
             beta, splits, ws, st);
diff --git a/csrc/kernels/gemm_impl.h b/csrc/kernels/gemm_impl.h
--- a/csrc/kernels/gemm_impl.h
+++ b/csrc/kernels/gemm_impl.h
@@ -92,6 +92,10 @@
     if (pre_c && in)
       c_r[t] = *reinterpret_cast<const int4*>(reinterpret_cast<const OutT*>(Cv) + (size_t)m * ldc + n);
   }
+  uint32_t mask_r[Epi::MBR];
+  if constexpr (EPI == EPI_DRELU_BITS)
+    Epi::mask_load(mask_r, reinterpret_cast<const unsigned char*>(aux), ldaux, M, N, m0 + wm * WTM,
+                   n0 + wn * WTN, lane);
 
   f32x4 acc[TM][TN];
 #pragma unroll
@@ -194,7 +198,7 @@
               nullptr, 0, epi_vec_ok<EPI_NONE, true>(Cs, ldc, nullptr, 0));
   } else {
     Epi::template run_pre<true>(smem + wid * Epi::BYTES, acc, lane, Cv, ldc, M, N, mw0, nw0, alpha,
-                                beta, bias, aux, ldaux, vec, aux_r, pre_aux, c_r, pre_c);
+                                beta, bias, aux, ldaux, vec, aux_r, pre_aux, c_r, pre_c, mask_r);
   }
 #ifdef TDG_STAMPS
   TDG_STAMP(3);
@@ -338,6 +342,11 @@
     if (ph == 0) bsum0 = bs;
     else bsum1 = bs;
   };
+  using Epi = EpiLds<EPI, OUT_F32, 8, 4, (OUT_F32 ? 32 : 64)>;
+  uint32_t mask_r[Epi::MBR];
+  if constexpr (EPI == EPI_DRELU_BITS)
+    Epi::mask_load(mask_r, reinterpret_cast<const unsigned char*>(aux), ldaux, M, N, m0 + wm * 128,
+                   n0 + wn * 64, lane);
   {
 #pragma unroll
     for (int h = 0; h < 4; ++h) issue_half(0, h);
@@ -471,11 +480,14 @@
   wait_vmcnt<0>();
   lds_barrier();
   {
-    constexpr int RPASS = OUT_F32 ? 32 : 64;
-    using Epi = EpiLds<EPI, OUT_F32, 8, 4, RPASS>;
     static_assert(8 * Epi::BYTES <= 2 * 4 * 128 * BK * 2, "epilogue images fit in the stages");
-    Epi::run(smem + wid * Epi::BYTES, acc, lane, Cv, ldc, M, N, m0 + wm * 128, n0 + wn * 64, alpha,
-             beta, bias, aux, ldaux, epi_vec_ok<EPI, OUT_F32>(Cv, ldc, aux, ldaux));
+    if constexpr (EPI == EPI_DRELU_BITS)
+      Epi::run_mask(smem + wid * Epi::BYTES, acc, lane, Cv, ldc, M, N, m0 + wm * 128, n0 + wn * 64,
+                    alpha, beta, bias, aux, ldaux, epi_vec_ok<EPI, OUT_F32>(Cv, ldc, aux, ldaux),
+                    mask_r);
+    else
+      Epi::run(smem + wid * Epi::BYTES, acc, lane, Cv, ldc, M, N, m0 + wm * 128, n0 + wn * 64, alpha,
+               beta, bias, aux, ldaux, epi_vec_ok<EPI, OUT_F32>(Cv, ldc, aux, ldaux));
   }
 #ifdef TDG_STAMPS
   TDG_STAMP(3);
@@ -557,7 +569,7 @@
 template <bool AK, bool BKc, int EPI, bool F32>
 constexpr bool has_256() {
   if (AK && BKc) return !F32 || EPI == EPI_NONE;
-  if (AK && !BKc) return !F32 && (EPI == EPI_NONE || EPI == EPI_DRELU);
+  if (AK && !BKc) return !F32 && (EPI == EPI_NONE || EPI == EPI_DRELU || EPI == EPI_DRELU_BITS);
   if (!AK && !BKc) return EPI == EPI_NONE;
   return false;
 }
@@ -612,6 +624,8 @@
 bool launch_pipe(const bf16_t* A, const bf16_t* B, void* C, const float* bias, const bf16_t* aux,
                  int M, int N, int K, int lda, int ldb, int ldc, int ldaux, float alpha, float beta,
                  hipStream_t st) {
+  if constexpr (epi_has_bits(EPI) && BN / WN > 64) return false;
+  else {
   if (K % PK != 0 || K <= 0) return false;
   const long long ab = AK ? (long long)(M - 1) * lda + K : (long long)(K - 1) * lda + M;
   const long long bb = BKc ? (long long)(N - 1) * ldb + K : (long long)(K - 1) * ldb + N;
@@ -630,6 +644,7 @@
                      st, A, B, C, bias, aux, M, N, K, lda, ldb, ldc, ldaux, alpha, beta,
                      (int)(ab * 2), (int)(bb * 2));
   return true;
+  }
 }
 
 template <bool AK, bool BKc, int EPI, bool F32>
@@ -716,6 +731,13 @@
   TDG_E(EPI_BIAS, true)
   TDG_E(EPI_BIAS_RELU, false)
   TDG_E(EPI_DRELU, false)
+  if (epi_has_bits(epi) && (splits > 1 || (tile_cfg >= 23 && tile_cfg <= 26))) return -12;
+  if constexpr (AK && BKc) {
+    TDG_E(EPI_BIAS_RELU_BITS, false)
+  }
+  if constexpr (AK) {
+    TDG_E(EPI_DRELU_BITS, false)
+  }
 #undef TDG_E
   return -1;
 }
diff --git a/csrc/kernels/gemm_pipe.h b/csrc/kernels/gemm_pipe.h
--- a/csrc/kernels/gemm_pipe.h
+++ b/csrc/kernels/gemm_pipe.h
@@ -230,6 +230,12 @@
     for (int j = 0; j < TN; ++j) acc[i][j] = f32x4{0.f, 0.f, 0.f, 0.f};
 
   const int abase = wm * WTM, bbase = wn * WTN;
+  constexpr int RPASS = OUT_F32 ? (WTM < 32 ? WTM : 32) : (WTM > 64 ? 64 : WTM);
+  using Epi = EpiLds<EPI, OUT_F32, TM, TN, RPASS>;
+  uint32_t mask_r[Epi::MBR];
+  if constexpr (EPI == EPI_DRELU_BITS)
+    Epi::mask_load(mask_r, reinterpret_cast<const unsigned char*>(aux), ldaux, M, N, m0 + abase,
+                   n0 + bbase, lane);
 #pragma unroll
   for (int s = 0; s < NS - 1; ++s)
     if (s < nk) P::stage(sa, sb, smem, s, wid);
@@ -267,11 +273,14 @@
   {
     using OutT = typename std::conditional<OUT_F32, float, bf16_t>::type;
     (void)sizeof(OutT);
-    constexpr int RPASS = OUT_F32 ? (WTM < 32 ? WTM : 32) : (WTM > 64 ? 64 : WTM);
-    using Epi = EpiLds<EPI, OUT_F32, TM, TN, RPASS>;
     static_assert(NW * Epi::BYTES <= NS * SB, "epilogue images fit in the stages");
-    Epi::run(smem + wid * Epi::BYTES, acc, lane, Cv, ldc, M, N, m0 + wm * WTM, n0 + wn * WTN, alpha,
-             beta, bias, aux, ldaux, epi_vec_ok<EPI, OUT_F32>(Cv, ldc, aux, ldaux));
+    if constexpr (EPI == EPI_DRELU_BITS)
+      Epi::run_mask(smem + wid * Epi::BYTES, acc, lane, Cv, ldc, M, N, m0 + wm * WTM, n0 + wn * WTN,
+                    alpha, beta, bias, aux, ldaux, epi_vec_ok<EPI, OUT_F32>(Cv, ldc, aux, ldaux),
+                    mask_r);
+    else
+      Epi::run(smem + wid * Epi::BYTES, acc, lane, Cv, ldc, M, N, m0 + wm * WTM, n0 + wn * WTN, alpha,
+               beta, bias, aux, ldaux, epi_vec_ok<EPI, OUT_F32>(Cv, ldc, aux, ldaux));
   }
 }
 
diff --git a/tensorflow_distributed_on_gke_amd/models/layers.py b/tensorflow_distributed_on_gke_amd/models/layers.py
--- a/tensorflow_distributed_on_gke_amd/models/layers.py
+++ b/tensorflow_distributed_on_gke_amd/models/layers.py
@@ -874,6 +874,9 @@
         return (dx.view(B, T, d), dkv_ret) + (None,) * 12
 
 
+RELU_BITS = os.environ.get("TDG_RELU_BITS", "1") != "0"
+
+
 class FFNBlockFn(torch.autograd.Function):
 
     @staticmethod
@@ -885,6 +888,7 @@
         ctx.meta = (site, rt)
         ctx.f8 = None
         ctx.lean = False
+        ctx.hbits = None
         if x.is_cuda and rt.fp8 is not None:
             st = rt.fp8
             xs, hs = st.ffn_slots[id(w1)]
@@ -903,7 +907,12 @@
             ctx.f8 = (x8, h8) if rt.training else None
             ctx.lean = lean
         elif x.is_cuda:
-            h = K.linear_fwd(x2, w1.compute, b1.master, relu=True)
+            ff = w1.shape[0]
+            hbits = None
+            if RELU_BITS and rt.training and ff % 8 == 0:
+                hbits = torch.empty(B * L, ff // 8, dtype=torch.uint8, device=x.device)
+            h = K.linear_fwd(x2, w1.compute, b1.master, relu=True, relu_bits=hbits)
+            ctx.hbits = hbits
             f = None
         else:
             h = torch.relu(x2 @ w1.master.t() + b1.master)
@@ -957,10 +966,11 @@
                 fp8.gemm_bf8_dgrad(dpre8, st.gmeta, gh, w1t8, st.meta, s1t, dh.view(M, d), beta=1.0,
                                    w_plain=wp)
                 return (dh.view(B, L, d),) + (None,) * 8
+            mask = dict(relu_bits=ctx.hbits) if ctx.hbits is not None else dict(relu_aux=h)
             if w2.compute_t is not None and not w2.compute_t_stale:
-                dpre = K.linear_dgrad_t(ds2, w2.compute_t, relu_aux=h)
+                dpre = K.linear_dgrad_t(ds2, w2.compute_t, **mask)
             else:
-                dpre = K.linear_dgrad(ds2, w2.compute, d, relu_aux=h)
+                dpre = K.linear_dgrad(ds2, w2.compute, d, **mask)
             _wgrad(rt, dpre, x2, ff, w1, b1)
             dx = _dgrad_res(dpre, w1, ff, dh)
             return (dx.view(B, L, d),) + (None,) * 8
diff --git a/tensorflow_distributed_on_gke_amd/ops/kernels.py b/tensorflow_distributed_on_gke_amd/ops/kernels.py
--- a/tensorflow_distributed_on_gke_amd/ops/kernels.py
+++ b/tensorflow_distributed_on_gke_amd/ops/kernels.py
@@ -131,13 +131,18 @@
 
 
 def gemm(A, B, Cout, M, N, K, lda, ldb, ldc, a_kc, b_kc, epi=EPI_NONE, bias=None, aux=None,
-         ldaux=0, alpha=1.0, beta=0.0, cfg: Optional[Tuple[int, int]] = None) -> torch.Tensor:
+         ldaux=0, alpha=1.0, beta=0.0, cfg: Optional[Tuple[int, int]] = None,
+         relu_bits: Optional[torch.Tensor] = None) -> torch.Tensor:
 
     def run(c, out=Cout):
         tile, splits = c
         ws = workspace("splitk", splits * M * ldc, A.device) if splits > 1 else None
-        C().gemm(A, B, out, bias, aux, M, N, K, lda, ldb, ldc, ldaux, a_kc, b_kc, epi, alpha,
-                 beta, tile, splits, ws)
+        if relu_bits is None:
+            C().gemm(A, B, out, bias, aux, M, N, K, lda, ldb, ldc, ldaux, a_kc, b_kc, epi, alpha,
+                     beta, tile, splits, ws)
+        else:
+            C().gemm(A, B, out, bias, aux, M, N, K, lda, ldb, ldc, ldaux, a_kc, b_kc, epi, alpha,
+                     beta, tile, splits, ws, relu_bits=relu_bits, ldbits=relu_bits.stride(0))
 
     if cfg is None:
         Mk, Kk = (M, _tok_bucket(K)) if (not a_kc and not b_kc) else (_tok_bucket(M), K)
@@ -169,26 +174,40 @@
             for k, v in _TUNED.items()}
 
 
+def pack_relu_bits(h: torch.Tensor) -> torch.Tensor:
+    M, N = h.shape
+    w = (1 << torch.arange(8, device=h.device, dtype=torch.int32))
+    return ((h > 0).view(M, N // 8, 8).to(torch.int32) * w).sum(-1).to(torch.uint8)
+
+
 def linear_fwd(x2: torch.Tensor, w: torch.Tensor, bias: Optional[torch.Tensor], relu: bool = False,
-               out: Optional[torch.Tensor] = None, ldc: Optional[int] = None) -> torch.Tensor:
+               out: Optional[torch.Tensor] = None, ldc: Optional[int] = None,
+               relu_bits: Optional[torch.Tensor] = None) -> torch.Tensor:
     M, K = x2.shape
     N = w.shape[0]
     ldc = ldc or N
     if out is None:
         out = torch.empty(M, ldc, dtype=torch.bfloat16, device=x2.device)
     epi = EPI_BIAS_RELU if relu else (EPI_BIAS if bias is not None else EPI_NONE)
-    return gemm(x2, w, out, M, N, K, x2.stride(0), w.stride(0), ldc, True, True, epi, bias=bias)
+    if relu_bits is not None and not relu:
+        raise ValueError("linear_fwd: relu_bits needs relu=True")
+    return gemm(x2, w, out, M, N, K, x2.stride(0), w.stride(0), ldc, True, True, epi, bias=bias,
+                relu_bits=relu_bits)
 
 
 def linear_dgrad(dy2: torch.Tensor, w: torch.Tensor, N: int, relu_aux: Optional[torch.Tensor] = None,
-                 out: Optional[torch.Tensor] = None, beta: float = 0.0) -> torch.Tensor:
+                 out: Optional[torch.Tensor] = None, beta: float = 0.0,
+                 relu_bits: Optional[torch.Tensor] = None) -> torch.Tensor:
     M = dy2.shape[0]
     K = w.shape[1]
     if out is None:
         out = torch.empty(M, K, dtype=torch.bfloat16, device=dy2.device)
-    epi = EPI_DRELU if relu_aux is not None else EPI_NONE
+    if relu_bits is not None:
+        relu_aux = None
+    epi = EPI_DRELU if (relu_aux is not None or relu_bits is not None) else EPI_NONE
     return gemm(dy2, w, out, M, K, N, dy2.stride(0), w.stride(0), out.stride(0), True, False, epi,
-                aux=relu_aux, ldaux=(relu_aux.stride(0) if relu_aux is not None else 0), beta=beta)
+                aux=relu_aux, ldaux=(relu_aux.stride(0) if relu_aux is not None else 0), beta=beta,
+                relu_bits=relu_bits)
 
 
 def transpose_grouped(srcs, dsts) -> None:
@@ -197,14 +216,18 @@
 
 
 def linear_dgrad_t(dy2: torch.Tensor, w_t: torch.Tensor, relu_aux: Optional[torch.Tensor] = None,
-                   out: Optional[torch.Tensor] = None) -> torch.Tensor:
+                   out: Optional[torch.Tensor] = None,
+                   relu_bits: Optional[torch.Tensor] = None) -> torch.Tensor:
     M, K = dy2.shape
     N = w_t.shape[0]
     if out is None:
         out = torch.empty(M, N, dtype=torch.bfloat16, device=dy2.device)
-    epi = EPI_DRELU if relu_aux is not None else EPI_NONE
+    if relu_bits is not None:
+        relu_aux = None
+    epi = EPI_DRELU if (relu_aux is not None or relu_bits is not None) else EPI_NONE
     return gemm(dy2, w_t, out, M, N, K, dy2.stride(0), w_t.stride(0), out.stride(0), True, True, epi,
-                aux=relu_aux, ldaux=(relu_aux.stride(0) if relu_aux is not None else 0))
+                aux=relu_aux, ldaux=(relu_aux.stride(0) if relu_aux is not None else 0),
+                relu_bits=relu_bits)
 
 
 def linear_wgrad(dy2: torch.Tensor, x2: torch.Tensor, N: int, dw: torch.Tensor,
```

New measurement: 3.641 million tokens/s (median of 6 runs). 1.01x the previous value.
